# mosure/bevy_gaussian_splatting

Measured on AMD Instinct MI355X. Metric: frames/sec @1080p, 1M-splat 3DGS (sort + rasterize every frame), higher is better.
Workload: dtype f32; 1 GPU; 1000000-splat 3DGS f32 planar cloud (seed 2, reference random_gaussians_3d distributions), 1920x1080, SH degree 3, CloudSettings::default(), examples/headless.rs camera incl. its Msaa (Bevy's default Sample4: 4 samples per pixel, resolved frame); one camera per GPU; sample_count=4, parallelism=views1, sort=radix32, frames_in_flight=8, lanes=8, streams=4

## Files before the change

### bevy_gaussian_splatting_amd/_native.py

```python
from __future__ import annotations

import ctypes
import os
from typing import Optional

from . import _build_id
from .camera import BgsView
from .settings import BgsSettings

_HERE = os.path.dirname(os.path.abspath(__file__))
LIB_PATH = os.path.join(_HERE, "csrc", "libbgs.so")

BGS_OK = 0
BGS_EINVAL = -1
BGS_ENOMEM = -2
BGS_EHIP = -3
BGS_ECAPACITY = -4
BGS_EINTERNAL = -5

STAGE_NAMES = ("keygen", "depth_sort", "project", "tile_sort", "ranges", "raster")

EXPORTED_SYMBOLS = (
    "bgs_create",
    "bgs_destroy",
    "bgs_last_error",
    "bgs_version",
    "bgs_build_id",
    "bgs_set_queue_holders",
    "bgs_set_tile_trace",
    "bgs_selftest_ln_f32",
    "bgs_selftest_pack",
    "bgs_settings_default",
    "bgs_view_perspective",
    "bgs_cloud_upload_f32",
    "bgs_cloud_upload_f16",
    "bgs_cloud_free",
    "bgs_cloud_len",
    "bgs_sort",
    "bgs_render",
    "bgs_framebuffer_device_ptr",
    "bgs_sorted_entries_device_ptr",
    "bgs_set_output_srgb8",
    "bgs_framebuffer_srgb8_device_ptr",
    "bgs_set_srgb8_target",
    "bgs_set_pipeline_depth",
    "bgs_pipeline_pop",
    "bgs_frames_in_flight",
    "bgs_synchronize",
    "bgs_set_async",
    "bgs_stream",
    "bgs_set_profiling",
    "bgs_set_profiling_stride",
    "bgs_set_binning",
    "bgs_set_debug_flags",
    "bgs_get_stats",
    "bgs_radix_sort_pairs",
    "bgs_hbm_probe",
    "bgs_download",
    "bgs_set_pipeline_streams",
    "bgs_set_graphs",
    "bgs_graph_counters",
    "bgs_tile_order_counters",
    "bgs_selftest_tile_order",
    "bgs_reset_adaptive_state",
    "bgs_cloud_upload_cov3d_f32",
    "bgs_adaptive_counters",
    "bgs_set_output_rgba16f",
    "bgs_framebuffer_rgba16f_device_ptr",
    "bgs_set_packed_only",
    "bgs_device_alloc",
    "bgs_device_free",
    "bgs_upload",
    "bgs_abi_check",
    "bgs_learning_counters",
    "bgs_comm_unique_id",
    "bgs_comm_create",
    "bgs_comm_gather",
    "bgs_comm_gather_after",
    "bgs_comm_wait",
    "bgs_comm_stream",
    "bgs_comm_destroy",
)

COMM_ID_BYTES = 128
ABI_VERSION = (0 << 16) | 4


class BgsSortEntry(ctypes.Structure):
    _fields_ = [("key", ctypes.c_uint32), ("index", ctypes.c_uint32)]


class BgsStats(ctypes.Structure):
    _fields_ = [
        ("stage_ms", ctypes.c_float * 6),
        ("total_ms", ctypes.c_float),
        ("splat_count", ctypes.c_uint32),
        ("visible_count", ctypes.c_uint32),
        ("draw_count", ctypes.c_uint32),
        ("sort_path", ctypes.c_uint32),
        ("instance_count", ctypes.c_uint64),
        ("instance_capacity", ctypes.c_uint64),
        ("tiles_x", ctypes.c_uint32),
        ("tiles_y", ctypes.c_uint32),
        ("depth_passes", ctypes.c_uint32),
        ("tile_passes", ctypes.c_uint32),
        ("algorithmic_bytes", ctypes.c_uint64),
        ("regrow_count", ctypes.c_uint32),
        ("binning_mode", ctypes.c_uint32),
        ("frames_averaged", ctypes.c_uint32),
        ("list_capacity", ctypes.c_uint32),
        ("list_entries_allocated", ctypes.c_uint64),
        ("strip_tiles", ctypes.c_uint32),
        ("tile_saturation", ctypes.c_uint32),
    ]


class BgsError(RuntimeError):
    def __init__(self, status: int, message: str):
        super().__init__(f"libbgs error {status}: {message}")
        self.status = status


_lib: Optional[ctypes.CDLL] = None


def rebuild() -> str:
    import subprocess
    p = subprocess.run(["make", "-C", os.path.join(_HERE, "csrc"), "-j4", "ARCH=gfx950"], stdout=subprocess.PIPE,
                       stderr=subprocess.STDOUT, text=True)
    if p.returncode != 0:
        raise ImportError(f"building libbgs.so failed:\n{p.stdout}")
    return p.stdout


def ensure_current() -> str:
    want = _build_id.kernel_source_sha256()
    have = _build_id.library_build_id(LIB_PATH) if os.path.exists(LIB_PATH) else None
    if have != want and os.environ.get("BGS_NO_AUTOBUILD", "0") != "1":
        import fcntl
        with open(os.path.join(_HERE, "csrc", ".build.lock"), "w") as lock:
            fcntl.flock(lock, fcntl.LOCK_EX)
            try:
                have = _build_id.library_build_id(LIB_PATH) if os.path.exists(LIB_PATH) else None
                if have != want:
                    rebuild()
                    have = _build_id.library_build_id(LIB_PATH) if os.path.exists(LIB_PATH) else None
            finally:
                fcntl.flock(lock, fcntl.LOCK_UN)
    if have is None:
        raise ImportError(
            f"{LIB_PATH} not found (or it carries no build id): build the HIP extension first "
            "(python -c 'import __graft_entry__ as g; g.build()'); there is no CPU fallback")
    if have != want:
        raise ImportError(f"{LIB_PATH} was built from kernel sources {have[:12]}, this tree is {want[:12]}: rebuild it "
                          "(make -C bevy_gaussian_splatting_amd/csrc)")
    return want


def build_id() -> str:
    return load().bgs_build_id().decode()


def load() -> ctypes.CDLL:
    global _lib
    if _lib is not None:
        return _lib
    override = os.environ.get("BGS_LIB_OVERRIDE")
    if override:
        import sys
        print(f"bevy_gaussian_splatting_amd: BGS_LIB_OVERRIDE={override} — NOT the library of this tree "
              f"(build id {_build_id.library_build_id(override)})", file=sys.stderr)
        lib = ctypes.CDLL(override, mode=ctypes.RTLD_GLOBAL)
        lib.bgs_build_id.argtypes = []
        lib.bgs_build_id.restype = ctypes.c_char_p
    else:
        want = ensure_current()
        lib = ctypes.CDLL(LIB_PATH, mode=ctypes.RTLD_GLOBAL)
        lib.bgs_build_id.argtypes = []
        lib.bgs_build_id.restype = ctypes.c_char_p
        if lib.bgs_build_id().decode() != want:
            raise ImportError(f"{LIB_PATH}: bgs_build_id() disagrees with the id in the file's bytes")
    vp = ctypes.c_void_p
    u32 = ctypes.c_uint32
    fp = ctypes.POINTER(ctypes.c_float)
    up = ctypes.POINTER(ctypes.c_uint32)

    lib.bgs_create.argtypes = [ctypes.c_int, ctypes.POINTER(vp)]
    lib.bgs_create.restype = ctypes.c_int
    lib.bgs_destroy.argtypes = [vp]
    lib.bgs_destroy.restype = None
    lib.bgs_last_error.argtypes = [vp]
    lib.bgs_last_error.restype = ctypes.c_char_p
    lib.bgs_version.argtypes = []
    lib.bgs_version.restype = u32
    lib.bgs_build_id.argtypes = []
    lib.bgs_build_id.restype = ctypes.c_char_p
    lib.bgs_set_tile_trace.argtypes = [vp, vp]
    lib.bgs_set_tile_trace.restype = ctypes.c_int
    lib.bgs_set_queue_holders.argtypes = [ctypes.c_int]
    lib.bgs_set_queue_holders.restype = ctypes.c_int
    lib.bgs_selftest_ln_f32.argtypes = [vp, u32, u32, ctypes.POINTER(ctypes.c_float), ctypes.POINTER(ctypes.c_uint64)]
    lib.bgs_selftest_ln_f32.restype = ctypes.c_int
    lib.bgs_selftest_pack.argtypes = [vp, u32, vp, u32, vp]
    lib.bgs_selftest_pack.restype = ctypes.c_int
    lib.bgs_settings_default.argtypes = [ctypes.POINTER(BgsSettings)]
    lib.bgs_settings_default.restype = None
    lib.bgs_view_perspective.argtypes = [
        fp, ctypes.c_float, ctypes.c_float, u32, u32, ctypes.POINTER(BgsView)]
    lib.bgs_view_perspective.restype = None
    lib.bgs_cloud_upload_f32.argtypes = [vp, u32, fp, fp, fp, fp, ctypes.POINTER(vp)]
    lib.bgs_cloud_upload_f32.restype = ctypes.c_int
    lib.bgs_cloud_upload_f16.argtypes = [vp, u32, fp, up, up, ctypes.POINTER(vp)]
    lib.bgs_cloud_upload_f16.restype = ctypes.c_int
    lib.bgs_cloud_free.argtypes = [vp, vp]
    lib.bgs_cloud_free.restype = None
    lib.bgs_cloud_len.argtypes = [vp]
    lib.bgs_cloud_len.restype = u32
    lib.bgs_sort.argtypes = [
        vp, vp, ctypes.POINTER(BgsView), ctypes.POINTER(BgsSettings), ctypes.POINTER(BgsSortEntry)]
    lib.bgs_sort.restype = ctypes.c_int
    lib.bgs_render.argtypes = [
        vp, vp, ctypes.POINTER(BgsView), ctypes.POINTER(BgsSettings), fp]
    lib.bgs_render.restype = ctypes.c_int
    lib.bgs_framebuffer_device_ptr.argtypes = [vp, ctypes.POINTER(vp), ctypes.POINTER(ctypes.c_uint64)]
    lib.bgs_framebuffer_device_ptr.restype = ctypes.c_int
    lib.bgs_sorted_entries_device_ptr.argtypes = [vp, ctypes.POINTER(vp), up]
    lib.bgs_sorted_entries_device_ptr.restype = ctypes.c_int
    lib.bgs_synchronize.argtypes = [vp]
    lib.bgs_synchronize.restype = ctypes.c_int
    lib.bgs_set_output_srgb8.argtypes = [vp, ctypes.c_int]
    lib.bgs_set_output_srgb8.restype = ctypes.c_int
    lib.bgs_framebuffer_srgb8_device_ptr.argtypes = [vp, ctypes.POINTER(vp), ctypes.POINTER(ctypes.c_uint64)]
    lib.bgs_framebuffer_srgb8_device_ptr.restype = ctypes.c_int
    lib.bgs_set_srgb8_target.argtypes = [vp, vp]
    lib.bgs_set_srgb8_target.restype = ctypes.c_int
    lib.bgs_set_pipeline_depth.argtypes = [vp, u32]
    lib.bgs_set_pipeline_depth.restype = ctypes.c_int
    lib.bgs_pipeline_pop.argtypes = [vp, ctypes.POINTER(vp), ctypes.POINTER(vp)]
    lib.bgs_pipeline_pop.restype = ctypes.c_int
    lib.bgs_frames_in_flight.argtypes = [vp, up]
    lib.bgs_frames_in_flight.restype = ctypes.c_int
    lib.bgs_set_async.argtypes = [vp, ctypes.c_int]
    lib.bgs_set_async.restype = ctypes.c_int
    lib.bgs_stream.argtypes = [vp, ctypes.POINTER(vp)]
    lib.bgs_stream.restype = ctypes.c_int
    lib.bgs_set_profiling.argtypes = [vp, ctypes.c_int]
    lib.bgs_set_profiling.restype = ctypes.c_int
    lib.bgs_set_profiling_stride.argtypes = [vp, u32]
    lib.bgs_set_profiling_stride.restype = ctypes.c_int
    lib.bgs_set_binning.argtypes = [vp, u32]
    lib.bgs_set_binning.restype = ctypes.c_int
    lib.bgs_set_debug_flags.argtypes = [vp, u32]
    lib.bgs_set_debug_flags.restype = ctypes.c_int
    lib.bgs_get_stats.argtypes = [vp, ctypes.POINTER(BgsStats)]
    lib.bgs_get_stats.restype = ctypes.c_int
    lib.bgs_radix_sort_pairs.argtypes = [vp, ctypes.POINTER(BgsSortEntry), u32, u32]
    lib.bgs_radix_sort_pairs.restype = ctypes.c_int
    lib.bgs_hbm_probe.argtypes = [ctypes.c_void_p, ctypes.c_uint64, ctypes.c_uint32,
                                  ctypes.POINTER(ctypes.c_float), ctypes.POINTER(ctypes.c_float)]
    lib.bgs_hbm_probe.restype = ctypes.c_int
    lib.bgs_download.argtypes = [vp, vp, vp, ctypes.c_uint64]
    lib.bgs_download.restype = ctypes.c_int
    lib.bgs_set_pipeline_streams.argtypes = [vp, u32]
    lib.bgs_set_pipeline_streams.restype = ctypes.c_int
    lib.bgs_set_graphs.argtypes = [vp, ctypes.c_int]
    lib.bgs_set_graphs.restype = ctypes.c_int
    lib.bgs_graph_counters.argtypes = [vp, ctypes.POINTER(ctypes.c_uint64), ctypes.POINTER(ctypes.c_uint64)]
    lib.bgs_graph_counters.restype = ctypes.c_int
    lib.bgs_tile_order_counters.argtypes = [vp] + [ctypes.POINTER(ctypes.c_uint64)] * 3
    lib.bgs_tile_order_counters.restype = ctypes.c_int
    lib.bgs_selftest_tile_order.argtypes = [vp, vp, u32, u32, vp, vp]
    lib.bgs_selftest_tile_order.restype = ctypes.c_int
    lib.bgs_cloud_upload_cov3d_f32.argtypes = [vp, ctypes.c_uint32, ctypes.POINTER(ctypes.c_float), ctypes.POINTER(ctypes.c_float),
                                               ctypes.POINTER(ctypes.c_float), ctypes.POINTER(vp)]
    lib.bgs_cloud_upload_cov3d_f32.restype = ctypes.c_int
    lib.bgs_set_output_rgba16f.argtypes = [vp, ctypes.c_int]
    lib.bgs_set_output_rgba16f.restype = ctypes.c_int
    lib.bgs_set_packed_only.argtypes = [vp, ctypes.c_int]
    lib.bgs_set_packed_only.restype = ctypes.c_int
    lib.bgs_framebuffer_rgba16f_device_ptr.argtypes = [vp, ctypes.POINTER(vp), ctypes.POINTER(ctypes.c_uint64)]
    lib.bgs_framebuffer_rgba16f_device_ptr.restype = ctypes.c_int
    lib.bgs_device_alloc.argtypes = [vp, ctypes.c_uint64, ctypes.POINTER(vp)]
    lib.bgs_device_alloc.restype = ctypes.c_int
    lib.bgs_device_free.argtypes = [vp, vp]
    lib.bgs_device_free.restype = ctypes.c_int
    lib.bgs_upload.argtypes = [vp, vp, vp, ctypes.c_uint64]
    lib.bgs_upload.restype = ctypes.c_int
    lib.bgs_adaptive_counters.argtypes = [vp, ctypes.POINTER(ctypes.c_uint64)]
    lib.bgs_adaptive_counters.restype = ctypes.c_int
    lib.bgs_reset_adaptive_state.argtypes = [vp]
    lib.bgs_reset_adaptive_state.restype = ctypes.c_int
    lib.bgs_learning_counters.argtypes = [vp, ctypes.POINTER(ctypes.c_uint64), ctypes.POINTER(ctypes.c_uint64)]
    lib.bgs_learning_counters.restype = ctypes.c_int
    lib.bgs_abi_check.argtypes = [u32, u32, u32, u32]
    lib.bgs_abi_check.restype = ctypes.c_int
    lib.bgs_comm_unique_id.argtypes = [ctypes.c_char_p]
    lib.bgs_comm_unique_id.restype = ctypes.c_int
    lib.bgs_comm_create.argtypes = [vp, ctypes.c_char_p, u32, u32, ctypes.POINTER(vp)]
    lib.bgs_comm_create.restype = ctypes.c_int
    lib.bgs_comm_gather.argtypes = [vp, vp, u32, vp, ctypes.c_uint64, vp, ctypes.POINTER(ctypes.c_uint64)]
    lib.bgs_comm_gather.restype = ctypes.c_int
    lib.bgs_comm_gather_after.argtypes = [vp, vp, u32, vp, ctypes.c_uint64, vp, vp, ctypes.POINTER(ctypes.c_uint64)]
    lib.bgs_comm_gather_after.restype = ctypes.c_int
    lib.bgs_comm_wait.argtypes = [vp, vp, ctypes.c_uint64]
    lib.bgs_comm_wait.restype = ctypes.c_int
    lib.bgs_comm_stream.argtypes = [vp, vp, ctypes.POINTER(vp)]
    lib.bgs_comm_stream.restype = ctypes.c_int
    lib.bgs_comm_destroy.argtypes = [vp, vp]
    lib.bgs_comm_destroy.restype = None
    rc = lib.bgs_abi_check(ABI_VERSION, ctypes.sizeof(BgsView), ctypes.sizeof(BgsSettings), ctypes.sizeof(BgsStats))
    if rc != BGS_OK:
        raise ImportError("libbgs.so refuses this binding: " + (lib.bgs_last_error(None) or b"").decode("utf-8", "replace"))
    _lib = lib
    return lib


def check(lib: ctypes.CDLL, ctx, status: int) -> None:
    if status != BGS_OK:
        msg = lib.bgs_last_error(ctx)
        raise BgsError(status, msg.decode("utf-8", "replace") if msg else "")
```

### bevy_gaussian_splatting_amd/csrc/bgs_api.hip

```cpp
#include "bgs_context.h"
#include "build_id.inc"

static const char g_build_id[] = "BGS_BUILD_ID=" BGS_BUILD_ID;

namespace {
void mat4_mul(const float* a, const float* b, float* out) {
    for (int c = 0; c < 4; ++c)
        for (int r = 0; r < 4; ++r) {
            float acc = 0.0f;
            for (int k = 0; k < 4; ++k) acc += a[4 * k + r] * b[4 * c + k];
            out[4 * c + r] = acc;
        }
}

bool mat4_inverse(const float* m, float* out) {
    double a[4][8];
    for (int r = 0; r < 4; ++r)
        for (int c = 0; c < 4; ++c) {
            a[r][c] = m[4 * c + r];
            a[r][4 + c] = r == c ? 1.0 : 0.0;
        }
    for (int i = 0; i < 4; ++i) {
        int piv = i;
        for (int r = i + 1; r < 4; ++r)
// ... 154 lines not shown
    if (n && (!pv || !sh || !rot || !so)) return fail(ctx, BGS_EINVAL, "NULL plane pointer");
    if (hipSetDevice(ctx->device) != hipSuccess) return fail(ctx, BGS_EHIP, "hipSetDevice failed");
    bgs_cloud* c = new (std::nothrow) bgs_cloud();
    if (!c) return fail(ctx, BGS_ENOMEM, "out of host memory");
    const void* const planes[3] = {rot, so, sh};
    const uint32_t v4[3] = {1u, 1u, 12u};
    int rc = upload_and_pack(ctx, c, CLOUD_F32, n, pv, planes, v4, 16u);
    if (rc != BGS_OK) { bgs_cloud_free(ctx, c); return rc; }
    *out = c;
    return BGS_OK;
}

int bgs_cloud_upload_f16(bgs_ctx* ctx, uint32_t n, const float* pv, const uint32_t* sh_h2,
                         const uint32_t* rso, bgs_cloud** out) {
    if (!ctx) return fail(nullptr, BGS_EINVAL, "ctx is NULL");
    if (!out) return fail(ctx, BGS_EINVAL, "out is NULL");
    *out = nullptr;
    if (n > MAX_SPLATS) return fail(ctx, BGS_EINVAL, "too many splats");
    if (n && (!pv || !sh_h2 || !rso)) return fail(ctx, BGS_EINVAL, "NULL plane pointer");
    if (hipSetDevice(ctx->device) != hipSuccess) return fail(ctx, BGS_EHIP, "hipSetDevice failed");
    bgs_cloud* c = new (std::nothrow) bgs_cloud();
    if (!c) return fail(ctx, BGS_ENOMEM, "out of host memory");
    const void* const planes[3] = {rso, sh_h2, nullptr};
    const uint32_t v4[3] = {1u, 6u, 0u};
    int rc = upload_and_pack(ctx, c, CLOUD_F16, n, pv, planes, v4, 8u);
    if (rc != BGS_OK) { bgs_cloud_free(ctx, c); return rc; }
    *out = c;
    return BGS_OK;
}

int bgs_cloud_upload_cov3d_f32(bgs_ctx* ctx, uint32_t n, const float* pv, const float* sh, const float* cov3d_opacity,
                               bgs_cloud** out) {
    if (!ctx) return fail(nullptr, BGS_EINVAL, "ctx is NULL");
    if (!out) return fail(ctx, BGS_EINVAL, "out is NULL");
    *out = nullptr;
    if (n > MAX_SPLATS) return fail(ctx, BGS_EINVAL, "too many splats");
    if (n && (!pv || !sh || !cov3d_opacity)) return fail(ctx, BGS_EINVAL, "NULL plane pointer");
    if (hipSetDevice(ctx->device) != hipSuccess) return fail(ctx, BGS_EHIP, "hipSetDevice failed");
    bgs_cloud* c = new (std::nothrow) bgs_cloud();
    if (!c) return fail(ctx, BGS_ENOMEM, "out of host memory");
    const void* const planes[3] = {cov3d_opacity, nullptr, sh};
    const uint32_t v4[3] = {2u, 0u, 12u};
    int rc = upload_and_pack(ctx, c, CLOUD_COV3D, n, pv, planes, v4, 16u);
    if (rc != BGS_OK) { bgs_cloud_free(ctx, c); return rc; }
    *out = c;
    return BGS_OK;
}

void bgs_cloud_free(bgs_ctx* ctx, bgs_cloud* cloud) {
    if (!cloud) return;
    if (ctx) {
        (void)hipSetDevice(ctx->device);
        (void)finish_all(ctx);
        for (auto& L : ctx->lanes) {
            if (L.stream) (void)hipStreamSynchronize(L.stream);
            if (L.in.cloud == cloud) L.in.cloud = nullptr;
        }
        for (auto& sl : ctx->split_slots)
            if (sl.cloud == cloud) sl.epoch = 0;
    }
    for (auto p : cloud->allocs) if (p) (void)hipFree(p);
    delete cloud;
}

uint32_t bgs_cloud_len(const bgs_cloud* cloud) { return cloud ? cloud->ptrs.n : 0; }

int bgs_sort(bgs_ctx* ctx, const bgs_cloud* cloud, const bgs_view* view, const bgs_settings* settings,
             bgs_sort_entry* host_out) {
    int rc = run(ctx, cloud, view, settings, false);
    if (rc != BGS_OK) return rc;
    Lane& L = ctx->lanes[0];
    if (host_out && L.last_sorted_n)
        HIP_TRY(ctx, hipMemcpy(host_out, L.last_sorted, (size_t)L.last_sorted_n * sizeof(uint2), hipMemcpyDeviceToHost));
    return BGS_OK;
}

int bgs_render(bgs_ctx* ctx, const bgs_cloud* cloud, const bgs_view* view, const bgs_settings* settings,
               float* rgba_host_out) {
    int rc = run(ctx, cloud, view, settings, true);
    if (rc != BGS_OK) return rc;
    if (rgba_host_out) {
        Lane& L = ctx->lanes[ctx->recent];
        if (L.pending && (rc = finish_lane(ctx, L)) != BGS_OK) return rc;
        if (!L.fb_valid) return fail(ctx, BGS_EINVAL, "the frame wrote its packed image only (bgs_set_packed_only): no f32 target to copy");
        HIP_TRY(ctx, hipMemcpy(rgba_host_out, L.fb, (size_t)L.fb_w * L.fb_h * sizeof(float4), hipMemcpyDeviceToHost));
    }
    return BGS_OK;
}

int bgs_framebuffer_device_ptr(bgs_ctx* ctx, void** dptr, uint64_t* bytes) {
    if (!ctx || !dptr) return fail(ctx, BGS_EINVAL, "NULL argument");
    Lane& L = ctx->lanes[ctx->recent];
    if (L.pending) {
        int rc = finish_lane(ctx, L);
        if (rc != BGS_OK) return rc;
    }
    if (!L.fb) return fail(ctx, BGS_EINVAL, "no frame has been rendered yet");
    if (!L.fb_valid) return fail(ctx, BGS_EINVAL, "the last frame wrote its packed image only (bgs_set_packed_only)");
    *dptr = L.fb;
    if (bytes) *bytes = (uint64_t)L.fb_w * L.fb_h * sizeof(float4);
    return BGS_OK;
}

int bgs_framebuffer_srgb8_device_ptr(bgs_ctx* ctx, void** dptr, uint64_t* bytes) {
    if (!ctx || !dptr) return fail(ctx, BGS_EINVAL, "NULL argument");
    Lane& L = ctx->lanes[ctx->recent];
    if (L.pending) {
        int rc = finish_lane(ctx, L);
        if (rc != BGS_OK) return rc;
    }
    if (!L.fb8_out || !L.fb8_valid || L.fb8_is_f16)
        return fail(ctx, BGS_EINVAL, "no Rgba8UnormSrgb frame: call bgs_set_output_srgb8(ctx, 1) before rendering");
    *dptr = L.fb8_out;
    if (bytes) *bytes = (uint64_t)L.fb_w * L.fb_h * 4u;
    return BGS_OK;
}

int bgs_pipeline_pop(bgs_ctx* ctx, void** rgba_f32, void** rgba8) {
    if (!ctx) return fail(nullptr, BGS_EINVAL, "ctx is NULL");
    if (hipSetDevice(ctx->device) != hipSuccess) return fail(ctx, BGS_EHIP, "hipSetDevice failed");
    int best = -1;
    for (int i = 0; i < MAX_LANES; ++i)
        if ((ctx->lanes[i].pending || ctx->lanes[i].ready) && (best < 0 || ctx->lanes[i].seq < ctx->lanes[best].seq)) best = i;
    if (best < 0) return fail(ctx, BGS_EINVAL, "no frame in flight");
    Lane& L = ctx->lanes[best];
    int rc = finish_lane(ctx, L);
    if (rc != BGS_OK) return rc;
    if (rgba_f32) *rgba_f32 = L.fb_valid ? L.fb : nullptr;
    if (rgba8) *rgba8 = L.fb8_valid ? L.fb8_out : nullptr;
    return BGS_OK;
}

int bgs_frames_in_flight(bgs_ctx* ctx, uint32_t* count) {
    if (!ctx || !count) return fail(ctx, BGS_EINVAL, "NULL argument");
    uint32_t c = 0;
    for (auto& L : ctx->lanes) c += (L.pending || L.ready) ? 1u : 0u;
    *count = c;
    return BGS_OK;
}

int bgs_sorted_entries_device_ptr(bgs_ctx* ctx, void** dptr, uint32_t* n) {
    if (!ctx || !dptr) return fail(ctx, BGS_EINVAL, "NULL argument");
    Lane& L = ctx->lanes[ctx->recent];
    if (L.pending) {
        int rc = finish_lane(ctx, L);
        if (rc != BGS_OK) return rc;
    }
    if (!L.last_sorted) return fail(ctx, BGS_EINVAL, "no sort has been run yet");
    *dptr = (void*)L.last_sorted;
    if (n) *n = L.last_sorted_n;
    return BGS_OK;
}

int bgs_synchronize(bgs_ctx* ctx) {
    if (!ctx) return fail(nullptr, BGS_EINVAL, "ctx is NULL");
    if (hipSetDevice(ctx->device) != hipSuccess) return fail(ctx, BGS_EHIP, "hipSetDevice failed");
    int rc = finish_all(ctx);
    if (rc != BGS_OK) return rc;
    for (auto& L : ctx->lanes)
        if (L.stream) HIP_TRY(ctx, hipStreamSynchronize(L.stream));
    return BGS_OK;
}

int bgs_set_async(bgs_ctx* ctx, int enabled) {
    if (!ctx) return fail(nullptr, BGS_EINVAL, "ctx is NULL");
    if (!enabled) {
        int rc = finish_all(ctx);
        if (rc != BGS_OK) return rc;
    }
    ctx->async_frames = enabled != 0;
    return BGS_OK;
}

int bgs_set_pipeline_depth(bgs_ctx* ctx, uint32_t lanes) {
    if (!ctx) return fail(nullptr, BGS_EINVAL, "ctx is NULL");
    if (lanes < 1 || lanes > (uint32_t)MAX_LANES) return fail(ctx, BGS_EINVAL, "pipeline depth must be 1..8");
    if (hipSetDevice(ctx->device) != hipSuccess) return fail(ctx, BGS_EHIP, "hipSetDevice failed");
    int rc = finish_all(ctx);
    if (rc != BGS_OK) return rc;
    ctx->depth = (int)lanes;
    ctx->next = 0;
    ctx->recent = 0;
    for (uint32_t i = 0; i < lanes; ++i)
        if ((rc = lane_create(ctx, ctx->lanes[i])) != BGS_OK) return rc;
    return assign_streams(ctx);
}

int bgs_set_pipeline_streams(bgs_ctx* ctx, uint32_t streams) {
    if (!ctx) return fail(nullptr, BGS_EINVAL, "ctx is NULL");
    if (streams > (uint32_t)MAX_LANES) return fail(ctx, BGS_EINVAL, "pipeline streams must be 0..8");
    if (hipSetDevice(ctx->device) != hipSuccess) return fail(ctx, BGS_EHIP, "hipSetDevice failed");
    int rc = finish_all(ctx);
    if (rc != BGS_OK) return rc;
    for (auto st : ctx->streams)
        if (st) HIP_TRY(ctx, hipStreamSynchronize(st));
    ctx->num_streams = (int)streams;
    return assign_streams(ctx);
}

int bgs_set_srgb8_target(bgs_ctx* ctx, void* device_ptr) {
    if (!ctx) return fail(nullptr, BGS_EINVAL, "ctx is NULL");
    ctx->next_srgb8_target = (uint32_t*)device_ptr;
    return BGS_OK;
}

int bgs_download(bgs_ctx* ctx, const void* device_ptr, void* host_out, uint64_t bytes) {
    if (!ctx || !device_ptr || !host_out) return fail(ctx, BGS_EINVAL, "NULL argument");
    if (hipSetDevice(ctx->device) != hipSuccess) return fail(ctx, BGS_EHIP, "hipSetDevice failed");
    if (bytes) HIP_TRY(ctx, hipMemcpy(host_out, device_ptr, (size_t)bytes, hipMemcpyDeviceToHost));
    return BGS_OK;
}

int bgs_device_alloc(bgs_ctx* ctx, uint64_t bytes, void** device_ptr_out) {
    if (!ctx || !device_ptr_out) return fail(ctx, BGS_EINVAL, "NULL argument");
    *device_ptr_out = nullptr;
    if (hipSetDevice(ctx->device) != hipSuccess) return fail(ctx, BGS_EHIP, "hipSetDevice failed");
    void* p = nullptr;
    if (hipMalloc(&p, std::max<size_t>((size_t)bytes, 16)) != hipSuccess) {
        (void)hipGetLastError();
        return fail(ctx, BGS_ENOMEM, "hipMalloc(" + std::to_string(bytes) + " bytes) failed");
    }
    *device_ptr_out = p;
    return BGS_OK;
}

int bgs_device_free(bgs_ctx* ctx, void* device_ptr) {
    if (!ctx) return fail(nullptr, BGS_EINVAL, "ctx is NULL");
    if (!device_ptr) return BGS_OK;
    if (hipSetDevice(ctx->device) != hipSuccess) return fail(ctx, BGS_EHIP, "hipSetDevice failed");
    int rc = finish_all(ctx);
    if (rc != BGS_OK) return rc;
    HIP_TRY(ctx, hipFree(device_ptr));
    return BGS_OK;
}

int bgs_upload(bgs_ctx* ctx, void* device_ptr, const void* host_in, uint64_t bytes) {
    if (!ctx || !device_ptr || !host_in) return fail(ctx, BGS_EINVAL, "NULL argument");
    if (hipSetDevice(ctx->device) != hipSuccess) return fail(ctx, BGS_EHIP, "hipSetDevice failed");
    if (bytes) HIP_TRY(ctx, hipMemcpy(device_ptr, host_in, (size_t)bytes, hipMemcpyHostToDevice));
    return BGS_OK;
}

int bgs_set_output_srgb8(bgs_ctx* ctx, int enabled) {
    if (!ctx) return fail(nullptr, BGS_EINVAL, "ctx is NULL");
    ctx->output_srgb8 = enabled != 0;
    if (enabled) ctx->output_rgba16f = false;
    return BGS_OK;
}

int bgs_set_output_rgba16f(bgs_ctx* ctx, int enabled) {
    if (!ctx) return fail(nullptr, BGS_EINVAL, "ctx is NULL");
    ctx->output_rgba16f = enabled != 0;
    if (enabled) ctx->output_srgb8 = false;
    return BGS_OK;
}

int bgs_set_packed_only(bgs_ctx* ctx, int enabled) {
    if (!ctx) return fail(nullptr, BGS_EINVAL, "ctx is NULL");
    ctx->packed_only = enabled != 0;
    return BGS_OK;
}

int bgs_framebuffer_rgba16f_device_ptr(bgs_ctx* ctx, void** dptr, uint64_t* bytes) {
    if (!ctx || !dptr) return fail(ctx, BGS_EINVAL, "NULL argument");
    Lane& L = ctx->lanes[ctx->recent];
    if (L.pending) {
        int rc = finish_lane(ctx, L);
        if (rc != BGS_OK) return rc;
    }
    if (!L.fb8_out || !L.fb8_valid || !L.fb8_is_f16)
        return fail(ctx, BGS_EINVAL, "no Rgba16Float frame: call bgs_set_output_rgba16f(ctx, 1) before rendering");
    *dptr = L.fb8_out;
    if (bytes) *bytes = (uint64_t)L.fb_w * L.fb_h * 8u;
    return BGS_OK;
}

int bgs_stream(bgs_ctx* ctx, void** hip_stream) {
    if (!ctx || !hip_stream) return fail(ctx, BGS_EINVAL, "NULL argument");
    *hip_stream = (void*)ctx->lanes[ctx->recent].stream;
    return BGS_OK;
}

int bgs_set_profiling(bgs_ctx* ctx, int enabled) {
    if (!ctx) return fail(nullptr, BGS_EINVAL, "ctx is NULL");
    if (enabled < 0 || enabled > 2) return fail(ctx, BGS_EINVAL, "profiling level must be 0, 1 or 2");
    ctx->profiling = enabled;
    return BGS_OK;
}

int bgs_set_profiling_stride(bgs_ctx* ctx, uint32_t every_nth_frame) {
    if (!ctx) return fail(nullptr, BGS_EINVAL, "ctx is NULL");
    if (every_nth_frame == 0) return fail(ctx, BGS_EINVAL, "stride must be >= 1");
    ctx->profiling_stride = every_nth_frame;
    ctx->frame_counter = 0;
    return BGS_OK;
}

int bgs_set_binning(bgs_ctx* ctx, uint32_t mode) {
    if (!ctx) return fail(nullptr, BGS_EINVAL, "ctx is NULL");
    if (mode > BINNING_SORT) return fail(ctx, BGS_EINVAL, "binning mode must be 0 (scan) or 1 (sort)");
    int rc = finish_all(ctx);
    if (rc != BGS_OK) return rc;
    ctx->binning = mode;
    return BGS_OK;
}

// ... 102 lines not shown
```

### bevy_gaussian_splatting_amd/csrc/bgs_context.h

```cpp
#pragma once
#include <hip/hip_runtime.h>

#include <dlfcn.h>

#include <algorithm>
#include <chrono>
#include <cmath>
#include <cstdio>
#include <cstdlib>
#include <cstring>
#include <mutex>
#include <new>
#include <string>
#include <unordered_map>
#include <vector>

#include "../../include/bgs.h"
#include "../../include/bgs_diag.h"
#include "bgs_device.h"
#include "frame_params.h"
#include "kernels.h"

using namespace bgs;

struct bgs_cloud {
    CloudPtrs ptrs{};
    void* allocs[4] = {nullptr, nullptr, nullptr, nullptr};
    uint64_t bytes = 0;
};

namespace bgs_host {

extern thread_local std::string g_error;

constexpr uint64_t MIN_INSTANCE_CAPACITY = 1ull << 22;
constexpr uint64_t MAX_INSTANCE_CAPACITY = 1ull << 30;
constexpr uint32_t MAX_SPLATS = (1u << 30) - 1u;
constexpr int EV_COUNT = BGS_STAGE_COUNT + 1;
constexpr int EV_RING = 64;
constexpr int MAX_LANES = 8;

template <class T>
T* dev_alloc(size_t count) {
    void* p = nullptr;
    if (hipMalloc(&p, std::max<size_t>(count, 1) * sizeof(T)) != hipSuccess) return nullptr;
    return (T*)p;
}

struct GraphKey {
    const void* cloud[6];
    const void* bufs[11];
    uint32_t n, format, places, sort_mode, gaussian_mode, aabb, any_mode, srgb8, debug_flags;
    int32_t width, height;
    int32_t sort_blocks, bin_blocks, keygen_blocks;
    uint32_t sup_edge;
    uint64_t scratch_bytes, scratch_inst_cap;
    uint32_t scratch_n, coarse_cap, sort_path;
    const void* keygen_func;
    uint32_t keygen_threads;
    uint32_t wide_bin;
    uint32_t raster_variant;
    uint32_t split_sub;
};
struct FrameGraph {
    hipGraph_t graph = nullptr;
    hipGraphExec_t exec = nullptr;
    hipGraphNode_t keygen_node = nullptr;
    GraphKey key{};
};

struct FrameInputs {
    const bgs_cloud* cloud = nullptr;
    bgs_view view{};
    bgs_settings settings{};
    bool render = false, allow_graph = false;
    uint32_t* srgb8_target = nullptr;
    bool output_srgb8 = false, output_rgba16f = false, packed_only = false;
    uint32_t debug_flags = 0;
    uint64_t kind = 0;
    bool force_passes = false;
};

struct FramePlan {
    FrameParams fp{};
    bool render = false, scan = false, surfel = false, culled_tail = true;
    uint32_t n = 0, places = 0, rec_bytes = 0, cloud_format = 0;
    bool bucket = false, wide = false;
    uint32_t bucket_sub = 1, split_sub_out = 1;
    int split_slot = -1;
    uint64_t split_epoch = 0;
    uint32_t edges[4] = {6, 8, 16, 32}, level = 1, sup_edge = 8, num_st = 0;
    bool large = false, wide_bin = false, want_srgb8 = false;
    int sort_blocks = 0, bin_blocks = 0, binning_blocks = 0;
    uint32_t out_format = 0, ntiles = 0;
    bool raster_cleans = false;
    RasterInst raster{};
    bool heavy = false, cost = false, ordered = false, refresh = false, graph_ok = false;
    uint64_t sat_kind = 0;
};

struct Lane {
    hipStream_t stream = nullptr;
    hipEvent_t done = nullptr;
    FrameParams* d_fp = nullptr;
    FrameGraph graph[2];

    uint8_t* scratch = nullptr;
    size_t scratch_bytes = 0;
    size_t off_depth_status = 0, off_scan_status = 0, off_tile_status = 0, off_ranges = 0, off_bin_status = 0,
           off_part_status = 0, off_ctl1 = 0;
    uint32_t ctl_parity = 0;
    bool scratch_clean = false;
    uint32_t scratch_n = 0;
    uint64_t scratch_inst_cap = 0;

    uint2* entries[2] = {nullptr, nullptr};
    uint2* culled = nullptr;
    uint32_t entries_cap = 0;
    void* records = nullptr;
    size_t records_bytes = 0;
    uint32_t* rects = nullptr;
    uint2* inst[2] = {nullptr, nullptr};
    uint64_t inst_cap = 0;
    uint32_t* coarse = nullptr;
    size_t coarse_entries = 0;
    uint2* bucket_slots = nullptr;
    uint32_t bucket_sub_cap = 0;
    uint32_t* d_split_keys = nullptr;
    uint32_t* h_split_keys = nullptr;
    uint8_t* heavy[2] = {nullptr, nullptr};
    uint32_t heavy_tiles = 0, heavy_parity = 0;
    const uint8_t* heavy_done = nullptr;
    uint32_t heavy_done_grid = 0;
    bool ready = false;
    uint16_t* cost[2] = {nullptr, nullptr};
    uint16_t* order = nullptr;
    uint32_t cost_tiles = 0, cost_parity = 0;
    const uint16_t* cost_done = nullptr;
    uint32_t cost_done_grid = 0;
    uint32_t order_grid = 0xFFFFFFFFu, order_age = 0;
    float4* fb = nullptr;
    size_t fb_pixels = 0;
    uint32_t* fb8 = nullptr;
    uint32_t* fb8_out = nullptr;
    size_t fb8_pixels = 0;
    uint32_t fb_w = 0, fb_h = 0;
    bool fb8_valid = false, fb8_is_f16 = false;
    bool fb_valid = true;

    Control* h_ctl = nullptr;
    Control* h_ctl_dev = nullptr;
    hipEvent_t ev_ring[EV_RING][EV_COUNT] = {};
    uint8_t ev_kind[EV_RING] = {};
    uint32_t ev_head = 0;
    uint32_t frames_timed = 0;

    bool pending = false;
    FrameInputs in;
    FramePlan plan;
    uint32_t pending_coarse_cap = 0;
    uint64_t cost_done_kind = 0;
    uint64_t order_kind = 0;
    uint64_t seq = 0;

    const uint2* last_sorted = nullptr;
    uint32_t last_sorted_n = 0;

    bgs_stats result{};
    bool has_result = false;
    uint8_t result_kind = 0;
};

}
using namespace bgs_host;

struct bgs_ctx {
    int device = 0;
    int num_cus = 256;
    std::string error;

    Lane lanes[MAX_LANES];
    hipStream_t streams[MAX_LANES] = {};
    int num_streams = 4;
    int depth = 1;
    int next = 0;
    int recent = 0;
    uint64_t seq = 0;

    uint32_t binning = BINNING_SCAN;
    uint32_t debug_flags = 0;
    int profiling = 2;
    uint32_t profiling_stride = 1;
    uint32_t frame_counter = 0;
    bool async_frames = false;
    bool output_srgb8 = false;
    bool output_rgba16f = false;
    bool packed_only = false;
    uint32_t* next_srgb8_target = nullptr;

    uint32_t draw_hint = 0;
    bool draw_hint_valid = false;
    uint32_t draw_shrink_votes = 0;
    uint32_t sup_level = 1;
    struct SplitterSlot {
        SplitterKeys table{};
        const bgs_cloud* cloud = nullptr;
        uint32_t n = 0;
        uint32_t sort_mode = 0;
        float transform[16] = {};
        float pos[3] = {}, fwd[3] = {};
        float clip_from_view[16] = {};
        float viewport_wh[2] = {};
        float reach = 0.0f;
        uint64_t epoch = 0;
        uint64_t last_used = 0;
    };
    static constexpr int SPLITTER_SLOTS = 16;
    SplitterSlot split_slots[SPLITTER_SLOTS];
    uint64_t split_epoch = 0;
    uint64_t split_failed_epoch = 0;
    uint32_t bucket_block = 0;
    uint32_t bucket_fail_streak = 0;
    uint32_t list_shrink_votes = 0;
    uint64_t bucket_frames = 0, onesweep_frames = 0;
    uint64_t reruns_sort = 0, reruns_lists = 0, reruns_instances = 0, level_changes = 0;
    uint32_t coarse_cap_hint = 0;
    struct KindState { uint32_t sup_level = 1; bool midround = false; };
    std::unordered_map<uint64_t, KindState> kinds;
    static constexpr uint32_t LEARN_MAX = 3;
    static constexpr double MIDROUND_ON = 0.30, MIDROUND_OFF = 0.15;
    uint64_t cur_kind = 0;
    std::unordered_map<uint64_t, uint32_t> learning;
    uint64_t early_frames = 0;
    uint4* tile_trace = nullptr;
    bool use_graphs = false;
    uint64_t graph_captures = 0, graph_replays = 0;
    uint64_t cost_frames = 0, ordered_frames = 0, order_refreshes = 0;

    bool have_stats = false;
    bgs_stats stats{};
// ... 26 lines not shown
```

### bevy_gaussian_splatting_amd/csrc/bgs_frame.hip

```cpp
#include "bgs_context.h"

thread_local std::string bgs_host::g_error;

namespace bgs_host {


constexpr int MAX_DEVICES = 64;
hipStream_t g_queue_holders[MAX_DEVICES][3] = {};
int g_queue_holders_mode = -1;
std::mutex g_queue_holders_mutex;

int fail(bgs_ctx* ctx, int status, const std::string& msg) {
    if (ctx) ctx->error = msg;
    g_error = msg;
    return status;
}


size_t align_up(size_t v, size_t a) { return (v + a - 1) / a * a; }

int assign_streams(bgs_ctx* ctx) {
    const int S = ctx->num_streams > 0 ? std::min(ctx->num_streams, ctx->depth) : ctx->depth;
    for (int i = 0; i < MAX_LANES; ++i) {
        Lane& L = ctx->lanes[i];
// ... 514 lines not shown
    stt.tiles_x = render ? (uint32_t)p.fp.tiles_x : 0;
    stt.tiles_y = render ? (uint32_t)p.fp.tiles_y : 0;
    stt.depth_passes = p.places;
    stt.tile_passes = (render && !scan) ? 2 : 0;
    stt.binning_mode = scan ? BINNING_SCAN : BINNING_SORT;
    const uint64_t N = p.n, k = p.places, D = h.draw_count;
    uint64_t bytes = N * 16 + D * 8 + (p.culled_tail ? (N - D) * 8 : 0) + (p.bucket ? D * 24 : k * D * 16);
    if (render) {
        const uint64_t B = p.cloud_format == CLOUD_F16 ? 128 : 240, R = p.rec_bytes, V = h.visible_count, I = t.instances;
        const uint64_t P = (uint64_t)(uint32_t)p.fp.width * (uint32_t)p.fp.height;
        if (scan)
            bytes += V * (B - 16) + V * R + V * 8 + V * 8 + I * 8 + I * 8 + P * 16;
        else
            bytes += V * (B - 16) + V * R + I * 8 + 2 * I * 16 + I * (4 + R) + P * 16;
    }
    stt.algorithmic_bytes = bytes;
    L.has_result = true;
    L.result_kind = (uint8_t)(!render ? 1 : (scan ? 2 : 3));
}

int finish_lane(bgs_ctx* ctx, Lane& L) {
    L.ready = false;
    for (int attempt = 0; L.pending; ++attempt) {
        HIP_TRY(ctx, hipEventSynchronize(L.done));
        L.pending = false;
        int rc = check_watchdog(ctx, L);
        if (rc != BGS_OK) return rc;
        const FramePlan& p = L.plan;
        const Control& h = *L.h_ctl;
        const FrameTotals t = frame_totals(p, h);
        bool rerun = false;
        if ((rc = check_capacities(ctx, L, t, attempt, &rerun)) != BGS_OK) return rc;
        if (rerun) {
            if (attempt >= 8) return fail(ctx, BGS_ECAPACITY, "frame kept overflowing its buffers");
            ctx->regrow_count += 1;
            if ((rc = enqueue_frame(ctx, L, L.in)) != BGS_OK) return rc;
            continue;
        }

        if (p.render && p.scan) learn_feedback(ctx, L);
        learn_draw_hint(ctx, h.draw_count);
        learn_splitters(ctx, L);
        const bool level_moved = p.render && p.scan && h.visible_count > 0 && learn_level(ctx, L, t);
        if (p.render && p.scan && attempt == 0 && !level_moved && L.in.kind) {
            if (ctx->kinds.size() >= (1u << 20)) ctx->kinds.clear();
            ctx->kinds[L.in.kind].sup_level = p.level;
        }

        L.last_sorted_n = p.render ? h.draw_count : p.n;
        if (!p.render && h.draw_count < p.n) {
            HIP_TRY(ctx, hipMemcpyAsync(const_cast<uint2*>(L.last_sorted) + h.draw_count, L.culled,
                                        (size_t)(p.n - h.draw_count) * sizeof(uint2), hipMemcpyDeviceToDevice, L.stream));
            HIP_TRY(ctx, hipStreamSynchronize(L.stream));
        }
        fill_stats(ctx, L, t);
    }
    return BGS_OK;
}

int finish_all(bgs_ctx* ctx) {
    for (;;) {
        int best = -1;
        for (int i = 0; i < MAX_LANES; ++i)
            if (ctx->lanes[i].pending && (best < 0 || ctx->lanes[i].seq < ctx->lanes[best].seq)) best = i;
        if (best < 0) break;
        int rc = finish_lane(ctx, ctx->lanes[best]);
        if (rc != BGS_OK) return rc;
    }
    for (auto& L : ctx->lanes) L.ready = false;
    return BGS_OK;
}

int collect_stats(bgs_ctx* ctx) {
    Lane& R = ctx->lanes[ctx->recent];
    if (!R.has_result) return fail(ctx, BGS_EINVAL, "no frame has been run yet");
    ctx->stats = R.result;
    bgs_stats& stt = ctx->stats;
    if (ctx->profiling >= 1) {
        const uint8_t kind = R.result_kind;
        const bool render = kind != 1, scan = kind == 2;
        const int last = render ? 6 : 2;
        uint32_t used = 0;
        float acc[BGS_STAGE_COUNT] = {0, 0, 0, 0, 0, 0}, acc_total = 0.0f;
        for (auto& L : ctx->lanes) {
            const uint32_t frames = std::min<uint32_t>(L.frames_timed, EV_RING);
            for (uint32_t f = 0; f < frames; ++f) {
                const uint32_t slot = (L.ev_head + EV_RING - f) % EV_RING;
                if (L.ev_kind[slot] != kind) continue;
                hipEvent_t* const ev = L.ev_ring[slot];
                auto ms = [&](int a, int b) { float t = 0; (void)hipEventElapsedTime(&t, ev[a], ev[b]); return t; };
                if (ctx->profiling >= 2) {
                    acc[BGS_STAGE_KEYGEN] += ms(0, 1);
                    acc[BGS_STAGE_DEPTH_SORT] += ms(1, 2);
                    if (render && scan) {
                        acc[BGS_STAGE_PROJECT] += ms(2, 3);
                        acc[BGS_STAGE_RASTER] += ms(3, 6);
                    } else if (render) {
                        acc[BGS_STAGE_PROJECT] += ms(2, 3);
                        acc[BGS_STAGE_TILE_SORT] += ms(3, 4);
                        acc[BGS_STAGE_RANGES] += ms(4, 5);
                        acc[BGS_STAGE_RASTER] += ms(5, 6);
                    }
                }
                acc_total += ms(0, last);
                ++used;
            }
            L.frames_timed = 0;
        }
        if (used) {
            for (int i = 0; i < BGS_STAGE_COUNT; ++i) stt.stage_ms[i] = acc[i] / (float)used;
            stt.total_ms = acc_total / (float)used;
        }
        stt.frames_averaged = used;
    }
    ctx->have_stats = true;
    return BGS_OK;
}

FramePlan plan_frame(const bgs_ctx& ctx, const Lane& L, const FrameInputs& in) {
    FramePlan p;
    const uint32_t flags = in.debug_flags;
    const bgs_settings* s = &in.settings;
    FrameParams& fp = p.fp;
    fill_frame_params(in.cloud->ptrs.n, &in.view, s, fp);
    fp.debug = flags;
    fp.srgb8_target = (uint64_t)(uintptr_t)in.srgb8_target;
    const uint32_t n = p.n = fp.n;
    p.places = depth_places(s);
    p.render = in.render;
    p.scan = ctx.binning == BINNING_SCAN;
    p.surfel = in.render && fp.gaussian_mode == 0u && fp.aabb != 0u;
    p.rec_bytes = p.surfel ? sizeof(RecordSurfel) : sizeof(Record);
    p.cloud_format = in.cloud->ptrs.format;
    p.culled_tail = !in.render || s->rasterize_mode == BGS_RASTERIZE_DEPTH;

    const bool hint = ctx.draw_hint_valid;
    const int slot = (p.places == 4 && n > 0) ? find_splitter_slot(&ctx, in.cloud, &in.view, s) : -1;
    const uint32_t narrow_max = BUCKET_COUNT * BUCKET_SUB_KERNARG * BUCKET_TARGET;
    p.wide = (hint && ctx.draw_hint > narrow_max && !(flags & BGS_DEBUG_BUCKETS_NARROW)) || (flags & BGS_DEBUG_BUCKETS_WIDE);
    const uint32_t cap_out = p.wide ? BUCKET_CAP_WIDE : BUCKET_CAP, target_out = p.wide ? BUCKET_TARGET_WIDE : BUCKET_TARGET;
    p.bucket = p.places == 4 && n > 0 && !(flags & BGS_DEBUG_NO_BUCKET_SORT) && ctx.bucket_block == 0 && !in.force_passes &&
               ((slot >= 0 && hint) || (flags & BGS_DEBUG_GUESSED_SPLITTERS)) &&
               (!hint || ctx.draw_hint <= BUCKET_MAX * (cap_out / 4u) * 3u);
    if (hint)
        p.split_sub_out = std::min<uint32_t>(std::max<uint32_t>((ctx.draw_hint + BUCKET_COUNT * target_out - 1u) / (BUCKET_COUNT * target_out), 1u), BUCKET_SUB_MAX);
    if (flags & BGS_DEBUG_SPLIT_SUB_3) p.split_sub_out = std::max<uint32_t>(p.split_sub_out, BUCKET_SUB_KERNARG);
    if (flags & BGS_DEBUG_SPLIT_SUB_5) p.split_sub_out = std::max<uint32_t>(p.split_sub_out, 5u);
    if (p.bucket && slot >= 0) {
        p.bucket_sub = std::min<uint32_t>(std::max<uint32_t>(ctx.split_slots[slot].table.sub, 1u), BUCKET_SUB_MAX);
        if (hint && ctx.draw_hint > BUCKET_COUNT * p.bucket_sub * (cap_out / 4u) * 3u) p.bucket = false;
    }
    if (p.bucket && slot >= 0) { p.split_slot = slot; p.split_epoch = ctx.split_slots[slot].epoch; }
    fp.sort_path = p.bucket ? 1u : 0u;

    supertile_edges((uint32_t)fp.tiles_x, (uint32_t)fp.tiles_y, p.edges);
    uint32_t level = ctx.sup_level;
    if (flags & BGS_DEBUG_LEVEL_0) level = 0;
    else if (flags & BGS_DEBUG_LEVEL_1) level = 1;
    else if (flags & BGS_DEBUG_LEVEL_2) level = 2;
    else if (flags & BGS_DEBUG_LEVEL_3) level = 3;
    p.level = canonical_supertile_level(level, p.edges);
    p.sup_edge = supertile_bins_fit((uint32_t)fp.tiles_x, (uint32_t)fp.tiles_y, p.edges[p.level]) ? p.edges[p.level] : p.edges[1];
    p.num_st = (((uint32_t)fp.tiles_x + p.sup_edge - 1) / p.sup_edge) * (((uint32_t)fp.tiles_y + p.sup_edge - 1) / p.sup_edge);

    p.large = n > (4u << 20);
    p.wide_bin = ctx.depth == 1;
    p.sort_blocks = ctx.num_cus * 4;
    p.bin_blocks = ctx.num_cus * 3;
    p.binning_blocks = ctx.num_cus * 4;
    if (hint && !(flags & BGS_DEBUG_NO_DRAW_HINT)) {
        const uint64_t want = (uint64_t)ctx.draw_hint / sort_tile_size(p.large) + 8;
        p.sort_blocks = (int)std::min<uint64_t>((uint64_t)p.sort_blocks, std::max<uint64_t>(want, 32));
        p.bin_blocks = (int)std::min<uint64_t>((uint64_t)p.bin_blocks, std::max<uint64_t>((uint64_t)ctx.draw_hint / 256 + 8, 32));
        p.binning_blocks = (int)std::min<uint64_t>((uint64_t)p.binning_blocks, std::max<uint64_t>((uint64_t)ctx.draw_hint / 1024 + 4, 16));
    }
    p.want_srgb8 = in.render && (in.output_srgb8 || in.output_rgba16f || in.srgb8_target);
    p.out_format = !p.want_srgb8 ? 0u : ((in.output_rgba16f ? OUT_RGBA16F : OUT_SRGB8) |
                                         ((in.packed_only && p.scan) ? OUT_SKIP_F32 : 0u));

    p.raster_cleans = in.render && p.scan && fp.tiles_x > 0 && fp.tiles_y > 0 && !(flags & BGS_DEBUG_NO_RASTER_CLEANUP);
    bool kind_midround = false;
    if (ctx.depth > 1) { const auto kit = ctx.kinds.find(in.kind); if (kit != ctx.kinds.end()) kind_midround = kit->second.midround; }
    p.raster = raster_instantiation(fp, p.level, kind_midround, ctx.depth, flags);
    p.ntiles = (uint32_t)(fp.tiles_x * fp.tiles_y);
    const bool feedback = p.raster_cleans && !(in.allow_graph && ctx.use_graphs) && p.ntiles <= 65535u;
    p.heavy = feedback && p.raster.mode == 1 && p.level >= 2u && !ctx.tile_trace &&
              (ctx.depth == 1 || (flags & BGS_DEBUG_STRIPS_ANY_DEPTH)) && !(flags & BGS_DEBUG_NO_STRIPS);
    p.cost = feedback && (ctx.depth == 1 || !(flags & BGS_DEBUG_NO_TILE_COST_PIPELINED)) && !(flags & BGS_DEBUG_NO_TILE_COST);
    if (p.cost && p.ntiles > (uint32_t)(ctx.num_cus * 4 * raster_scan_waves_per_simd(fp))) {
        const uint32_t grid = (uint32_t)fp.tiles_x | ((uint32_t)fp.tiles_y << 16);
        const bool kept = L.cost[0] && p.ntiles <= L.cost_tiles;
        const bool have_costs = kept && L.cost_done && L.cost_done != L.cost[L.cost_parity] && L.cost_done_grid == grid;
        const bool have_order = kept && L.order_grid == grid;
        p.refresh = have_costs && (!have_order || L.order_age + 1u >= TILE_ORDER_REFRESH || (flags & BGS_DEBUG_ORDER_EVERY_FRAME));
        p.ordered = p.refresh || have_order;
    }
    p.sat_kind = !p.ordered ? 0 : (p.refresh ? L.cost_done_kind : L.order_kind);
    p.graph_ok = in.allow_graph && ctx.use_graphs && p.raster_cleans && p.bucket_sub <= BUCKET_SUB_KERNARG &&
                 !(flags & BGS_DEBUG_NO_GRAPHS) && !ctx.tile_trace;
    return p;
}

GraphKey graph_key(const FramePlan& p, const FrameInputs& in, const Lane& L, const KeygenLaunch& kg, uint32_t coarse_cap) {
    GraphKey key;
    std::memset(&key, 0, sizeof key);
    const FrameParams& fp = p.fp;
    const void* planes[6] = {in.cloud->ptrs.position_visibility, in.cloud->ptrs.packed, nullptr, nullptr, nullptr, nullptr};
    std::memcpy(key.cloud, planes, sizeof planes);
    const void* bufs[11] = {L.entries[0], L.entries[1], L.culled, L.records, L.coarse, L.fb, L.fb8, L.scratch, L.d_fp,
                            L.h_ctl_dev, L.bucket_slots};
    std::memcpy(key.bufs, bufs, sizeof bufs);
    key.n = p.n; key.format = p.cloud_format; key.places = p.places; key.sort_mode = in.settings.sort_mode;
    key.gaussian_mode = fp.gaussian_mode; key.aabb = fp.aabb;
    key.any_mode = (fp.rasterize_mode != RASTERIZE_COLOR || fp.draw_mode != 0u) ? 1u : 0u;
    key.srgb8 = p.out_format;
    key.debug_flags = in.debug_flags;
    key.width = fp.width; key.height = fp.height;
    key.sort_blocks = p.bucket ? 0 : p.sort_blocks;
    key.bin_blocks = p.bin_blocks * 4096 + p.binning_blocks;
    key.keygen_blocks = (int32_t)kg.blocks; key.keygen_func = kg.func; key.keygen_threads = kg.threads;
    key.wide_bin = p.wide_bin ? 1u : 0u;
    const RasterInst& r = p.raster;
    key.raster_variant = r.samples | (r.depth ? 0x100u : 0u) | (r.overlay ? 0x200u : 0u) | (r.mode == 1 ? 0x400u : r.mode == 2 ? 0x800u : 0u);
    key.split_sub = p.split_sub_out;
    key.sup_edge = p.sup_edge;
    key.scratch_bytes = L.scratch_bytes; key.scratch_inst_cap = L.scratch_inst_cap; key.scratch_n = L.scratch_n;
    key.coarse_cap = coarse_cap;
    key.sort_path = p.bucket ? (p.bucket_sub | (p.wide ? 0x100u : 0u)) : 0u;
    return key;
}

template <class Issue>
int launch_graph(bgs_ctx* ctx, Lane& L, const GraphKey& key, KeygenLaunch& kg, Issue&& issue) {
    FrameGraph& G = L.graph[L.ctl_parity];
    if (G.exec && std::memcmp(&G.key, &key, sizeof key) == 0) {
        HIP_TRY(ctx, kg.update_node(G.exec, G.keygen_node));
        ctx->graph_replays += 1;
    } else {
        graph_destroy(G);
        HIP_TRY(ctx, hipStreamBeginCapture(L.stream, hipStreamCaptureModeThreadLocal));
        const hipError_t ie = issue();
        const hipError_t ce = hipStreamEndCapture(L.stream, &G.graph);
        size_t roots = 1;
        if (ie != hipSuccess || ce != hipSuccess || !G.graph ||
            hipGraphInstantiate(&G.exec, G.graph, nullptr, nullptr, 0) != hipSuccess ||
            hipGraphGetRootNodes(G.graph, &G.keygen_node, &roots) != hipSuccess || roots != 1) {
            graph_destroy(G);
            (void)hipGetLastError();
            return fail(ctx, BGS_EHIP, "capturing the frame into a hipGraph failed");
        }
        G.key = key;
        ctx->graph_captures += 1;
    }
    HIP_TRY(ctx, hipGraphLaunch(G.exec, L.stream));
    return BGS_OK;
}

int ensure_frame_buffers(bgs_ctx* ctx, Lane& L, const FramePlan& p, const FrameInputs& in, uint32_t* coarse_cap) {
    int rc;
    if ((rc = lane_create(ctx, L)) != BGS_OK) return rc;
    if ((rc = ensure_entries(ctx, L, p.n)) != BGS_OK) return rc;
    if (p.bucket && p.bucket_sub > BUCKET_SUB_KERNARG && !L.d_split_keys) {
        L.d_split_keys = dev_alloc<uint32_t>(BUCKET_MAX);
        void* hp = nullptr;
        if (!L.d_split_keys || hipHostMalloc(&hp, BUCKET_MAX * sizeof(uint32_t), hipHostMallocDefault) != hipSuccess) {
            (void)hipGetLastError();
            return fail(ctx, BGS_ENOMEM, "hipMalloc / hipHostMalloc(splitter table) failed");
        }
        L.h_split_keys = (uint32_t*)hp;
    }
    if (p.bucket && (rc = ensure_bucket_slots(ctx, L, p.bucket_sub, p.wide)) != BGS_OK) return rc;
    if (p.render) {
        if (p.scan) {
            if ((rc = ensure_coarse(ctx, L, p.n, p.num_st, in.debug_flags, coarse_cap)) != BGS_OK) return rc;
            if ((rc = ensure_rects(ctx, L)) != BGS_OK) return rc;
        } else {
            if ((rc = ensure_instances(ctx, L, std::max<uint64_t>(L.inst_cap, MIN_INSTANCE_CAPACITY))) != BGS_OK) return rc;
        }
        if ((rc = ensure_records(ctx, L, (size_t)p.n * p.rec_bytes)) != BGS_OK) return rc;
        if ((rc = ensure_framebuffer(ctx, L, (uint32_t)p.fp.width, (uint32_t)p.fp.height, in.output_srgb8 || in.output_rgba16f)) != BGS_OK) return rc;
    }
    if ((rc = ensure_scratch(ctx, L, p.n, L.inst_cap)) != BGS_OK) return rc;
    if (p.heavy && (rc = ensure_heavy(ctx, L, p.ntiles)) != BGS_OK) return rc;
    if (p.cost && (rc = ensure_cost(ctx, L, p.ntiles)) != BGS_OK) return rc;
    return BGS_OK;
}

int enqueue_frame(bgs_ctx* ctx, Lane& L, const FrameInputs& in) {
    const FramePlan p = plan_frame(*ctx, L, in);
    const FrameParams& fp = p.fp;
    const uint32_t n = p.n, places = p.places, flags = in.debug_flags;
    const bool render = p.render, scan = p.scan, bucket = p.bucket;

    uint32_t coarse_cap = 1;
    int rc = ensure_frame_buffers(ctx, L, p, in, &coarse_cap);
    if (rc != BGS_OK) return rc;

    hipStream_t st = L.stream;
    const bool need_memset = !L.scratch_clean;
    if (need_memset) L.ctl_parity = 0;
    Control* ctl = (Control*)(L.scratch + (L.ctl_parity ? L.off_ctl1 : 0));
    uint32_t* depth_status = (uint32_t*)(L.scratch + L.off_depth_status);
    unsigned long long* scan_status = (unsigned long long*)(L.scratch + L.off_scan_status);
    uint32_t* tile_status = (uint32_t*)(L.scratch + L.off_tile_status);
    uint2* ranges = (uint2*)(L.scratch + L.off_ranges);
    uint32_t* bin_status = (uint32_t*)(L.scratch + L.off_bin_status);
    uint32_t* part_status = (uint32_t*)(L.scratch + L.off_part_status);
    const size_t depth_tiles = ((size_t)L.scratch_n + sort_tile_size(false) - 1) / sort_tile_size(false) + 1;
    const uint32_t grid = (uint32_t)fp.tiles_x | ((uint32_t)fp.tiles_y << 16);
    uint8_t* const heavy_out = p.heavy ? L.heavy[L.heavy_parity] : nullptr;
    const uint8_t* const heavy_in = (p.heavy && L.heavy_done && L.heavy_done != heavy_out && L.heavy_done_grid == grid) ? L.heavy_done : nullptr;
    uint16_t* const cost_out = p.cost ? L.cost[L.cost_parity] : nullptr;
    const uint16_t* const cost_in = p.refresh ? L.cost_done : nullptr;
    uint16_t* const tile_order = p.ordered ? L.order : nullptr;
    uint2* const draw_list = L.entries[places & 1u];
    const uint32_t final_xor = (fp.sort_mode == BGS_SORT_RAYON || fp.sort_mode == BGS_SORT_STD) ? 0xFFFFFFFFu : 0u;

    KeygenLaunch kg{};
    kg.fp = fp;
    kg.pos = in.cloud->ptrs.position_visibility;
    kg.entries = L.entries[0];
    kg.culled = p.culled_tail ? L.culled : nullptr;
    kg.ctl = ctl;
    kg.part_status = part_status;
    kg.places = places;
    kg.ticket_slot = 7;
    kg.fp_out = L.d_fp;
    kg.zero_word = reinterpret_cast<uint32_t*>(heavy_out);
    kg.bucket_slots = L.bucket_slots;
    kg.bucket_status = depth_status;
    if (bucket) {
        if (p.split_slot >= 0) {
            const SplitterKeys& tk = ctx->split_slots[p.split_slot].table;
            const uint32_t nkeys = BUCKET_COUNT * p.bucket_sub - 1u;
            if (p.bucket_sub <= BUCKET_SUB_KERNARG) std::memcpy(kg.split.key, tk.key, nkeys * sizeof(uint32_t));
            else std::memcpy(L.h_split_keys, tk.key, nkeys * sizeof(uint32_t));
            kg.split.device_keys = L.d_split_keys;
        } else {
            for (uint32_t i = 0; i < BUCKET_COUNT; ++i) kg.split.key[i] = (i + 1u) << 24;
        }
        kg.split.sub = p.bucket_sub;
        kg.split.wide = p.wide ? 1u : 0u;
    }
    kg.wide = p.wide_bin;
    const bool have_keygen = kg.prepare(ctx->num_cus * 4);
    FrameCleanup cl{};
    if (p.raster_cleans) {
        cl.part_status = part_status;
        cl.depth_status = depth_status;
        cl.bin_status = bin_status;
        cl.other_ctl = (Control*)(L.scratch + (L.ctl_parity ? 0 : L.off_ctl1));
        cl.host_ctl = L.h_ctl_dev;
        cl.pass_stride = (uint32_t)(depth_tiles * RADIX_BASE);
        cl.places = bucket ? 0u : places;
        cl.depth_tile = sort_tile_size(p.large);
        cl.sorted = draw_list;
        cl.key_xor = final_xor;
        cl.split_sub = p.split_sub_out;
        if (tile_order) cl.order_stats = reinterpret_cast<const uint32_t*>(reinterpret_cast<const uint8_t*>(tile_order) + tile_order_stats_offset(p.ntiles));
    }

    if (ctx->bucket_block > 0 && places == 4) ctx->bucket_block -= 1;
    if (bucket) ctx->bucket_frames += 1;
    else if (places > 0) ctx->onesweep_frames += 1;
    if (bucket && p.split_slot >= 0) ctx->split_slots[p.split_slot].last_used = ctx->seq + 1;
    if (p.cost) ctx->cost_frames += 1;
    if (p.ordered) ctx->ordered_frames += 1;
    if (p.refresh) { ctx->order_refreshes += 1; L.order_kind = L.cost_done_kind; L.order_grid = grid; L.order_age = 0; }
    else if (p.ordered) L.order_age += 1u;
    const bool timed_frame = (ctx->frame_counter++ % ctx->profiling_stride) == 0;
    const int prof = timed_frame ? ctx->profiling : 0;
    const int last_mark = render ? 6 : 2;
    if (prof) {
        L.ev_head = (L.ev_head + 1) % EV_RING;
        L.ev_kind[L.ev_head] = (uint8_t)(!render ? 1 : (scan ? 2 : 3));
        L.frames_timed += 1;
    }
    hipEvent_t* const ev = L.ev_ring[L.ev_head];
    auto mark = [&](int i) {
        if (prof >= 2 || (prof == 1 && (i == 0 || i == last_mark))) (void)hipEventRecord(ev[i], st);
    };

    auto issue = [&]() -> hipError_t {
        mark(0);
        if (cost_in) launch_tile_order(st, cost_in, tile_order, p.ntiles, fp, p.raster.mode != 0);
        if (have_keygen) {
            if (bucket && p.bucket_sub > BUCKET_SUB_KERNARG) {
                const hipError_t ce = hipMemcpyAsync(L.d_split_keys, L.h_split_keys, (BUCKET_COUNT * p.bucket_sub - 1u) * sizeof(uint32_t),
                                                     hipMemcpyHostToDevice, st);
                if (ce != hipSuccess) return ce;
            }
            hipError_t e = kg.launch(st);
            if (e != hipSuccess) return e;
        }
        mark(1);
        int cur = 0;
        if (bucket) {
            const hipError_t e = launch_bucket_sort(st, L.bucket_slots, draw_list, ctl, final_xor, BUCKET_COUNT * p.bucket_sub, p.wide);
            if (e != hipSuccess) return e;
        }
        for (uint32_t q = 0; q < (bucket ? 0u : places); ++q) {
            launch_onesweep_pass(st, L.entries[cur], L.entries[cur ^ 1], &ctl->draw_count, n, ctl->hist_depth[q],
                                 depth_status + (size_t)q * depth_tiles * RADIX_BASE, &ctl->ticket[q][0], &ctl->error,
                                 q * RADIX_BITS, q + 1 == places ? final_xor : 0u, p.large, p.sort_blocks);
            cur ^= 1;
        }
        mark(2);
        if (render && scan) {
            launch_project_bin(st, fp, L.d_fp, in.cloud->ptrs, draw_list, L.culled, ctl, bin_status, L.records, L.rects, L.coarse,
                               coarse_cap, p.sup_edge, 4, p.bin_blocks, p.binning_blocks, p.wide_bin);
            mark(3);
            launch_raster_scan(st, fp, L.d_fp, L.records, L.coarse, coarse_cap, p.sup_edge, ctl, L.fb, L.fb8,
                               (flags & BGS_DEBUG_SEPARATE_ENCODE) ? 0u : p.out_format, cl, ctx->tile_trace,
                               p.raster.mode, heavy_in, heavy_out, tile_order, cost_out);
            mark(6);
        } else if (render) {
            const uint32_t capacity = (uint32_t)std::min<uint64_t>(L.inst_cap, MAX_INSTANCE_CAPACITY);
            launch_project_emit(st, fp, in.cloud->ptrs, draw_list, L.culled, ctl, scan_status, L.records, L.inst[0], capacity,
                                4, ctx->num_cus * 3);
            mark(3);
            const size_t inst_tiles = (L.scratch_inst_cap + sort_tile_size(true) - 1) / sort_tile_size(true) + 1;
            for (uint32_t q = 0; q < 2; ++q)
                launch_onesweep_pass(st, L.inst[q], L.inst[q ^ 1], &ctl->instance_count, capacity, ctl->hist_tile[q],
                                     tile_status + (size_t)q * inst_tiles * RADIX_BASE, &ctl->ticket[5 + q][0],
                                     &ctl->error, q * RADIX_BITS, 0u, true, ctx->num_cus * 4);
            mark(4);
            launch_tile_ranges(st, L.inst[0], ctl, ranges);
            mark(5);
            launch_raster(st, fp, L.records, L.inst[0], ranges, L.fb, in.view.clear_color, ctl);
            mark(6);
        }
        if (p.want_srgb8 && !(render && scan && !(flags & BGS_DEBUG_SEPARATE_ENCODE)))
            launch_encode_srgb8(st, L.fb, L.fb8, (uint32_t)fp.width * (uint32_t)fp.height, L.d_fp, p.out_format);
        return hipGetLastError();
    };
    if (p.graph_ok && !need_memset && prof == 0 && have_keygen) {
        if ((rc = launch_graph(ctx, L, graph_key(p, in, L, kg, coarse_cap), kg, issue)) != BGS_OK) return rc;
    } else {
        if (need_memset) HIP_TRY(ctx, hipMemsetAsync(L.scratch, 0, L.scratch_bytes, st));
        if (!have_keygen) HIP_TRY(ctx, hipMemcpyAsync(L.d_fp, &fp, sizeof fp, hipMemcpyHostToDevice, st));
        HIP_TRY(ctx, issue());
    }
    L.scratch_clean = p.raster_cleans;
    if (p.raster_cleans) {
        L.ctl_parity ^= 1u;
    } else {
        if (places == 4 && n > 0) launch_splitters(st, draw_list, ctl, final_xor, p.split_sub_out);
        HIP_TRY(ctx, hipMemcpyAsync(L.h_ctl, ctl, sizeof(Control), hipMemcpyDeviceToHost, st));
    }
    HIP_TRY(ctx, hipEventRecord(L.done, st));

    L.last_sorted = draw_list;
    L.last_sorted_n = n;
    L.fb_valid = !(p.out_format & OUT_SKIP_F32) || (flags & BGS_DEBUG_SEPARATE_ENCODE);
    L.fb8_is_f16 = (p.out_format & OUT_RGBA16F) != 0u;
    L.fb8_valid = p.want_srgb8;
    if (p.want_srgb8) L.fb8_out = in.srgb8_target ? in.srgb8_target : L.fb8;
    L.pending = true;
    L.pending_coarse_cap = coarse_cap;
    L.in = in;
    L.plan = p;
    L.seq = ++ctx->seq;
    return BGS_OK;
}

int run(bgs_ctx* ctx, const bgs_cloud* cloud, const bgs_view* view, const bgs_settings* s, bool render) {
    int rc = validate(ctx, cloud, view, s, render);
    if (rc != BGS_OK) return rc;
    if (hipSetDevice(ctx->device) != hipSuccess) return fail(ctx, BGS_EHIP, "hipSetDevice failed");
    const bool async = ctx->async_frames && render && ctx->binning == BINNING_SCAN;
    Lane& L = ctx->lanes[async ? ctx->next : 0];
    if (!async && (rc = finish_all(ctx)) != BGS_OK) return rc;
    if (async && L.pending && (rc = finish_lane(ctx, L)) != BGS_OK) return rc;
    const FrameInputs in{cloud, *view, *s, render, async, render ? ctx->next_srgb8_target : nullptr,
                         ctx->output_srgb8, ctx->output_rgba16f, ctx->packed_only, ctx->debug_flags,
                         render ? frame_kind(cloud, view, s) : 0ull, false};
    if (!async) {
        ctx->recent = 0;
        ctx->regrow_count = 0;
        if (render) switch_kind(ctx, in.kind);
        if ((rc = enqueue_frame(ctx, L, in)) != BGS_OK) return rc;
        ctx->next_srgb8_target = nullptr;
        return finish_lane(ctx, L);
    }
    L.ready = false;
    const bool learn = ctx->kinds.find(in.kind) == ctx->kinds.end();
    switch_kind(ctx, in.kind);
    if ((rc = enqueue_frame(ctx, L, in)) != BGS_OK) return rc;
    ctx->next_srgb8_target = nullptr;
    ctx->recent = ctx->next;
    ctx->next = (ctx->next + 1) % ctx->depth;
    if (learn) {
        if ((rc = finish_lane(ctx, L)) != BGS_OK) return rc;
        L.ready = true;
        ctx->early_frames += 1;
        if (ctx->kinds.find(in.kind) != ctx->kinds.end()) {
            ctx->learning.erase(in.kind);
        } else if (++ctx->learning[in.kind] >= bgs_ctx::LEARN_MAX) {
            ctx->kinds[in.kind].sup_level = ctx->sup_level;
            ctx->learning.erase(in.kind);
        }
        if (ctx->learning.size() >= (1u << 16)) ctx->learning.clear();
    }
    return BGS_OK;
}

}
```

### bevy_gaussian_splatting_amd/csrc/kernels.h

```cpp
#pragma once
#include <hip/hip_runtime.h>
#include <stdint.h>

#include "bgs_device.h"

namespace bgs {

struct CloudPtrs {
    const float4* position_visibility;
    const uint4* packed;
    uint32_t packed_v4;
    uint32_t n;
    uint32_t format;
};
constexpr uint32_t PACK_ROT = 1u, PACK_SCALE_OPACITY = 2u, PACK_SH_F32 = 3u;
constexpr uint32_t PACK_COV3D = 1u;
constexpr uint32_t PACK_RSO_F16 = 1u, PACK_SH_F16 = 2u;
constexpr uint32_t CLOUD_F32 = 0, CLOUD_F16 = 1, CLOUD_COV3D = 2;

struct FrameCleanup {
    uint32_t* part_status;
    uint32_t* depth_status;
    uint32_t* bin_status;
    Control* other_ctl;
    Control* host_ctl;
    uint32_t pass_stride;
    uint32_t places;
    uint32_t depth_tile;
    const uint2* sorted;
    uint32_t key_xor;
    uint32_t split_sub;
    const uint32_t* order_stats;
};

constexpr int SORT_THREADS = 256;
constexpr int SORT_KPT_SMALL = 8;
constexpr int SORT_KPT_LARGE = 16;
inline uint32_t sort_tile_size(bool large) { return SORT_THREADS * (large ? SORT_KPT_LARGE : SORT_KPT_SMALL); }

struct KeygenLaunch {
    FrameParams fp;
    const float4* pos;
    uint2* entries;
    uint2* culled;
    Control* ctl;
    uint32_t* part_status;
    uint32_t places;
    uint32_t ticket_slot;
    FrameParams* fp_out;
    uint2* bucket_slots;
    uint32_t* bucket_status;
    SplitterTable split;
    uint32_t* zero_word;
    bool wide = false;
    const void* func;
    uint32_t blocks, threads;
    void* argv[13];
    uint32_t lds_bytes;
    bool prepare(int max_blocks);
    hipError_t launch(hipStream_t stream);
    hipError_t update_node(hipGraphExec_t exec, hipGraphNode_t node);
};
constexpr uint32_t KEYGEN_TILE = 2048;
#ifndef BGS_KEYGEN_WIDE_THREADS
#define BGS_KEYGEN_WIDE_THREADS 256
#endif
#ifndef BGS_KEYGEN_HUGE_LOG2
#define BGS_KEYGEN_HUGE_LOG2 (BGS_KEYGEN_WIDE_THREADS == 256 ? 31 : 22)
#endif
inline uint32_t keygen_tile_splats(uint32_t n) { return n >= (1u << BGS_KEYGEN_HUGE_LOG2) ? 8192u : (n >= (1u << 19) ? 4096u : 2048u); }

void launch_histogram(hipStream_t stream, const uint2* pairs, uint32_t n, uint32_t* hist ,
                      uint32_t passes);

void launch_onesweep_pass(hipStream_t stream, const uint2* in, uint2* out, const uint32_t* n_ptr,
                          uint32_t max_n, const uint32_t* hist, uint32_t* status, uint32_t* ticket,
                          uint32_t* error_flag, uint32_t shift, uint32_t key_xor, bool large_tiles,
                          int max_blocks);

hipError_t launch_bucket_sort(hipStream_t stream, const uint2* bucket_slots, uint2* out, Control* ctl, uint32_t key_xor,
                              uint32_t buckets = BUCKET_COUNT , bool wide = false);
void launch_splitters(hipStream_t stream, const uint2* sorted, Control* ctl, uint32_t key_xor, uint32_t sub = 1u);

void launch_project_emit(hipStream_t stream, const FrameParams& fp, const CloudPtrs& cloud,
                         const uint2* draw_list, const uint2* culled, Control* ctl, unsigned long long* scan_status,
                         void* records, uint2* instances, uint32_t capacity, uint32_t ticket_slot,
                         int max_blocks);

void launch_project_bin(hipStream_t stream, const FrameParams& fp, const FrameParams* d_fp, const CloudPtrs& cloud,
                        const uint2* draw_list, const uint2* culled, Control* ctl, uint32_t* bin_status, void* records,
                        uint32_t* rects, uint32_t* coarse, uint32_t coarse_cap, uint32_t sup_edge,
                        uint32_t ticket_slot, int project_blocks, int bin_blocks, bool wide_bin);

void launch_raster_scan(hipStream_t stream, const FrameParams& fp, const FrameParams* d_fp, const void* records,
                        const uint32_t* coarse, uint32_t coarse_cap,
                        uint32_t sup_edge, Control* ctl, float4* framebuffer, uint32_t* srgb8_default,
                        uint32_t out_format, const FrameCleanup& cleanup, uint4* tile_trace = nullptr,
                        int mode = 0 ,
                        const uint8_t* heavy_in = nullptr, uint8_t* heavy_out = nullptr,
                        const uint16_t* order = nullptr, uint16_t* cost_out = nullptr);
constexpr uint32_t TILE_ORDER_REFRESH = 8u;
inline size_t tile_cost_bytes(uint32_t tiles) { return ((size_t)tiles + 4u) * 2u; }
__host__ __device__ inline size_t tile_order_stats_offset(uint32_t tiles) { return (((((size_t)tiles + 3u) / 4u + 8u) * 2u + 63u) / 64u) * 64u; }
inline size_t tile_order_bytes(uint32_t tiles) { return tile_order_stats_offset(tiles) + 16u * sizeof(uint32_t); }
void launch_tile_order(hipStream_t stream, const uint16_t* cost, uint16_t* order, uint32_t ntiles, const FrameParams& fp,
                       bool midround_exit);
void launch_tile_order_runs(hipStream_t stream, const uint16_t* cost, uint16_t* order, uint32_t ntiles, uint32_t runs);
int raster_scan_waves_per_simd(const FrameParams& fp);
constexpr uint32_t HEAVY_CAP = 256u, HEAVY_LIST_OFFSET = 128u, HEAVY_FLAGS_OFFSET = HEAVY_LIST_OFFSET + 2u * HEAVY_CAP;
inline size_t heavy_feedback_bytes(uint32_t tiles) { return (size_t)HEAVY_FLAGS_OFFSET + tiles; }
constexpr uint32_t OUT_SRGB8 = 1u;
constexpr uint32_t OUT_RGBA16F = 2u;
constexpr uint32_t OUT_SKIP_F32 = 4u;

void launch_tile_ranges(hipStream_t stream, const uint2* instances, const Control* ctl, uint2* ranges);

void launch_raster(hipStream_t stream, const FrameParams& fp, const void* records,
                   const uint2* instances, const uint2* ranges, float4* framebuffer,
                   const float clear_color[4], const Control* ctl);

void launch_encode_srgb8(hipStream_t stream, const float4* framebuffer, uint32_t* default_out, uint32_t pixels,
                         const FrameParams* d_fp, uint32_t out_format = 1u);

void launch_pack_cloud(hipStream_t stream, const uint4* pos, const uint4* a, uint32_t v4_a, const uint4* b, uint32_t v4_b,
                       const uint4* c, uint32_t v4_c, uint4* out, uint32_t stride_v4, uint32_t n);

void launch_triad(hipStream_t stream, float4* a, const float4* b, const float4* c, float s, size_t n4,
                  int blocks);

void launch_selftest_ln(hipStream_t stream, uint32_t first_bits, uint32_t count, float* out, unsigned long long* sum,
                        int blocks);

}
```

### bevy_gaussian_splatting_amd/csrc/render_kernels.hip

```cpp
#include <algorithm>
#include <type_traits>

#include <hip/hip_fp16.h>
#include <hip/hip_runtime.h>

#include "kernels.h"
#include "lookback.h"
#include "pack_tables.h"
#include "splat_math.h"

#ifndef BGS_ABLATION
#define BGS_ABLATION 0
#endif

namespace bgs {

namespace {

__device__ __forceinline__ unsigned long long ld_agent64(const unsigned long long* p) {
    return __hip_atomic_load(p, __ATOMIC_RELAXED, __HIP_MEMORY_SCOPE_AGENT);
}
__device__ __forceinline__ void st_agent64(unsigned long long* p, unsigned long long v) {
    __hip_atomic_store(p, v, __ATOMIC_RELAXED, __HIP_MEMORY_SCOPE_AGENT);
}

constexpr unsigned long long S64_FLAG_SHIFT = 62;
constexpr unsigned long long S64_VALUE_MASK = (1ull << S64_FLAG_SHIFT) - 1ull;
constexpr unsigned long long S64_AGGREGATE = 1ull << S64_FLAG_SHIFT;
constexpr unsigned long long S64_PREFIX = 2ull << S64_FLAG_SHIFT;
constexpr uint32_t SPIN_LIMIT = 1u << 22;

__device__ __forceinline__ uint32_t wave_inclusive_scan(uint32_t v, int lane) {
#pragma unroll
    for (int off = 1; off < 64; off <<= 1) {
        uint32_t t = __shfl_up(v, off, 64);
        if (lane >= off) v += t;
    }
    return v;
}

__device__ __forceinline__ float half_bits_to_float(unsigned short h) {
    _Float16 x;
    __builtin_memcpy(&x, &h, 2);
    return (float)x;
}
__device__ __forceinline__ float half_lo(uint32_t v) { return half_bits_to_float((unsigned short)(v & 0xFFFFu)); }
__device__ __forceinline__ float half_hi(uint32_t v) { return half_bits_to_float((unsigned short)(v >> 16)); }

struct ShF32 {
    const float* base;
    __device__ __forceinline__ void load_all(float* c) const {
        const float4* p = reinterpret_cast<const float4*>(base);
#pragma unroll
        for (int i = 0; i < 12; ++i) {
            const float4 v = p[i];
            c[4 * i] = v.x; c[4 * i + 1] = v.y; c[4 * i + 2] = v.z; c[4 * i + 3] = v.w;
        }
    }
};
struct ShF16 {
    const uint32_t* base;
    __device__ __forceinline__ void load_all(float* c) const {
        const uint4* p = reinterpret_cast<const uint4*>(base);
#pragma unroll
        for (int i = 0; i < 6; ++i) {
            const uint4 v = p[i];
            c[8 * i] = half_lo(v.x); c[8 * i + 1] = half_hi(v.x);
            c[8 * i + 2] = half_lo(v.y); c[8 * i + 3] = half_hi(v.y);
            c[8 * i + 4] = half_lo(v.z); c[8 * i + 5] = half_hi(v.z);
            c[8 * i + 6] = half_lo(v.w); c[8 * i + 7] = half_hi(v.w);
        }
    }
};

}

__device__ __forceinline__ ColorInputs frame_color_inputs(const FrameParams& fp, const CloudPtrs& cloud,
                                                          const uint2* draw_list, const uint2* culled,
                                                          uint32_t draw_count) {
    ColorInputs ci{0.0f, 0.0f, 0.0f};
    if (fp.rasterize_mode == RASTERIZE_DEPTH && fp.n > 0u) {
        const uint32_t j_first = fp.n > 1u ? 1u : 0u, j_last = fp.n - 1u;
        const uint32_t i_first = j_first < draw_count ? draw_list[j_first].y : culled[j_first - draw_count].y;
        const uint32_t i_last = j_last < draw_count ? draw_list[j_last].y : culled[j_last - draw_count].y;
        const float4 pf = cloud.position_visibility[i_first], pl = cloud.position_visibility[i_last];
        ci.max_distance = distance_to_camera(fp, V3{pf.x, pf.y, pf.z});
        ci.min_distance = distance_to_camera(fp, V3{pl.x, pl.y, pl.z});
    }
    return ci;
}

__device__ __forceinline__ void publish_color_max(Control* ctl, const float mag) {
    const uint32_t bits = __float_as_uint(mag);
    if (bits > __hip_atomic_load(&ctl->color_max_bits, __ATOMIC_RELAXED, __HIP_MEMORY_SCOPE_AGENT))
        atomicMax(&ctl->color_max_bits, bits);
}

template <int FMT, bool SURFEL, bool ANY_MODE>
__device__ __forceinline__ uint32_t project_rank(const FrameParams& fp, const CloudPtrs& cloud,
                                                 const uint2 entry, const uint32_t j,
                                                 float4* __restrict__ records, ColorInputs ci,
                                                 bool& visible, float& color_mag) {
    const uint32_t si = entry.y;
    const uint4* __restrict__ rec = cloud.packed + (size_t)si * cloud.packed_v4;
    const float4 pv = *reinterpret_cast<const float4*>(rec);
    float rot[4], so[4], cov[6];
    if constexpr (FMT == (int)CLOUD_COV3D) {
        const float4 c0 = *reinterpret_cast<const float4*>(rec + PACK_COV3D), c1 = *reinterpret_cast<const float4*>(rec + PACK_COV3D + 1u);
        cov[0] = c0.x; cov[1] = c0.y; cov[2] = c0.z; cov[3] = c0.w; cov[4] = c1.x; cov[5] = c1.y;
        rot[0] = 1.0f; rot[1] = rot[2] = rot[3] = 0.0f;
        so[0] = so[1] = so[2] = 0.0f; so[3] = c1.z;
    } else if constexpr (FMT == (int)CLOUD_F16) {
        const uint4 raw = rec[PACK_RSO_F16];
        rot[0] = half_hi(raw.x); rot[1] = half_lo(raw.x);
        rot[2] = half_hi(raw.y); rot[3] = half_lo(raw.y);
        so[0] = half_hi(raw.z); so[1] = half_lo(raw.z);
        so[2] = half_hi(raw.w); so[3] = half_lo(raw.w);
    } else {
        const float4 r4 = *reinterpret_cast<const float4*>(rec + PACK_ROT);
        const float4 s4 = *reinterpret_cast<const float4*>(rec + PACK_SCALE_OPACITY);
        rot[0] = r4.x; rot[1] = r4.y; rot[2] = r4.z; rot[3] = r4.w;
        so[0] = s4.x; so[1] = s4.y; so[2] = s4.z; so[3] = s4.w;
    }
    Projected pr;
    ci.visibility = pv.w;
    if constexpr (FMT == (int)CLOUD_F16)
        project_splat<ANY_MODE>(fp, entry.x, V3{pv.x, pv.y, pv.z}, rot, so, ShF16{reinterpret_cast<const uint32_t*>(rec + PACK_SH_F16)}, ci, pr);
    else if constexpr (FMT == (int)CLOUD_COV3D)
        project_splat<ANY_MODE>(fp, entry.x, V3{pv.x, pv.y, pv.z}, rot, so, ShF32{reinterpret_cast<const float*>(rec + PACK_SH_F32)}, ci, pr, cov);
    else
        project_splat<ANY_MODE>(fp, entry.x, V3{pv.x, pv.y, pv.z}, rot, so, ShF32{reinterpret_cast<const float*>(rec + PACK_SH_F32)}, ci, pr);
    visible = pr.visible;
    if (!pr.draw) return RECT_EMPTY;
    color_mag = fmaxf(color_mag, fmaxf(fabsf(pr.color[0]), fmaxf(fabsf(pr.color[1]), fabsf(pr.color[2]))));
    const uint32_t rect = (uint32_t)pr.tx0 | ((uint32_t)pr.tx1 << 8) | ((uint32_t)pr.ty0 << 16) |
                          ((uint32_t)pr.ty1 << 24);
    if constexpr (SURFEL) {
        float4* dst = records + (size_t)j * 6u;
        dst[0] = make_float4(pr.quad.cx, pr.quad.cy, pr.p[0], pr.p[1]);
        const double T0x = pr.surfel.T[0], T0y = pr.surfel.T[1], T0z = pr.surfel.T[2];
        const double T1x = pr.surfel.T[3], T1y = pr.surfel.T[4], T1z = pr.surfel.T[5];
        const double T2x = pr.surfel.T[6], T2y = pr.surfel.T[7], T2z = pr.surfel.T[8];
        dst[1] = make_float4(pr.radius, pr.surfel.mean_x, pr.surfel.mean_y, (float)(T1y * T2z - T1z * T2y));
        dst[2] = make_float4((float)(T1z * T2x - T1x * T2z), (float)(T1x * T2y - T1y * T2x),
                             (float)(T2y * T0z - T2z * T0y), (float)(T2z * T0x - T2x * T0z));
        dst[3] = make_float4((float)(T2x * T0y - T2y * T0x), (float)(T0y * T1z - T0z * T1y),
                             (float)(T0z * T1x - T0x * T1z), (float)(T0x * T1y - T0y * T1x));
        dst[4] = make_float4(pr.color[0], pr.color[1], pr.color[2], pr.color[3]);
        dst[5] = make_float4(pr.ndc_z, 0.0f, 0.0f, 0.0f);
    } else {
        float4* dst = records + (size_t)j * 3u;
        dst[0] = make_float4(pr.quad.cx, pr.quad.cy, pr.p[0], pr.p[1]);
        dst[1] = make_float4(pr.p[2], pr.p[3], pr.p[4], pr.color[0]);
        dst[2] = make_float4(pr.color[1], pr.color[2], pr.color[3], pr.ndc_z);
    }
    return rect;
}

// ... 43 lines not shown
        }
        const uint32_t inc = wave_inclusive_scan(ntiles, lane);
        if (lane == 63) s_tot[wave] = inc;
        s_rect[tid] = rect;
        __syncthreads();
        const uint32_t w0 = s_tot[0], w1 = s_tot[1], w2 = s_tot[2], w3 = s_tot[3];
        const uint32_t woff = wave == 0 ? 0u : (wave == 1 ? w0 : (wave == 2 ? w0 + w1 : w0 + w1 + w2));
        const uint32_t block_total = w0 + w1 + w2 + w3;
        s_prefix[tid] = woff + inc - ntiles;

        if (tid == 0) {
            unsigned long long excl = 0ull;
            if (tile > 0u) {
                st_agent64(scan_status + tile, S64_AGGREGATE | (unsigned long long)block_total);
                uint32_t p = tile - 1u, spins = 0u;
                for (;;) {
                    const unsigned long long v = ld_agent64(scan_status + p);
                    const unsigned long long flag = v >> S64_FLAG_SHIFT;
                    if (flag == 0ull) {
                        if (++spins > SPIN_LIMIT) { atomicOr(&ctl->error, 2u); break; }
                        __builtin_amdgcn_s_sleep(1);
                        continue;
                    }
                    excl += v & S64_VALUE_MASK;
                    if (flag == 2ull || p == 0u) break;
                    --p;
                }
            }
            const unsigned long long incl = excl + (unsigned long long)block_total;
            st_agent64(scan_status + tile, S64_PREFIX | (incl & S64_VALUE_MASK));
            s_base = excl;
            if (tile == num_tiles - 1u) {
                const bool overflow = incl > (unsigned long long)capacity;
                ctl->instance_total_lo = (uint32_t)incl;
                ctl->instance_total_hi = (uint32_t)(incl >> 32);
                ctl->overflow = overflow ? 1u : 0u;
                ctl->instance_count = overflow ? 0u : (uint32_t)incl;
            }
        }
        if (ntiles) {
            const uint32_t tx0 = rect & 255u, tx1 = (rect >> 8) & 255u;
            const uint32_t ty0 = (rect >> 16) & 255u, ty1 = rect >> 24;
            const uint32_t w = tx1 - tx0 + 1u, h = ty1 - ty0 + 1u;
            for (uint32_t x = tx0; x <= tx1; ++x) atomicAdd(&s_histx[x], h);
            for (uint32_t y = ty0; y <= ty1; ++y) atomicAdd(&s_histy[y], w);
        }
        __syncthreads();

        const unsigned long long base = s_base;
        for (uint32_t i = (uint32_t)tid; i < block_total; i += 256u) {
            uint32_t lo = 0u, hi = 255u;
#pragma unroll
            for (int it = 0; it < 8; ++it) {
                const uint32_t mid = (lo + hi + 1u) >> 1;
                if (s_prefix[mid] <= i) lo = mid; else hi = mid - 1u;
            }
            const uint32_t r = s_rect[lo];
            const uint32_t tx0 = r & 255u, tx1 = (r >> 8) & 255u, ty0 = (r >> 16) & 255u;
            const uint32_t w = tx1 - tx0 + 1u;
            const uint32_t k = i - s_prefix[lo];
            const uint32_t row = k / w, col = k - row * w;
            const unsigned long long g = base + (unsigned long long)i;
            if (g < (unsigned long long)capacity)
                instances[g] = make_uint2(((ty0 + row) << 8) | (tx0 + col), tile * 256u + lo);
        }
        __syncthreads();
    }
    {
        const uint32_t hx = s_histx[tid], hy = s_histy[tid];
        if (hx) atomicAdd(&ctl->hist_tile[0][tid], hx);
        if (hy) atomicAdd(&ctl->hist_tile[1][tid], hy);
    }
#pragma unroll
    for (int off = 32; off > 0; off >>= 1) {
        visible_acc += __shfl_down(visible_acc, off, 64);
        color_mag = fmaxf(color_mag, __shfl_down(color_mag, off, 64));
    }
    if (lane == 0 && visible_acc) atomicAdd(&ctl->visible_count, visible_acc);
    __shared__ float s_cmag[4];
    if (lane == 0) s_cmag[wave] = color_mag;
    __syncthreads();
    if (tid == 0) publish_color_max(ctl, fmaxf(fmaxf(s_cmag[0], s_cmag[1]), fmaxf(s_cmag[2], s_cmag[3])));
}

void launch_project_emit(hipStream_t stream, const FrameParams& fp, const CloudPtrs& cloud,
                         const uint2* draw_list, const uint2* culled, Control* ctl,
                         unsigned long long* scan_status,
                         void* records, uint2* instances, uint32_t capacity, uint32_t ticket_slot,
                         int max_blocks) {
    if (fp.n == 0) return;
    uint32_t blocks = (fp.n + 255u) / 256u;
    if (blocks > (uint32_t)max_blocks) blocks = (uint32_t)max_blocks;
    const bool surfel = fp.gaussian_mode == 0u && fp.aabb != 0u;
    float4* rec = (float4*)records;
    const bool any_mode = fp.rasterize_mode != RASTERIZE_COLOR || fp.draw_mode != 0u;
#define BGS_LAUNCH_PE(F16, SURFEL, ANY)                                                             \
    hipLaunchKernelGGL((project_emit_kernel<F16, SURFEL, ANY>), dim3(blocks), dim3(256), 0, stream, \
                       fp, cloud, draw_list, culled, ctl, scan_status, rec, instances, capacity,    \
                       ticket_slot)
#define BGS_LAUNCH_PE2(F16, SURFEL) \
    do { if (any_mode) BGS_LAUNCH_PE(F16, SURFEL, true); else BGS_LAUNCH_PE(F16, SURFEL, false); } while (0)
    if (cloud.format == CLOUD_F16) {
        if (surfel) BGS_LAUNCH_PE2(1, true); else BGS_LAUNCH_PE2(1, false);
    } else if (cloud.format == CLOUD_COV3D) {
        BGS_LAUNCH_PE2(2, false);
    } else {
        if (surfel) BGS_LAUNCH_PE2(0, true); else BGS_LAUNCH_PE2(0, false);
    }
#undef BGS_LAUNCH_PE2
#undef BGS_LAUNCH_PE
}

template <int FMT, bool SURFEL, bool ANY_MODE>
__global__ __launch_bounds__(256) void project_kernel(const FrameParams* __restrict__ fpp, CloudPtrs cloud,
                                                      const uint2* __restrict__ draw_list,
                                                      const uint2* __restrict__ culled, Control* ctl,
                                                      float4* __restrict__ records, uint32_t* __restrict__ rects) {
    const FrameParams& fp = *fpp;
    const int tid = threadIdx.x, lane = tid & 63, wave = tid >> 6;
    const uint32_t count = ctl->sort_overflow ? 0u : ctl->draw_count;
    const uint32_t num_tiles = (count + 255u) / 256u;
    if (num_tiles == 0u) return;
    uint32_t visible_acc = 0u;
    float color_mag = 0.0f;
    const ColorInputs ci = ANY_MODE ? frame_color_inputs(fp, cloud, draw_list, culled, count)
                                    : ColorInputs{0.0f, 0.0f, 0.0f};
    for (uint32_t tile = blockIdx.x; tile < num_tiles; tile += gridDim.x) {
        const uint32_t j = tile * 256u + (uint32_t)tid;
        if (j < count) {
            bool vis = false;
            rects[j] = project_rank<FMT, SURFEL, ANY_MODE>(fp, cloud, draw_list[count - 1u - j], j, records, ci, vis, color_mag);
            visible_acc += vis ? 1u : 0u;
        }
    }
    __shared__ uint32_t s_vis[4];
#pragma unroll
    for (int off = 32; off > 0; off >>= 1) {
        visible_acc += __shfl_down(visible_acc, off, 64);
        color_mag = fmaxf(color_mag, __shfl_down(color_mag, off, 64));
    }
    __shared__ float s_cmag[4];
    if (lane == 0) {
        s_vis[wave] = visible_acc;
        s_cmag[wave] = color_mag;
    }
    __syncthreads();
    if (tid == 0) {
        const uint32_t v = s_vis[0] + s_vis[1] + s_vis[2] + s_vis[3];
        if (v) atomicAdd(&ctl->visible_count, v);
        publish_color_max(ctl, fmaxf(fmaxf(s_cmag[0], s_cmag[1]), fmaxf(s_cmag[2], s_cmag[3])));
    }
}

#ifndef BGS_BIN_LOOKBACK
#define BGS_BIN_LOOKBACK 4
#endif
constexpr uint32_t BIN_GROUPS = 16u, BIN_RANKS = 64u * BIN_GROUPS;
template <uint32_t WAVES>
__global__ __launch_bounds__(64u * WAVES) void bin_kernel(const uint32_t* __restrict__ rects, Control* ctl, uint32_t* bin_status,
                                                          uint32_t* __restrict__ coarse, uint32_t coarse_cap, uint32_t sup_mul,
                                                          uint32_t sup_x, uint32_t sup_y, uint32_t ticket_slot) {
    constexpr uint32_t GPW = BIN_GROUPS / WAVES;
    constexpr uint32_t TPS = 64u * WAVES / MAX_SUPERTILES;
    static_assert(WAVES == 4u || WAVES == 16u, "256 or 1024 threads");
    __shared__ unsigned long long s_xmask[BIN_GROUPS][32];
    __shared__ unsigned long long s_ymask[BIN_GROUPS][32];
    __shared__ uint32_t s_rect[BIN_RANKS];
    __shared__ uint32_t s_excl[MAX_SUPERTILES];
    __shared__ uint16_t s_off[BIN_GROUPS][MAX_SUPERTILES];
    __shared__ uint32_t s_block_hits;
    __shared__ uint32_t s_tile;

    const int tid = threadIdx.x, lane = tid & 63, wave = tid >> 6;
    const uint32_t count = ctl->sort_overflow ? 0u : ctl->draw_count;
    const uint32_t num_tiles = (count + BIN_RANKS - 1u) / BIN_RANKS;
    if (num_tiles == 0u) return;
    const uint32_t num_st = sup_x * sup_y;
    const uint32_t st_of_thread = (uint32_t)tid & (MAX_SUPERTILES - 1u);
    const uint32_t my_sy = st_of_thread / sup_x, my_sx = st_of_thread - my_sy * sup_x;
    const bool single_shot = gridDim.x >= num_tiles;

    for (;;) {
        if (tid == 0) { s_tile = atomicAdd(&ctl->ticket[ticket_slot][0], 1u); s_block_hits = 0u; }
        __syncthreads();
        const uint32_t tile = s_tile;
        if (tile >= num_tiles) break;
        const uint32_t rank0 = tile * BIN_RANKS;
        uint32_t rect_g[GPW];
#pragma unroll
        for (uint32_t g = 0u; g < GPW; ++g) {
            const uint32_t j = rank0 + ((uint32_t)wave * GPW + g) * 64u + (uint32_t)lane;
            rect_g[g] = j < count ? rects[j] : RECT_EMPTY;
        }
#pragma unroll
        for (uint32_t g = 0u; g < GPW; ++g) {
            const uint32_t q = (uint32_t)wave * GPW + g, rect = rect_g[g];
            s_rect[q * 64u + (uint32_t)lane] = rect;
            const uint32_t sx0 = supertile_div(rect & 255u, sup_mul), sx1 = supertile_div((rect >> 8) & 255u, sup_mul);
            const uint32_t sy0 = supertile_div((rect >> 16) & 255u, sup_mul), sy1 = supertile_div(rect >> 24, sup_mul);
            for (uint32_t c = 0u; c < sup_x; ++c) {
                const unsigned long long b = __ballot(c >= sx0 && c <= sx1);
                if (lane == 0) s_xmask[q][c] = b;
            }
            for (uint32_t r = 0u; r < sup_y; ++r) {
                const unsigned long long b = __ballot(r >= sy0 && r <= sy1);
                if (lane == 0) s_ymask[q][r] = b;
            }
        }
        __syncthreads();
        if ((uint32_t)tid < num_st) {
            uint32_t total = 0u;
#pragma unroll 4
            for (uint32_t g = 0u; g < BIN_GROUPS; ++g) {
                s_off[g][tid] = (uint16_t)total;
                total += (uint32_t)__popcll(s_xmask[g][my_sx] & s_ymask[g][my_sy]);
            }
            uint32_t* const my_status = bin_status + (size_t)tile * MAX_SUPERTILES + tid;
            uint32_t excl = 0u;
            if (tile > 0u) {
                __hip_atomic_store(my_status, STATUS_AGGREGATE | total, __ATOMIC_RELAXED, __HIP_MEMORY_SCOPE_AGENT);
                excl = lookback_u32<BGS_BIN_LOOKBACK>(bin_status + tid, tile, MAX_SUPERTILES, &ctl->error, 4u);
            }
            __hip_atomic_store(my_status, STATUS_PREFIX | ((excl + total) & STATUS_VALUE_MASK),
                               __ATOMIC_RELAXED, __HIP_MEMORY_SCOPE_AGENT);
            if (tile == num_tiles - 1u) ctl->coarse_total[tid] = excl + total;
            s_excl[tid] = excl;
            if (total) atomicAdd(&s_block_hits, total);
        }
        __syncthreads();
        if (s_block_hits >= 32u * num_st) {
            for (uint32_t st = (uint32_t)wave; st < num_st; st += WAVES) {
                const uint32_t sy = st / sup_x, sx = st - sy * sup_x;
                uint32_t pos = s_excl[st];
                uint2* __restrict__ dst = reinterpret_cast<uint2*>(coarse) + (size_t)st * coarse_cap;
                for (uint32_t g = 0u; g < BIN_GROUPS; ++g) {
                    const unsigned long long m = s_xmask[g][sx] & s_ymask[g][sy];
                    const uint32_t at = pos + __builtin_amdgcn_mbcnt_hi((uint32_t)(m >> 32),
                                                                        __builtin_amdgcn_mbcnt_lo((uint32_t)m, 0u));
                    if (((m >> lane) & 1ull) && at < coarse_cap)
                        dst[at] = make_uint2(rank0 + g * 64u + (uint32_t)lane, s_rect[g * 64u + (uint32_t)lane]);
                    pos += (uint32_t)__popcll(m);
                }
            }
        } else if (st_of_thread < num_st) {
            uint2* __restrict__ dst = reinterpret_cast<uint2*>(coarse) + (size_t)st_of_thread * coarse_cap;
            const uint32_t g0 = ((uint32_t)tid >> 8) * (BIN_GROUPS / TPS);
            for (uint32_t g = g0; g < g0 + BIN_GROUPS / TPS; ++g) {
                unsigned long long bits = s_xmask[g][my_sx] & s_ymask[g][my_sy];
                uint32_t pos = s_excl[st_of_thread] + s_off[g][st_of_thread];
                while (bits) {
                    const uint32_t l = (uint32_t)__builtin_ctzll(bits);
                    bits &= bits - 1ull;
                    if (pos < coarse_cap) dst[pos] = make_uint2(rank0 + g * 64u + l, s_rect[g * 64u + l]);
                    ++pos;
                }
            }
        }
        if (single_shot) break;
        __syncthreads();
    }
}

void launch_project_bin(hipStream_t stream, const FrameParams& fp, const FrameParams* d_fp, const CloudPtrs& cloud,
                        const uint2* draw_list, const uint2* culled, Control* ctl, uint32_t* bin_status,
                        void* records, uint32_t* rects, uint32_t* coarse, uint32_t coarse_cap, uint32_t sup_edge,
                        uint32_t ticket_slot, int project_blocks, int bin_blocks, bool wide_bin) {
    if (fp.n == 0) return;
    uint32_t blocks = (fp.n + 255u) / 256u;
    if (blocks > (uint32_t)project_blocks) blocks = (uint32_t)project_blocks;
    const uint32_t sup = sup_edge, sup_mul = supertile_mul(sup_edge);
    const uint32_t sup_x = ((uint32_t)fp.tiles_x + sup - 1u) / sup, sup_y = ((uint32_t)fp.tiles_y + sup - 1u) / sup;
    const bool surfel = fp.gaussian_mode == 0u && fp.aabb != 0u;
    float4* rec = (float4*)records;
    const bool any_mode = fp.rasterize_mode != RASTERIZE_COLOR || fp.draw_mode != 0u;
#define BGS_LAUNCH_PB(F16, SURFEL, ANY)                                                            \
    hipLaunchKernelGGL((project_kernel<F16, SURFEL, ANY>), dim3(blocks), dim3(256), 0, stream,     \
                       d_fp, cloud, draw_list, culled, ctl, rec, rects)
#define BGS_LAUNCH_PB2(F16, SURFEL) \
    do { if (any_mode) BGS_LAUNCH_PB(F16, SURFEL, true); else BGS_LAUNCH_PB(F16, SURFEL, false); } while (0)
    if (cloud.format == CLOUD_F16) {
        if (surfel) BGS_LAUNCH_PB2(1, true); else BGS_LAUNCH_PB2(1, false);
    } else if (cloud.format == CLOUD_COV3D) {
        BGS_LAUNCH_PB2(2, false);
    } else {
        if (surfel) BGS_LAUNCH_PB2(0, true); else BGS_LAUNCH_PB2(0, false);
    }
#undef BGS_LAUNCH_PB2
#undef BGS_LAUNCH_PB
    uint32_t bblocks = (fp.n + BIN_RANKS - 1u) / BIN_RANKS;
    if (bblocks > (uint32_t)bin_blocks) bblocks = (uint32_t)bin_blocks;
    if (wide_bin)
        hipLaunchKernelGGL(bin_kernel<16u>, dim3(bblocks), dim3(1024), 0, stream, rects, ctl, bin_status, coarse, coarse_cap,
                           sup_mul, sup_x, sup_y, ticket_slot);
    else
        hipLaunchKernelGGL(bin_kernel<4u>, dim3(bblocks), dim3(256), 0, stream, rects, ctl, bin_status, coarse, coarse_cap,
                           sup_mul, sup_x, sup_y, ticket_slot);
}

__global__ __launch_bounds__(256) void tile_ranges_kernel(const uint2* __restrict__ inst,
                                                          const Control* ctl, uint2* ranges) {
    const uint32_t n = ctl->instance_count;
    for (uint32_t i = blockIdx.x * 256u + threadIdx.x; i < n; i += gridDim.x * 256u) {
        const uint32_t key = inst[i].x;
        if (i == 0u || inst[i - 1u].x != key) ranges[key].x = i;
        if (i == n - 1u || inst[i + 1u].x != key) ranges[key].y = i + 1u;
    }
}

void launch_tile_ranges(hipStream_t stream, const uint2* instances, const Control* ctl, uint2* ranges) {
    hipLaunchKernelGGL(tile_ranges_kernel, dim3(2048), dim3(256), 0, stream, instances, ctl, ranges);
}

#ifndef BGS_T_EPS_LOG2
#define BGS_T_EPS_LOG2 13
#endif
constexpr float T_EPS = 1.0f / (float)(1u << BGS_T_EPS_LOG2);
constexpr float T_BUDGET = 1.0f / 2048.0f;
__device__ __forceinline__ float frame_t_eps(const uint32_t color_max_bits) {
    return fminf(T_EPS, T_BUDGET / __uint_as_float(color_max_bits));
}

template <int VARIANT>
struct StagedRecord {
    float4 a0, a1, a2, a3, a4, a5;
    __device__ __forceinline__ void load(const float4* __restrict__ rec) {
        a0 = rec[0];
        a1 = rec[1];
        a2 = rec[2];
        if constexpr (VARIANT == 2) {
            a3 = rec[3];
            a4 = rec[4];
            a5 = rec[5];
        }
    }
};

constexpr float OBB_C = 2.5479654147f;
__device__ __forceinline__ void stage_obb(float4& r0, float4& r1, const float ox, const float oy) {
    const float m00 = OBB_C * r0.z, m01 = OBB_C * r0.w, m10 = OBB_C * r1.x, m11 = OBB_C * r1.y;
    const float dx = ox - r0.x, dy = oy - r0.y;
    r0 = make_float4(fmaf(m01, dy, m00 * dx), fmaf(m11, dy, m10 * dx), m00, m01);
    r1.x = m10;
    r1.y = m11;
}

__device__ __forceinline__ void stage_surfel(const float4* __restrict__ src, const float ox, const float oy,
                                             const float aspect, float4 out[6]) {
    const float4 r0 = src[0], r1 = src[1], r2 = src[2], r3 = src[3], r4 = src[4];
    const float Ax = r1.w, Ay = r2.x, Az = r2.y, Bx = r2.z, By = r2.w, Bz = r3.x, Cx = r3.y, Cy = r3.z, Cz = r3.w;
    const float U0 = r0.z * (ox - r0.x), V0 = r0.w * (oy - r0.y);
    const float radius = r1.x;
    const float ax = r0.z * radius, bx = fmaf(U0, radius, r1.y);
    const float ay = r0.w * radius * aspect, by = fmaf(V0 * radius, aspect, r1.z);
    constexpr float C1 = 0.84932180028801907f;
    constexpr float C2 = 1.2011224087864498f;
    out[0] = make_float4(U0, r0.z, V0, r0.w);
    out[1] = make_float4(C1 * fmaf(Ax, bx, fmaf(Bx, by, Cx)), C1 * fmaf(Ay, bx, fmaf(By, by, Cy)),
                         fmaf(Az, bx, fmaf(Bz, by, Cz)), C1 * Ax * ax);
    out[2] = make_float4(C1 * Ay * ax, Az * ax, C1 * Bx * ay, C1 * By * ay);
    out[3] = make_float4(Bz * ay, C2 * (r1.y - bx), -C2 * ax, C2 * (r1.z - by));
    out[4] = make_float4(-C2 * ay, r4.x, r4.y, r4.z);
    out[5] = make_float4(r4.w, 0.0f, 0.0f, 0.0f);
}

#ifndef BGS_SURFEL_CULL_LOG2
#define BGS_SURFEL_CULL_LOG2 23
#endif
__device__ __forceinline__ bool surfel_negligible_in_tile(const float4 st[6], const float limit) {
    constexpr float H = 7.5f;
    const float pxc = fmaf(H, st[1].w + st[2].z, st[1].x), ex = H * (fabsf(st[1].w) + fabsf(st[2].z));
    const float pyc = fmaf(H, st[2].x + st[2].w, st[1].y), ey = H * (fabsf(st[2].x) + fabsf(st[2].w));
    const float pzc = fmaf(H, st[2].y + st[3].x, st[1].z), ez = H * (fabsf(st[2].y) + fabsf(st[3].x));
    const float lx = fmaxf(fabsf(pxc) - ex, 0.0f), ly = fmaxf(fabsf(pyc) - ey, 0.0f), hz = fabsf(pzc) + ez;
    const float s3 = fmaf(lx, lx, ly * ly) * __builtin_amdgcn_rcpf(hz * hz);
    const float dx = fmaxf(fabsf(fmaf(H, st[3].z, st[3].y)) - H * fabsf(st[3].z), 0.0f);
    const float dy = fmaxf(fabsf(fmaf(H, st[4].x, st[3].w)) - H * fabsf(st[4].x), 0.0f);
    const float s2 = fmaf(dx, dx, dy * dy);
    return s3 >= limit && s2 >= limit;
}
__device__ __forceinline__ float frame_surfel_limit(const uint32_t color_max_bits) {
    return (float)BGS_SURFEL_CULL_LOG2 + __builtin_amdgcn_logf(fmaxf(1.0f, __uint_as_float(color_max_bits)));
}

typedef float v2f __attribute__((ext_vector_type(2)));
constexpr float BBOX_EDGE_WIDTH = 0.08f;
constexpr float BBOX_EDGE = 1.0f - 2.0f * BBOX_EDGE_WIDTH;
template <int VARIANT, bool DEPTH = false, bool BBOX = false>
__device__ __forceinline__ void blend_px(const StagedRecord<VARIANT>& s, const float qx, const float qy,
                                         const float aspect, const float t_eps, float& T, v2f& crg, float& cb,
                                         const float z = 0.0f, const float dpx = 0.0f) {
    float alpha, r, g, b;
    bool hit;
    [[maybe_unused]] float bu = 0.0f, bv = 0.0f, blim = 1.0f;
    if constexpr (VARIANT == RV_OBB) {
        const float u = fmaf(s.a0.w, qy, fmaf(s.a0.z, qx, s.a0.x));
        const float v = fmaf(s.a1.y, qy, fmaf(s.a1.x, qx, s.a0.y));
        hit = fmaxf(fabsf(u), fabsf(v)) <= OBB_C;
        if constexpr (BBOX) { bu = u; bv = v; blim = OBB_C; }
        const float e = __builtin_amdgcn_exp2f(-fmaf(u, u, v * v));
        alpha = fminf(e * s.a2.z, 0.999f);
        r = s.a1.w; g = s.a2.x; b = s.a2.y;
    } else if constexpr (VARIANT == RV_AABB3D) {
        const float dx = qx - s.a0.x, dy = qy - s.a0.y;
        const float u = s.a0.z * dx, v = s.a0.w * dy;
        if constexpr (BBOX) { bu = u; bv = v; }
        hit = fmaxf(fabsf(u), fabsf(v)) <= 1.0f;
        const float power = fmaf(s.a1.y * u, v, -0.5f * fmaf(s.a1.x * u, u, s.a1.z * v * v));
        hit = hit && !(power > 0.0f);
        alpha = fminf(__expf(power) * s.a2.z, 0.999f);
        r = s.a1.w; g = s.a2.x; b = s.a2.y;
    } else {
        const float u = fmaf(s.a0.y, qx, s.a0.x), v = fmaf(s.a0.w, qy, s.a0.z);
        if constexpr (BBOX) { bu = u; bv = v; }
        hit = fmaxf(fabsf(u), fabsf(v)) <= 1.0f;
        const float px = fmaf(s.a2.z, qy, fmaf(s.a1.w, qx, s.a1.x));
        const float py = fmaf(s.a2.w, qy, fmaf(s.a2.x, qx, s.a1.y));
        const float pz = fmaf(s.a3.x, qy, fmaf(s.a2.y, qx, s.a1.z));
        const float icz = __builtin_amdgcn_rcpf(pz);
        const float us = px * icz, vs = py * icz;
        const float ddx = fmaf(s.a3.z, qx, s.a3.y), ddy = fmaf(s.a4.x, qy, s.a3.w);
        const float s3 = fmaf(us, us, vs * vs);
        const float s2 = fmaf(ddx, ddx, ddy * ddy);
        alpha = fminf(__builtin_amdgcn_exp2f(-fminf(s3, s2)) * s.a5.x, 0.999f);
        r = s.a4.y; g = s.a4.z; b = s.a4.w;
    }
    if constexpr (DEPTH) hit = hit && z >= dpx;
    if constexpr (BBOX) {
        const bool frame = fmaxf(fabsf(bu), fabsf(bv)) > BBOX_EDGE * blim;
        alpha = frame ? 1.0f : alpha; r = frame ? 0.3f : r; g = frame ? 1.0f : g; b = frame ? 0.1f : b;
    }
    if (hit && T >= t_eps) {
        asm volatile("");
        const float w = T * alpha;
        crg = __builtin_elementwise_fma((v2f){w, w}, (v2f){r, g}, crg);
        cb = fmaf(w, b, cb);
        T -= w;
    }
}

struct PxMs { float S, rb, r0, r1, r2, r3; };
constexpr float MS_OX0 = -0.125f, MS_OY0 = -0.375f, MS_OX1 = 0.375f, MS_OY1 = -0.125f;
__device__ __forceinline__ float ms_margin(const float a, const float b) {
    return fmaxf(fabsf(fmaf(b, MS_OY0, a * MS_OX0)), fabsf(fmaf(b, MS_OY1, a * MS_OX1)));
}
__device__ __forceinline__ float ms_inside(const float x, const float big, const float limbig) {
    float r;
    asm("v_fma_f32 %0, -|%1|, %2, %3 clamp" : "=v"(r) : "v"(x), "v"(big), "v"(limbig));
    return r;
}
// ... 1255 lines not shown
```

### bevy_gaussian_splatting_amd/csrc/sort_kernels.hip

```cpp
#include <hip/hip_runtime.h>
#include <type_traits>

#include "kernels.h"
#include "lookback.h"
#include "splat_math.h"

namespace bgs {

namespace {

__device__ __forceinline__ uint32_t ld_agent(const uint32_t* p) {
    return __hip_atomic_load(p, __ATOMIC_RELAXED, __HIP_MEMORY_SCOPE_AGENT);
}
__device__ __forceinline__ void st_agent(uint32_t* p, uint32_t v) {
    __hip_atomic_store(p, v, __ATOMIC_RELAXED, __HIP_MEMORY_SCOPE_AGENT);
}

__device__ __forceinline__ uint32_t wave_inclusive_scan(uint32_t v, int lane) {
#pragma unroll
    for (int off = 1; off < 64; off <<= 1) {
        uint32_t t = __shfl_up(v, off, 64);
        if (lane >= off) v += t;
    }
    return v;
}

__device__ __forceinline__ uint32_t block_exclusive_scan_256(uint32_t v, uint32_t* s_tot,
                                                             uint32_t& total) {
    const int lane = threadIdx.x & 63, wave = threadIdx.x >> 6;
    const uint32_t inc = wave_inclusive_scan(v, lane);
    if (lane == 63) s_tot[wave] = inc;
    __syncthreads();
    const uint32_t w0 = s_tot[0], w1 = s_tot[1], w2 = s_tot[2], w3 = s_tot[3];
    const uint32_t woff = wave == 0 ? 0u : (wave == 1 ? w0 : (wave == 2 ? w0 + w1 : w0 + w1 + w2));
    total = w0 + w1 + w2 + w3;
    __syncthreads();
    return woff + inc - v;
}


}

#ifndef BGS_KG_GROUP
#define BGS_KG_GROUP 2
#endif
template <int KG_ITEMS, bool BUCKET, int THREADS, bool ORDERED = true>
__global__ __launch_bounds__(THREADS, (THREADS == 1024 && ORDERED) ? 8 : 1) void keygen_kernel(FrameParams fp, const float4* __restrict__ pos,
                                                         uint2* __restrict__ entries,
                                                         uint2* __restrict__ culled, Control* ctl,
                                                         uint32_t* part_status, uint32_t places,
                                                         uint32_t ticket_slot, FrameParams* fp_out,
                                                         uint2* __restrict__ bucket_slots, uint32_t* bucket_status,
                                                         SplitterTable split, uint32_t* zero_word) {
    constexpr int WAVES = THREADS / 64;
    constexpr int ROWS = KG_ITEMS * WAVES;
    static_assert((THREADS == 256 || THREADS == 512 || THREADS == 1024) && ROWS <= 128, "tile geometry");
    __shared__ uint32_t s_hist[BUCKET ? 1 : 4][RADIX_BASE];
    __shared__ uint32_t s_cnt[ROWS];
    __shared__ uint32_t s_off[ROWS];
    __shared__ uint32_t s_keys[THREADS * KG_ITEMS];
    __shared__ uint32_t s_idx[BUCKET ? THREADS * KG_ITEMS : 1];
    extern __shared__ uint32_t s_dyn[];
    uint32_t* const s_bcnt = s_dyn;
    uint32_t* const s_bexcl = s_dyn;
    uint32_t* const s_split = s_dyn + (BUCKET ? BUCKET_COUNT * split.sub : 0u);
    __shared__ uint16_t s_at[BUCKET ? THREADS * KG_ITEMS : 1];
    __shared__ uint16_t s_bk[BUCKET ? THREADS * KG_ITEMS : 1];
    __shared__ uint32_t s_total;
    __shared__ uint32_t s_base;
    __shared__ uint32_t s_tile;
    const int tid = threadIdx.x, lane = tid & 63, wave = tid >> 6;
    if (fp_out && blockIdx.x == 0 && (uint32_t)tid < (uint32_t)(sizeof(FrameParams) / 4u))
        reinterpret_cast<uint32_t*>(fp_out)[tid] = reinterpret_cast<const uint32_t*>(&fp)[tid];
    if (zero_word && blockIdx.x == 0 && tid == 0) *zero_word = 0u;
    const uint32_t nsub = BUCKET ? split.sub : 1u, nb = BUCKET_COUNT * nsub;
    const uint32_t bucket_cap = (BUCKET && split.wide != 0u) ? BUCKET_CAP_WIDE : BUCKET_CAP;
    uint32_t p2 = 256u;
    while (p2 < nb) p2 <<= 1;
    if constexpr (BUCKET) {
        const uint32_t* __restrict__ keys = nsub <= BUCKET_SUB_KERNARG ? split.key : split.device_keys;
        for (uint32_t t = (uint32_t)tid; t < p2; t += (uint32_t)THREADS)
            s_split[t] = t < nb - 1u ? keys[t] : 0xFFFFFFFFu;
    } else if (tid < 256) {
#pragma unroll
        for (int p = 0; p < 4; ++p) s_hist[p][tid] = 0u;
    }
    const uint32_t sentinel = KEY_CULLED >> fp.key_shift;
    constexpr uint32_t per_tile = (uint32_t)(THREADS * KG_ITEMS);
    const uint32_t num_tiles = (fp.n + per_tile - 1u) / per_tile;
    const unsigned long long lanes_below = (1ull << lane) - 1ull;
    const bool single_shot = gridDim.x >= num_tiles;

    auto bucket_of = [&](const uint32_t kk) -> uint32_t {
        uint32_t lo = 0u;
        if (nsub == 1u) {
#pragma unroll
            for (uint32_t step = 128u; step > 0u; step >>= 1)
                if (s_split[lo + step - 1u] <= kk) lo += step;
        } else if (p2 == 512u) {
#pragma unroll
            for (uint32_t step = 256u; step > 0u; step >>= 1)
                if (s_split[lo + step - 1u] <= kk) lo += step;
        } else if (p2 == 1024u) {
#pragma unroll
            for (uint32_t step = 512u; step > 0u; step >>= 1)
                if (s_split[lo + step - 1u] <= kk) lo += step;
        } else {
            for (uint32_t step = p2 >> 1; step > 0u; step >>= 1)
                if (s_split[lo + step - 1u] <= kk) lo += step;
        }
        return min(lo, nb - 1u);
    };
    auto claim_bucket_slots = [&]() {
        if (nb <= (uint32_t)THREADS) {
            if ((uint32_t)tid < nb) {
                const uint32_t mine = s_bcnt[tid];
                s_bexcl[tid] = mine ? atomicAdd(&ctl->bucket_count[tid], mine) : 0u;
            }
            return;
        }
        for (uint32_t f0 = (uint32_t)tid; f0 < nb; f0 += 8u * (uint32_t)THREADS) {
            uint32_t ex[8];
#pragma unroll
            for (uint32_t k = 0; k < 8u; ++k) {
                const uint32_t f = f0 + k * (uint32_t)THREADS;
                const uint32_t mine = f < nb ? s_bcnt[f] : 0u;
                ex[k] = mine ? atomicAdd(&ctl->bucket_count[f], mine) : 0u;
            }
#pragma unroll
            for (uint32_t k = 0; k < 8u; ++k) {
                const uint32_t f = f0 + k * (uint32_t)THREADS;
                if (f < nb) s_bexcl[f] = ex[k];
            }
        }
    };
    if constexpr (BUCKET && !ORDERED) {
        if (blockIdx.x == 0 && tid == 0) ctl->splat_count = fp.n;
        for (uint32_t tile = blockIdx.x; tile < num_tiles; tile += gridDim.x) {
            for (uint32_t f = (uint32_t)tid; f < nb; f += (uint32_t)THREADS) s_bcnt[f] = 0u;
            if (tid == 0) s_total = 0u;
            __syncthreads();
            const uint32_t base = tile * per_tile;
            float4 pin[KG_ITEMS];
#pragma unroll
            for (int k = 0; k < KG_ITEMS; ++k) {
                const uint32_t i = base + (uint32_t)(k * THREADS) + (uint32_t)tid;
                pin[k] = i < fp.n ? pos[i] : make_float4(0.0f, 0.0f, 0.0f, 0.0f);
            }
            uint32_t key[KG_ITEMS], below[KG_ITEMS], rowoff[KG_ITEMS];
            const bool all_draw = fp.sort_mode != SORT_RADIX;
#define BGS_KG_KEYS(KIND)                                                                      \
    _Pragma("unroll") for (int k0 = 0; k0 < KG_ITEMS; k0 += BGS_KG_GROUP) {                    \
         \
        uint32_t unsure_mask = 0u;                                                             \
        _Pragma("unroll") for (int k = k0; k < k0 + BGS_KG_GROUP; ++k) {                       \
// ... 315 lines not shown
#else
__global__ __launch_bounds__(256) void onesweep_kernel(
#endif
const uint2* __restrict__ in,
                                                       uint2* __restrict__ out,
                                                       const uint32_t* __restrict__ n_ptr,
                                                       const uint32_t* __restrict__ hist,
                                                       uint32_t* status, uint32_t* ticket,
                                                       uint32_t* error_flag, uint32_t shift,
                                                       uint32_t key_xor) {
    constexpr uint32_t TILE = 256u * KPT;
    __shared__ uint2 s_pairs[TILE];
    __shared__ uint32_t s_wave_hist[4][RADIX_BASE];
    __shared__ uint32_t s_global_base[RADIX_BASE];
    __shared__ uint32_t s_hist_excl[RADIX_BASE];
    __shared__ uint32_t s_tot[4];
    __shared__ uint32_t s_tile;

    const int tid = threadIdx.x, lane = tid & 63, wave = tid >> 6;
    const uint32_t h = hist[tid];
    const uint32_t n = *n_ptr;
    const uint32_t num_tiles = (n + TILE - 1u) / TILE;
    if (num_tiles == 0u) return;

    {
        uint32_t total;
        s_hist_excl[tid] = block_exclusive_scan_256(h, s_tot, total);
    }
    const bool single_shot = gridDim.x >= num_tiles;

    for (;;) {
        if (tid == 0) s_tile = atomicAdd(ticket, 1u);
#pragma unroll
        for (int w = 0; w < 4; ++w) s_wave_hist[w][tid] = 0u;
        __syncthreads();
        const uint32_t tile = s_tile;
        if (tile >= num_tiles) break;
        auto process = [&](auto full_c) {
            constexpr bool FULL = decltype(full_c)::value;
            const uint32_t tile_base = tile * TILE;
            const uint32_t row_base = tile_base + (uint32_t)wave * (uint32_t)(KPT * 64) + (uint32_t)lane;

            uint2 kv[KPT];
            uint32_t rank[KPT];
    #pragma unroll
            for (int k = 0; k < KPT; ++k) {
                const uint32_t idx = row_base + (uint32_t)k * 64u;
                kv[k] = (FULL || idx < n) ? in[idx] : make_uint2(0xFFFFFFFFu, 0xFFFFFFFFu);
            }
            uint32_t* const wh = s_wave_hist[wave];
    #pragma unroll
            for (int k = 0; k < KPT; ++k) {
                const uint32_t idx = row_base + (uint32_t)k * 64u;
                const bool valid = FULL || idx < n;
                const uint32_t d = (kv[k].x >> shift) & (RADIX_BASE - 1u);
                const unsigned long long mv = FULL ? ~0ull : __ballot(valid);
                uint32_t m_lo = (uint32_t)mv, m_hi = (uint32_t)(mv >> 32);
    #pragma unroll
                for (int b = 0; b < 8; ++b) {
                    const int32_t seli = __builtin_amdgcn_sbfe((int32_t)d, (uint32_t)b, 1u);
                    const uint32_t sel = (uint32_t)seli;
                    const unsigned long long bal = __builtin_amdgcn_ballot_w64(seli < 0);
                    m_lo &= ~((uint32_t)bal ^ sel);
                    m_hi &= ~((uint32_t)(bal >> 32) ^ sel);
                }
                const uint32_t below = __builtin_amdgcn_mbcnt_hi(m_hi, __builtin_amdgcn_mbcnt_lo(m_lo, 0u));
                const uint32_t prev = __atomic_load_n(&wh[d], __ATOMIC_RELAXED);
                __builtin_amdgcn_wave_barrier();
                if (valid && below == 0u) __atomic_store_n(&wh[d], prev + (uint32_t)__popc(m_lo) + (uint32_t)__popc(m_hi), __ATOMIC_RELAXED);
                __builtin_amdgcn_wave_barrier();
                rank[k] = prev + below;
            }
            __syncthreads();

            uint32_t total;
            {
                const uint32_t c0 = s_wave_hist[0][tid], c1 = s_wave_hist[1][tid];
                const uint32_t c2 = s_wave_hist[2][tid], c3 = s_wave_hist[3][tid];
                s_wave_hist[0][tid] = 0u;
                s_wave_hist[1][tid] = c0;
                s_wave_hist[2][tid] = c0 + c1;
                s_wave_hist[3][tid] = c0 + c1 + c2;
                total = c0 + c1 + c2 + c3;
            }
            uint32_t* const my_status = status + (size_t)tile * RADIX_BASE + tid;
            uint32_t excl = 0u;
            if (tile > 0u) {
                st_agent(my_status, STATUS_AGGREGATE | total);
                excl = num_tiles > 1024u ? lookback_u32<16>(status + tid, tile, RADIX_BASE, error_flag, 1u)
                                         : lookback_u32<4>(status + tid, tile, RADIX_BASE, error_flag, 1u);
            }
            st_agent(my_status, STATUS_PREFIX | ((excl + total) & STATUS_VALUE_MASK));

            uint32_t blk_total;
            const uint32_t bexcl = block_exclusive_scan_256(total, s_tot, blk_total);
            s_global_base[tid] = s_hist_excl[tid] + excl - bexcl;
    #pragma unroll
            for (int w = 0; w < 4; ++w) s_wave_hist[w][tid] += bexcl;
            __syncthreads();

    #pragma unroll
            for (int k = 0; k < KPT; ++k) {
                const uint32_t idx = row_base + (uint32_t)k * 64u;
                if (FULL || idx < n) {
                    const uint32_t d = (kv[k].x >> shift) & (RADIX_BASE - 1u);
                    const uint32_t slot = s_wave_hist[wave][d] + rank[k];
                    s_pairs[slot] = kv[k];
                }
            }
            __syncthreads();
            const uint32_t count = FULL ? TILE : min(TILE, n - tile_base);
    #pragma unroll
            for (int k = 0; k < KPT; ++k) {
                const uint32_t slot = (uint32_t)k * 256u + (uint32_t)tid;
                if (FULL || slot < count) {
                    uint2 e = s_pairs[slot];
                    const uint32_t d = (e.x >> shift) & (RADIX_BASE - 1u);
                    e.x ^= key_xor;
                    const uint32_t dst = s_global_base[d] + slot;
                    if (dst < n) out[dst] = e;
                }
            }
        };
        if ((tile + 1u) * TILE <= n) process(std::true_type{}); else process(std::false_type{});
        if (single_shot) break;
        __syncthreads();
    }
}

void launch_onesweep_pass(hipStream_t stream, const uint2* in, uint2* out, const uint32_t* n_ptr,
                          uint32_t max_n, const uint32_t* hist, uint32_t* status, uint32_t* ticket,
                          uint32_t* error_flag, uint32_t shift, uint32_t key_xor, bool large_tiles,
                          int max_blocks) {
    if (max_n == 0) return;
    const uint32_t tile = sort_tile_size(large_tiles);
    uint32_t blocks = (max_n + tile - 1u) / tile;
    if (blocks > (uint32_t)max_blocks) blocks = (uint32_t)max_blocks;
    if (large_tiles)
        hipLaunchKernelGGL(onesweep_kernel<SORT_KPT_LARGE>, dim3(blocks), dim3(256), 0, stream, in, out,
                           n_ptr, hist, status, ticket, error_flag, shift, key_xor);
    else
        hipLaunchKernelGGL(onesweep_kernel<SORT_KPT_SMALL>, dim3(blocks), dim3(256), 0, stream, in, out,
                           n_ptr, hist, status, ticket, error_flag, shift, key_xor);
}

#ifndef BGS_BUCKET_SORT_THREADS
#define BGS_BUCKET_SORT_THREADS 256
#endif
constexpr uint32_t BUCKET_SORT_THREADS = BGS_BUCKET_SORT_THREADS;
template <uint32_t THREADS, uint32_t CAP, uint32_t NF>
__global__ __launch_bounds__(THREADS) void bucket_sort_kernel(const uint2* __restrict__ slots,
                                                              uint2* __restrict__ out, Control* ctl,
                                                              uint32_t key_xor, uint32_t nb ) {
    constexpr uint32_t WAVES = THREADS / 64u;
    constexpr uint32_t EPT = CAP / THREADS;
    constexpr uint32_t FPT = NF / THREADS;
    constexpr bool PACK = NF > 4096u;
    constexpr uint32_t FWORDS = PACK ? NF / 2u + 1u : NF + 1u;
    static_assert((NF == 2048u || NF == 4096u || NF == 8192u) && BUCKET_COUNT == 256u && (THREADS == 256u || THREADS == 1024u) &&
                  EPT >= 1u && FPT >= 2u && FPT % 2u == 0u && CAP <= 65535u, "bucket geometry");
    extern __shared__ uint2 s_el[];
    __shared__ uint32_t s_f[FWORDS];
    __shared__ uint32_t s_tot[WAVES];
    __shared__ uint32_t s_red[WAVES][2];

    const int tid = threadIdx.x, lane = tid & 63, wave = tid >> 6;
    const uint32_t b = blockIdx.x;
    uint32_t before = 0u, mine = 0u, mx = 0u;
    for (uint32_t i = (uint32_t)tid; i < nb; i += THREADS) {
        const uint32_t cnt = ctl->bucket_count[i];
        before += i < b ? cnt : 0u;
        mine += i == b ? cnt : 0u;
        mx = max(mx, cnt);
    }
#pragma unroll
    for (int off = 32; off > 0; off >>= 1) {
        before += (uint32_t)__shfl_xor((int)before, off, 64);
        mine += (uint32_t)__shfl_xor((int)mine, off, 64);
        mx = max(mx, (uint32_t)__shfl_xor((int)mx, off, 64));
    }
    if (lane == 0) { s_red[wave][0] = before; s_red[wave][1] = mine; s_tot[wave] = mx; }
    for (uint32_t j = (uint32_t)tid; j < FWORDS; j += THREADS) s_f[j] = 0u;
    __syncthreads();
    uint32_t base = 0u, m = 0u;
    mx = 0u;
#pragma unroll
    for (uint32_t w = 0; w < WAVES; ++w) { base += s_red[w][0]; m += s_red[w][1]; mx = max(mx, s_tot[w]); }
    if (b == 0u && tid == 0) {
        ctl->bucket_max = mx;
        if (mx > CAP) {
            ctl->sort_overflow = 1u;
            ctl->draw_count = 0u;
        }
    }
    if (b == nb - 1u && tid == 0 && mx <= CAP) ctl->draw_count = base + m;
    if (m == 0u || mx > CAP) return;
    __syncthreads();

    const uint2* __restrict__ src = slots + (size_t)b * CAP;
    uint2 kv[EPT];
    uint32_t kmn = 0xFFFFFFFFu, kmx = 0u;
#pragma unroll
    for (uint32_t k = 0; k < EPT; ++k) {
        const uint32_t e = k * THREADS + (uint32_t)tid;
        kv[k] = make_uint2(0u, 0u);
        if (e < m) {
            kv[k] = src[e];
            kmn = min(kmn, kv[k].x);
            kmx = max(kmx, kv[k].x);
        }
    }
#pragma unroll
    for (int off = 32; off > 0; off >>= 1) {
        kmn = min(kmn, (uint32_t)__shfl_xor((int)kmn, off, 64));
        kmx = max(kmx, (uint32_t)__shfl_xor((int)kmx, off, 64));
    }
    if (lane == 0) { s_red[wave][0] = kmn; s_red[wave][1] = kmx; }
    __syncthreads();
    kmn = 0xFFFFFFFFu; kmx = 0u;
#pragma unroll
    for (uint32_t w = 0; w < WAVES; ++w) { kmn = min(kmn, s_red[w][0]); kmx = max(kmx, s_red[w][1]); }
    const uint32_t span = kmx - kmn;
    const bool direct = span < NF;
    const uint32_t scale = direct ? 0u : (uint32_t)(((unsigned long long)NF << 32) / ((unsigned long long)span + 1ull));
    auto fine_of = [&](const uint32_t key) -> uint32_t { const uint32_t d = key - kmn; return direct ? d : __umulhi(d, scale); };

    uint32_t slot[EPT];
#pragma unroll
    for (uint32_t k = 0; k < EPT; ++k) {
        const uint32_t e = k * THREADS + (uint32_t)tid;
        if (e < m) {
            const uint32_t fb = fine_of(kv[k].x);
            if constexpr (PACK) slot[k] = fb | (((atomicAdd(&s_f[fb >> 1], 1u << ((fb & 1u) << 4)) >> ((fb & 1u) << 4)) & 0xFFFFu) << 16);
            else slot[k] = fb | (atomicAdd(&s_f[fb], 1u) << 16);
        }
    }
    __syncthreads();
    uint32_t f[FPT], fsum = 0u, fmax = 0u;
#pragma unroll
    for (uint32_t j = 0; j < FPT; ++j) {
        if constexpr (PACK) f[j] = (s_f[((uint32_t)tid * FPT + j) >> 1] >> ((j & 1u) << 4)) & 0xFFFFu;
        else f[j] = s_f[(uint32_t)tid * FPT + j];
        fmax = max(fmax, f[j]);
        fsum += f[j];
    }
    const uint32_t finc = wave_inclusive_scan(fsum, lane);
    if (lane == 63) s_tot[wave] = finc;
    __syncthreads();
    uint32_t fexcl = finc - fsum;
#pragma unroll
    for (uint32_t w = 0; w < WAVES; ++w) fexcl += w < (uint32_t)wave ? s_tot[w] : 0u;
    if constexpr (PACK) {
#pragma unroll
        for (uint32_t j = 0; j < FPT; j += 2u) {
            s_f[((uint32_t)tid * FPT + j) >> 1] = fexcl | ((fexcl + f[j]) << 16);
            fexcl += f[j] + f[j + 1u];
        }
        if (tid == 0) s_f[NF / 2u] = m;
    } else {
#pragma unroll
        for (uint32_t j = 0; j < FPT; ++j) {
            s_f[(uint32_t)tid * FPT + j] = fexcl;
            fexcl += f[j];
        }
        if (tid == 0) s_f[NF] = m;
    }
    auto fine_start = [&](const uint32_t fb) -> uint32_t {
        if constexpr (PACK) return (uint32_t)reinterpret_cast<const uint16_t*>(s_f)[fb];
        else return s_f[fb];
    };
    if (__syncthreads_or(fmax > BUCKET_FINE_MAX ? 1 : 0)) {
        if (tid == 0) {
            atomicOr(&ctl->sort_overflow, 2u);
            ctl->draw_count = 0u;
        }
        return;
    }
#pragma unroll
    for (uint32_t k = 0; k < EPT; ++k) {
        const uint32_t e = k * THREADS + (uint32_t)tid;
        if (e < m) s_el[fine_start(slot[k] & 0xFFFFu) + (slot[k] >> 16)] = make_uint2(kv[k].y, kv[k].x);
    }
    __syncthreads();

    const unsigned long long* const s_el64 = reinterpret_cast<const unsigned long long*>(s_el);
    constexpr uint32_t G = EPT >= 8u ? 8u : EPT;
#pragma unroll 1
    for (uint32_t k0 = 0; k0 < EPT; k0 += G) {
        if (k0 * THREADS >= m) break;
        unsigned long long el[G];
        uint32_t fs[G], fe[G];
#pragma unroll
        for (uint32_t k = 0; k < G; ++k) {
            const uint32_t p = (k0 + k) * THREADS + (uint32_t)tid;
            el[k] = s_el64[min(p, m - 1u)];
        }
#pragma unroll
        for (uint32_t k = 0; k < G; ++k) {
            const uint32_t fb = fine_of((uint32_t)(el[k] >> 32));
            fs[k] = fine_start(fb);
            fe[k] = fine_start(fb + 1u);
        }
#pragma unroll
        for (uint32_t k = 0; k < G; ++k) {
            const uint32_t p = (k0 + k) * THREADS + (uint32_t)tid;
            if (p < m) {
                uint32_t r = 0u;
                for (uint32_t j = fs[k]; j < fe[k]; ++j) r += s_el64[j] < el[k] ? 1u : 0u;
                out[base + fs[k] + r] = make_uint2((uint32_t)(el[k] >> 32) ^ key_xor, (uint32_t)el[k]);
            }
        }
    }
}

hipError_t launch_bucket_sort(hipStream_t stream, const uint2* bucket_slots, uint2* out, Control* ctl, uint32_t key_xor, uint32_t buckets,
                              bool wide) {
    if (wide) {
        const auto k = &bucket_sort_kernel<1024u, BUCKET_CAP_WIDE, BUCKET_FINE_WIDE>;
        constexpr int lds = (int)(BUCKET_CAP_WIDE * sizeof(uint2));
        const hipError_t e = hipFuncSetAttribute(reinterpret_cast<const void*>(k), hipFuncAttributeMaxDynamicSharedMemorySize, lds);
        if (e != hipSuccess) return e;
        hipLaunchKernelGGL(k, dim3(buckets), dim3(1024), lds, stream, bucket_slots, out, ctl, key_xor, buckets);
    } else {
        hipLaunchKernelGGL((bucket_sort_kernel<BUCKET_SORT_THREADS, BUCKET_CAP, BUCKET_FINE>), dim3(buckets), dim3(BUCKET_SORT_THREADS),
                           BUCKET_CAP * sizeof(uint2), stream, bucket_slots, out, ctl, key_xor, buckets);
    }
    return hipSuccess;
}

__global__ __launch_bounds__(256) void splitter_kernel(const uint2* __restrict__ sorted, Control* ctl, uint32_t key_xor, uint32_t sub) {
    const uint32_t d = ctl->draw_count, nbk = BUCKET_COUNT * min(max(sub, 1u), BUCKET_SUB_MAX);
    for (uint32_t t = threadIdx.x; t < BUCKET_MAX; t += 256u)
        ctl->splitters[t] = (d != 0u && t < nbk - 1u) ? (sorted[(uint32_t)(((unsigned long long)(t + 1u) * d) / nbk)].x ^ key_xor) : 0xFFFFFFFFu;
}

void launch_splitters(hipStream_t stream, const uint2* sorted, Control* ctl, uint32_t key_xor, uint32_t sub) {
    hipLaunchKernelGGL(splitter_kernel, dim3(1), dim3(256), 0, stream, sorted, ctl, key_xor, sub);
}

__global__ __launch_bounds__(256) void triad_kernel(float4* __restrict__ a, const float4* __restrict__ b,
                                                    const float4* __restrict__ c, float s, size_t n4) {
    const size_t stride = (size_t)gridDim.x * 256u;
    for (size_t i = (size_t)blockIdx.x * 256u + threadIdx.x; i < n4; i += stride) {
        const float4 x = b[i], y = c[i];
        a[i] = make_float4(x.x + s * y.x, x.y + s * y.y, x.z + s * y.z, x.w + s * y.w);
    }
}

__global__ void __launch_bounds__(256) selftest_ln_kernel(uint32_t first_bits, uint32_t count, float* __restrict__ out,
                                                          unsigned long long* __restrict__ sum) {
    unsigned long long acc = 0;
    for (uint64_t i = (uint64_t)blockIdx.x * 256 + threadIdx.x; i < count; i += (uint64_t)gridDim.x * 256) {
        const uint32_t in_bits = first_bits + (uint32_t)i;
        const float r = ln_f32_cr(__uint_as_float(in_bits));
        if (out) out[i] = r;
        acc += ln_selftest_mix(in_bits, __float_as_uint(r));
    }
#pragma unroll
    for (int o = 32; o > 0; o >>= 1) acc += __shfl_xor(acc, o, 64);
    if ((threadIdx.x & 63) == 0) atomicAdd(sum, acc);
}

void launch_selftest_ln(hipStream_t stream, uint32_t first_bits, uint32_t count, float* out, unsigned long long* sum,
                        int blocks) {
    hipLaunchKernelGGL(selftest_ln_kernel, dim3(blocks), dim3(256), 0, stream, first_bits, count, out, sum);
}

void launch_triad(hipStream_t stream, float4* a, const float4* b, const float4* c, float s, size_t n4,
                  int blocks) {
    if (n4 == 0) return;
    hipLaunchKernelGGL(triad_kernel, dim3(blocks), dim3(256), 0, stream, a, b, c, s, n4);
}

}
```

### bevy_gaussian_splatting_amd/plugin.py

```python
from __future__ import annotations

import ctypes
from dataclasses import dataclass
from typing import Optional, Union

import numpy as np

from . import _native
from .camera import View
from .gaussian import PlanarGaussian3d, PlanarGaussian3dF16
from .settings import CloudSettings

SORT_ENTRY_DTYPE = np.dtype([("key", np.uint32), ("index", np.uint32)])


@dataclass
class SortedEntries:

    camera_count: int
    entry_count: int
    sorted: np.ndarray

    @staticmethod
    def new(camera_count: int, entry_count: int) -> "SortedEntries":
# ... 131 lines not shown
                     sorted_entries: Optional[SortedEntries] = None, camera_indices=None) -> SortedEntries:
        views = list(views)
        idx = list(range(len(views))) if camera_indices is None else [int(i) for i in camera_indices]
        if len(idx) != len(views):
            raise ValueError("camera_indices must match views")
        count = (max(idx) + 1) if idx else 0
        if sorted_entries is None:
            sorted_entries = SortedEntries.for_cloud(count, handle.n)
        if count > sorted_entries.camera_count:
            raise ValueError("sorted_entries has fewer camera chunks than the camera indices need")
        for view, ci in zip(views, idx):
            chunk = sorted_entries.chunk(ci, handle.n)
            v, s = view.to_native(), settings.to_native()
            tmp = np.empty(handle.n, dtype=SORT_ENTRY_DTYPE)
            self._check(self._lib.bgs_sort(self._ctx, handle._ptr, ctypes.byref(v), ctypes.byref(s),
                                           tmp.ctypes.data_as(ctypes.POINTER(_native.BgsSortEntry))))
            chunk[:] = tmp
        return sorted_entries

    def prepare(self, view: View, settings: CloudSettings) -> "PreparedView":
        return PreparedView(view.to_native(), settings.to_native(), view.width, view.height)

    def render(self, handle: PlanarGaussian3dHandle, view, settings: Optional[CloudSettings] = None,
               download: bool = True) -> Optional[np.ndarray]:
        if isinstance(view, PreparedView):
            v, s = view.view, view.settings
        else:
            v, s = view.to_native(), settings.to_native()
        if download:
            out = np.empty((view.height, view.width, 4), dtype=np.float32)
            ptr = _fptr(out)
        else:
            out, ptr = None, None
        self._check(self._lib.bgs_render(self._ctx, handle._ptr, ctypes.byref(v), ctypes.byref(s), ptr))
        return out

    def radix_sort_pairs(self, keys: np.ndarray, passes: int = 4) -> np.ndarray:
        keys = np.ascontiguousarray(keys, dtype=np.uint32)
        e = np.empty(keys.shape[0], dtype=SORT_ENTRY_DTYPE)
        e["key"] = keys
        e["index"] = np.arange(keys.shape[0], dtype=np.uint32)
        self._check(
            self._lib.bgs_radix_sort_pairs(
                self._ctx, e.ctypes.data_as(ctypes.POINTER(_native.BgsSortEntry)),
                keys.shape[0], int(passes)))
        return e

    def hbm_probe(self, nbytes: int = 1 << 29, iters: int = 20):
        c, t = ctypes.c_float(), ctypes.c_float()
        self._check(self._lib.bgs_hbm_probe(self._ctx, int(nbytes), int(iters), ctypes.byref(c), ctypes.byref(t)))
        return float(c.value), float(t.value)

    def selftest_ln(self, first_bits: int, count: int, download: Optional[bool] = None):
        if download is None:
            download = count <= (1 << 24)
        out = np.empty(count, np.float32) if download else None
        chk = ctypes.c_uint64()
        self._check(self._lib.bgs_selftest_ln_f32(
            self._ctx, int(first_bits), int(count),
            out.ctypes.data_as(ctypes.POINTER(ctypes.c_float)) if download else None, ctypes.byref(chk)))
        return out, int(chk.value)

    def selftest_pack(self, fmt: str, device_in: int, pixels: int, device_out: int) -> None:
        code = fmt if isinstance(fmt, int) else {"srgb8": 1, "rgba16f": 2}[fmt]
        self._check(self._lib.bgs_selftest_pack(self._ctx, code, device_in or None, int(pixels), device_out or None))

    def set_pipeline_streams(self, streams: int) -> None:
        self._check(self._lib.bgs_set_pipeline_streams(self._ctx, int(streams)))

    def set_graphs(self, enabled: bool) -> None:
        self._check(self._lib.bgs_set_graphs(self._ctx, 1 if enabled else 0))

    def graph_counters(self) -> tuple:
        c, r = ctypes.c_uint64(), ctypes.c_uint64()
        self._check(self._lib.bgs_graph_counters(self._ctx, ctypes.byref(c), ctypes.byref(r)))
        return int(c.value), int(r.value)

    def tile_order_counters(self) -> tuple:
        c, r, n = ctypes.c_uint64(), ctypes.c_uint64(), ctypes.c_uint64()
        self._check(self._lib.bgs_tile_order_counters(self._ctx, ctypes.byref(c), ctypes.byref(r), ctypes.byref(n)))
        return int(c.value), int(r.value), int(n.value)

    def selftest_tile_order(self, cost: np.ndarray, runs: int = 1, sums: bool = False):
        c = np.ascontiguousarray(cost, dtype=np.uint16)
        out = np.empty((c.size + 3) // 4, np.uint16)
        two = np.zeros(2, np.uint32)
        self._check(self._lib.bgs_selftest_tile_order(self._ctx, c.ctypes.data_as(ctypes.c_void_p), c.size, runs,
                                                      out.ctypes.data_as(ctypes.c_void_p), two.ctypes.data_as(ctypes.c_void_p)))
        return (out, (int(two[0]), int(two[1]))) if sums else out

    def synchronize(self) -> None:
        self._check(self._lib.bgs_synchronize(self._ctx))

    def set_profiling(self, level: int) -> None:
        self._check(self._lib.bgs_set_profiling(self._ctx, int(level)))

    def set_profiling_stride(self, every_nth_frame: int) -> None:
        self._check(self._lib.bgs_set_profiling_stride(self._ctx, int(every_nth_frame)))

    def set_pipeline_depth(self, lanes: int) -> None:
        self._check(self._lib.bgs_set_pipeline_depth(self._ctx, int(lanes)))

    def set_output_srgb8(self, enabled: bool) -> None:
        self._check(self._lib.bgs_set_output_srgb8(self._ctx, 1 if enabled else 0))

    def set_srgb8_target(self, device_ptr: Optional[int]) -> None:
        self._check(self._lib.bgs_set_srgb8_target(self._ctx, ctypes.c_void_p(device_ptr or 0)))

    def set_output_rgba16f(self, enabled: bool) -> None:
        self._check(self._lib.bgs_set_output_rgba16f(self._ctx, 1 if enabled else 0))

    def set_packed_only(self, enabled: bool) -> None:
        self._check(self._lib.bgs_set_packed_only(self._ctx, 1 if enabled else 0))

    def framebuffer_rgba16f_device_ptr(self):
        p = ctypes.c_void_p()
        nbytes = ctypes.c_uint64()
        self._check(self._lib.bgs_framebuffer_rgba16f_device_ptr(self._ctx, ctypes.byref(p), ctypes.byref(nbytes)))
        return p.value, nbytes.value

    def framebuffer_srgb8_device_ptr(self):
        p = ctypes.c_void_p()
        nbytes = ctypes.c_uint64()
        self._check(self._lib.bgs_framebuffer_srgb8_device_ptr(self._ctx, ctypes.byref(p), ctypes.byref(nbytes)))
        return p.value, nbytes.value

    def pipeline_pop(self):
        a, b = ctypes.c_void_p(), ctypes.c_void_p()
        self._check(self._lib.bgs_pipeline_pop(self._ctx, ctypes.byref(a), ctypes.byref(b)))
        return a.value, b.value

    def frames_in_flight(self) -> int:
        c = ctypes.c_uint32()
        self._check(self._lib.bgs_frames_in_flight(self._ctx, ctypes.byref(c)))
        return int(c.value)

    def set_async(self, enabled: bool) -> None:
        self._check(self._lib.bgs_set_async(self._ctx, 1 if enabled else 0))

    def set_binning(self, mode: str) -> None:
        self._check(self._lib.bgs_set_binning(self._ctx, {"scan": 0, "sort": 1}[mode]))

    def set_debug_flags(self, flags: int) -> None:
        self._check(self._lib.bgs_set_debug_flags(self._ctx, int(flags)))

    def draw_list(self) -> np.ndarray:
        p, n = ctypes.c_void_p(), ctypes.c_uint32()
        self._check(self._lib.bgs_sorted_entries_device_ptr(self._ctx, ctypes.byref(p), ctypes.byref(n)))
        out = np.empty(n.value, dtype=np.dtype([("key", np.uint32), ("index", np.uint32)]))
        if n.value:
            self._check(self._lib.bgs_download(self._ctx, p, out.ctypes.data_as(ctypes.c_void_p), out.nbytes))
        return out

    def device_alloc(self, nbytes: int) -> int:
        p = ctypes.c_void_p()
        self._check(self._lib.bgs_device_alloc(self._ctx, int(nbytes), ctypes.byref(p)))
        return int(p.value or 0)

    def device_free(self, device_ptr: int) -> None:
        self._check(self._lib.bgs_device_free(self._ctx, ctypes.c_void_p(device_ptr)))

    def upload_bytes(self, device_ptr: int, host: np.ndarray) -> None:
        a = np.ascontiguousarray(host)
        self._check(self._lib.bgs_upload(self._ctx, ctypes.c_void_p(device_ptr), a.ctypes.data_as(ctypes.c_void_p), a.nbytes))

    def download(self, device_ptr: int, host_out: np.ndarray) -> np.ndarray:
        if not host_out.flags["C_CONTIGUOUS"] or not host_out.flags["WRITEABLE"]:
            raise ValueError("host_out must be a writeable C-contiguous array")
        self._check(self._lib.bgs_download(self._ctx, ctypes.c_void_p(device_ptr), host_out.ctypes.data_as(ctypes.c_void_p),
                                           host_out.nbytes))
        return host_out

    def upload_depth(self, depth: np.ndarray) -> int:
        d = np.ascontiguousarray(depth, dtype=np.float32)
        if d.ndim != 3 or d.shape[2] not in (1, 2, 4, 8):
            raise ValueError("depth must be [height, width, samples] with 1, 2, 4 or 8 samples")
        p = self.device_alloc(d.nbytes)
        self.upload_bytes(p, d)
        return p

    def set_tile_trace(self, device_ptr: Optional[int]) -> None:
        self._check(self._lib.bgs_set_tile_trace(self._ctx, ctypes.c_void_p(device_ptr or 0)))

    def build_id(self) -> str:
        return self._lib.bgs_build_id().decode()

    def adaptive_counters(self) -> dict:
        out = (ctypes.c_uint64 * 8)()
        self._check(self._lib.bgs_adaptive_counters(self._ctx, out))
        names = ("bucket_frames", "onesweep_frames", "reruns_sort", "reruns_lists", "reruns_instances",
                 "level_changes", "supertile_level", "list_capacity_hint")
        return {k: int(v) for k, v in zip(names, out)}

    def learning_counters(self) -> dict:
        a, b = ctypes.c_uint64(), ctypes.c_uint64()
        self._check(self._lib.bgs_learning_counters(self._ctx, ctypes.byref(a), ctypes.byref(b)))
        return {"early_frames": a.value, "kinds_settled": b.value}

    @staticmethod
    def comm_unique_id() -> bytes:
        buf = ctypes.create_string_buffer(_native.COMM_ID_BYTES)
        lib = _native.load()
        _native.check(lib, None, lib.bgs_comm_unique_id(buf))
        return buf.raw

    def comm_create(self, unique_id: bytes, world_size: int, rank: int) -> int:
        if len(unique_id) != _native.COMM_ID_BYTES:
            raise ValueError("unique_id must be the 128 bytes of comm_unique_id()")
        out = ctypes.c_void_p()
        self._check(self._lib.bgs_comm_create(self._ctx, unique_id, int(world_size), int(rank), ctypes.byref(out)))
        return out.value

    def comm_gather(self, comm: int, root: int, send_ptr: int, nbytes: int, recv_ptr: Optional[int]) -> int:
        ticket = ctypes.c_uint64()
        self._check(self._lib.bgs_comm_gather(self._ctx, comm, int(root), ctypes.c_void_p(send_ptr), int(nbytes),
                                              ctypes.c_void_p(recv_ptr or 0), ctypes.byref(ticket)))
        return ticket.value

    def comm_gather_after(self, comm: int, root: int, send_ptr: int, nbytes: int, recv_ptr: Optional[int],
                          hip_stream: Optional[int] = None) -> int:
        t = ctypes.c_uint64(0)
        self._check(self._lib.bgs_comm_gather_after(self._ctx, comm, int(root), ctypes.c_void_p(send_ptr), int(nbytes),
                                                    ctypes.c_void_p(recv_ptr or 0), ctypes.c_void_p(hip_stream or 0), ctypes.byref(t)))
        return int(t.value)

    def comm_wait(self, comm: int, ticket: int = 0) -> None:
        self._check(self._lib.bgs_comm_wait(self._ctx, comm, int(ticket)))

    def comm_destroy(self, comm: int) -> None:
        self._lib.bgs_comm_destroy(self._ctx, comm)

    def reset_adaptive_state(self) -> None:
        self._check(self._lib.bgs_reset_adaptive_state(self._ctx))

    def framebuffer_device_ptr(self):
        p = ctypes.c_void_p()
        nbytes = ctypes.c_uint64()
        self._check(self._lib.bgs_framebuffer_device_ptr(self._ctx, ctypes.byref(p), ctypes.byref(nbytes)))
        return p.value, nbytes.value

    def stream_handle(self) -> int:
        p = ctypes.c_void_p()
        self._check(self._lib.bgs_stream(self._ctx, ctypes.byref(p)))
        return p.value or 0

    def stats(self) -> dict:
        st = _native.BgsStats()
        self._check(self._lib.bgs_get_stats(self._ctx, ctypes.byref(st)))
        d = {
            "total_ms": float(st.total_ms),
            "splat_count": int(st.splat_count),
            "visible_count": int(st.visible_count),
            "draw_count": int(st.draw_count),
            "instance_count": int(st.instance_count),
            "instance_capacity": int(st.instance_capacity),
            "list_entries_allocated": int(st.list_entries_allocated),
            "strip_tiles": int(st.strip_tiles),
            "tile_saturation": {"known": bool((int(st.tile_saturation) >> 16) & 1), "work_share": (int(st.tile_saturation) & 0x7FFF) / 0x7FFF,
                                "midround_exit": bool(int(st.tile_saturation) >> 31)},
            "tiles": (int(st.tiles_x), int(st.tiles_y)),
            "depth_passes": int(st.depth_passes),
            "tile_passes": int(st.tile_passes),
            "algorithmic_bytes": int(st.algorithmic_bytes),
            "regrow_count": int(st.regrow_count),
            "sort_path": "bucket" if st.sort_path else "onesweep",
            "list_capacity": int(st.list_capacity),
            "binning": "sort" if st.binning_mode else "scan",
            "frames_averaged": int(st.frames_averaged),
            "stage_ms": {n: float(st.stage_ms[i]) for i, n in enumerate(_native.STAGE_NAMES)},
        }
        return d
```

### include/bgs.h

```cpp
#ifndef BGS_H
#define BGS_H

#include <stdint.h>

#ifdef __cplusplus
extern "C" {
#endif

#define BGS_VERSION_MAJOR 0
#define BGS_VERSION_MINOR 4

typedef enum bgs_status {
    BGS_OK = 0,
    BGS_EINVAL = -1,
    BGS_ENOMEM = -2,
    BGS_EHIP = -3,
    BGS_ECAPACITY = -4,
    BGS_EINTERNAL = -5
} bgs_status;

typedef struct bgs_ctx bgs_ctx;
typedef struct bgs_cloud bgs_cloud;

typedef struct bgs_view {
    float world_from_view[16];
    float view_from_world[16];
    float clip_from_view[16];
    float clip_from_world[16];
    float viewport[4];
    float clear_color[4];
    float previous_clip_from_world[16];
    float delta_time;
    uint32_t sample_count;
    uint32_t reserved[2];
    uint64_t depth_device_ptr;
    uint64_t reserved_ptr;
} bgs_view;

#define BGS_GAUSSIAN_2D 0u
#define BGS_GAUSSIAN_3D 1u
#define BGS_COLOR_SRGB 0u
#define BGS_COLOR_LINEAR 1u
#define BGS_SORT_NONE 0u
#define BGS_SORT_RADIX 1u
#define BGS_SORT_RAYON 2u
#define BGS_SORT_STD 3u

#define BGS_RASTERIZE_CLASSIFICATION 0u
#define BGS_RASTERIZE_COLOR 1u
#define BGS_RASTERIZE_DEPTH 2u
#define BGS_RASTERIZE_NORMAL 3u
#define BGS_RASTERIZE_OPTICAL_FLOW 4u
#define BGS_RASTERIZE_POSITION 5u
#define BGS_RASTERIZE_VELOCITY 6u

#define BGS_DRAW_ALL 0u
#define BGS_DRAW_SELECTED 1u
#define BGS_DRAW_HIGHLIGHT_SELECTED 2u

typedef struct bgs_settings {
    float transform[16];
    float global_opacity;
    float global_scale;
    uint32_t gaussian_mode;
    uint32_t aabb;
    uint32_t opacity_adaptive_radius;
    uint32_t color_space;
    uint32_t radix_depth_bits;
    uint32_t sh_degree;
    uint32_t sort_mode;
    uint32_t rasterize_mode;
    uint32_t num_classes;
    uint32_t draw_mode;
    uint32_t visualize_bounding_box;
    uint32_t reserved[1];
    float position_min[4];
    float position_max[4];
} bgs_settings;

typedef struct bgs_sort_entry {
    uint32_t key;
    uint32_t index;
} bgs_sort_entry;

#define BGS_STAGE_KEYGEN 0
#define BGS_STAGE_DEPTH_SORT 1
#define BGS_STAGE_PROJECT 2
#define BGS_STAGE_TILE_SORT 3
#define BGS_STAGE_RANGES 4
#define BGS_STAGE_RASTER 5
#define BGS_STAGE_COUNT 6

typedef struct bgs_stats {
    float stage_ms[BGS_STAGE_COUNT];
    float total_ms;
    uint32_t splat_count;
    uint32_t visible_count;
    uint32_t draw_count;
    uint32_t sort_path;
    uint64_t instance_count;
    uint64_t instance_capacity;
    uint32_t tiles_x, tiles_y;
    uint32_t depth_passes;
    uint32_t tile_passes;
    uint64_t algorithmic_bytes;
    uint32_t regrow_count;
    uint32_t binning_mode;
    uint32_t frames_averaged;
    uint32_t list_capacity;
    uint64_t list_entries_allocated;
    uint32_t strip_tiles;
    uint32_t tile_saturation;
} bgs_stats;

int bgs_create(int hip_device, bgs_ctx** out);
void bgs_destroy(bgs_ctx* ctx);
const char* bgs_last_error(const bgs_ctx* ctx);
uint32_t bgs_version(void);
#define BGS_ABI_VERSION ((BGS_VERSION_MAJOR << 16) | BGS_VERSION_MINOR)
int bgs_abi_check(uint32_t version, uint32_t sizeof_view, uint32_t sizeof_settings, uint32_t sizeof_stats);
const char* bgs_build_id(void);

void bgs_settings_default(bgs_settings* out);

void bgs_view_perspective(const float world_from_view[16], float fov_y_radians,
                          float near_plane, uint32_t width, uint32_t height,
                          bgs_view* out);

int bgs_cloud_upload_f32(bgs_ctx* ctx, uint32_t n, const float* position_visibility,
                         const float* spherical_harmonic, const float* rotation,
                         const float* scale_opacity, bgs_cloud** out);
int bgs_cloud_upload_f16(bgs_ctx* ctx, uint32_t n, const float* position_visibility,
                         const uint32_t* spherical_harmonic_h2,
                         const uint32_t* rotation_scale_opacity, bgs_cloud** out);
int bgs_cloud_upload_cov3d_f32(bgs_ctx* ctx, uint32_t n, const float* position_visibility,
                               const float* spherical_harmonic, const float* covariance_3d_opacity,
                               bgs_cloud** out);
void bgs_cloud_free(bgs_ctx* ctx, bgs_cloud* cloud);
uint32_t bgs_cloud_len(const bgs_cloud* cloud);

int bgs_sort(bgs_ctx* ctx, const bgs_cloud* cloud, const bgs_view* view,
             const bgs_settings* settings, bgs_sort_entry* host_out);

int bgs_render(bgs_ctx* ctx, const bgs_cloud* cloud, const bgs_view* view,
               const bgs_settings* settings, float* rgba_host_out);

int bgs_framebuffer_device_ptr(bgs_ctx* ctx, void** dptr, uint64_t* bytes);
int bgs_set_output_srgb8(bgs_ctx* ctx, int enabled);
int bgs_framebuffer_srgb8_device_ptr(bgs_ctx* ctx, void** dptr, uint64_t* bytes);
int bgs_set_output_rgba16f(bgs_ctx* ctx, int enabled);
int bgs_framebuffer_rgba16f_device_ptr(bgs_ctx* ctx, void** dptr, uint64_t* bytes);
int bgs_set_packed_only(bgs_ctx* ctx, int enabled);
int bgs_set_srgb8_target(bgs_ctx* ctx, void* device_ptr);
int bgs_download(bgs_ctx* ctx, const void* device_ptr, void* host_out, uint64_t bytes);
int bgs_device_alloc(bgs_ctx* ctx, uint64_t bytes, void** device_ptr_out);
int bgs_device_free(bgs_ctx* ctx, void* device_ptr);
int bgs_upload(bgs_ctx* ctx, void* device_ptr, const void* host_in, uint64_t bytes);

int bgs_set_pipeline_depth(bgs_ctx* ctx, uint32_t lanes );
int bgs_pipeline_pop(bgs_ctx* ctx, void** rgba_f32_dptr_or_null, void** rgba8_dptr_or_null);
int bgs_frames_in_flight(bgs_ctx* ctx, uint32_t* count);

int bgs_sorted_entries_device_ptr(bgs_ctx* ctx, void** dptr, uint32_t* n);

int bgs_synchronize(bgs_ctx* ctx);
int bgs_set_async(bgs_ctx* ctx, int enabled);
int bgs_stream(bgs_ctx* ctx, void** hip_stream);

#define BGS_BINNING_SCAN 0u
#define BGS_BINNING_SORT 1u
int bgs_set_binning(bgs_ctx* ctx, uint32_t mode);

int bgs_reset_adaptive_state(bgs_ctx* ctx);
int bgs_set_profiling(bgs_ctx* ctx, int enabled);
int bgs_set_profiling_stride(bgs_ctx* ctx, uint32_t every_nth_frame);
int bgs_get_stats(bgs_ctx* ctx, bgs_stats* out);

int bgs_set_pipeline_streams(bgs_ctx* ctx, uint32_t streams);
int bgs_set_graphs(bgs_ctx* ctx, int enabled);

#define BGS_COMM_ID_BYTES 128
typedef struct bgs_comm bgs_comm;
int bgs_comm_unique_id(uint8_t id_out[BGS_COMM_ID_BYTES]);
int bgs_comm_create(bgs_ctx* ctx, const uint8_t id[BGS_COMM_ID_BYTES], uint32_t world_size, uint32_t rank, bgs_comm** out);
int bgs_comm_gather(bgs_ctx* ctx, bgs_comm* comm, uint32_t root, const void* send_device_ptr, uint64_t bytes_per_rank,
                    void* recv_device_ptr_root_only, uint64_t* ticket_out_or_null);
int bgs_comm_gather_after(bgs_ctx* ctx, bgs_comm* comm, uint32_t root, const void* send_device_ptr, uint64_t bytes_per_rank,
                          void* recv_device_ptr_root_only, void* hip_stream_or_null, uint64_t* ticket_out_or_null);
int bgs_comm_wait(bgs_ctx* ctx, bgs_comm* comm, uint64_t ticket);
int bgs_comm_stream(bgs_ctx* ctx, bgs_comm* comm, void** hip_stream);
void bgs_comm_destroy(bgs_ctx* ctx, bgs_comm* comm);
#ifdef __cplusplus
}
#endif
#endif
```

### include/bgs_diag.h

```cpp
#ifndef BGS_DIAG_H
#define BGS_DIAG_H

#include "bgs.h"

#ifdef __cplusplus
extern "C" {
#endif

enum bgs_debug_flag {
    BGS_DEBUG_BUCKETS_NARROW = 0x100,
    BGS_DEBUG_SPLIT_SUB_3 = 0x200,
    BGS_DEBUG_SPLIT_SUB_5 = 0x400,
    BGS_DEBUG_BUCKETS_WIDE = 0x800,
    BGS_DEBUG_NO_RASTER_CLEANUP = 0x1000,
    BGS_DEBUG_NO_DRAW_HINT = 0x2000,
    BGS_DEBUG_NO_GRAPHS = 0x4000,
    BGS_DEBUG_LEVEL_1 = 0x8000,
    BGS_DEBUG_LEVEL_0 = 0x10000,
    BGS_DEBUG_MIDROUND_ALWAYS = 0x20000,
    BGS_DEBUG_SEPARATE_ENCODE = 0x40000,
    BGS_DEBUG_NO_BUCKET_SORT = 0x80000,
    BGS_DEBUG_SMALL_LISTS = 0x100000,
    BGS_DEBUG_GUESSED_SPLITTERS = 0x200000,
    BGS_DEBUG_LEVEL_2 = 0x400000,
    BGS_DEBUG_LEVEL_3 = 0x800000,
    BGS_DEBUG_NO_MIDROUND = 0x1000000,
    BGS_DEBUG_NO_STRIPS = 0x2000000,
    BGS_DEBUG_STRIPS_ANY_DEPTH = 0x4000000,
    BGS_DEBUG_RERUN_EVERY_FRAME = 0x8000000,
    BGS_DEBUG_NO_TILE_COST = 0x10000000,
    BGS_DEBUG_NO_TILE_COST_PIPELINED = 0x20000000,
    BGS_DEBUG_ORDER_EVERY_FRAME = 0x40000000
};
int bgs_set_debug_flags(bgs_ctx* ctx, uint32_t flags);

int bgs_adaptive_counters(bgs_ctx* ctx, uint64_t out[8]);

int bgs_learning_counters(bgs_ctx* ctx, uint64_t* early_frames, uint64_t* kinds_settled);

int bgs_radix_sort_pairs(bgs_ctx* ctx, bgs_sort_entry* entries_inout, uint32_t n,
                         uint32_t passes);

int bgs_hbm_probe(bgs_ctx* ctx, uint64_t bytes, uint32_t iters, float* copy_gbs, float* triad_gbs);

int bgs_selftest_ln_f32(bgs_ctx* ctx, uint32_t first_bits, uint32_t count, float* host_out, uint64_t* checksum_out);

int bgs_set_queue_holders(int enabled);

int bgs_set_tile_trace(bgs_ctx* ctx, void* device_ptr);

int bgs_graph_counters(bgs_ctx* ctx, uint64_t* captures, uint64_t* replays);

int bgs_tile_order_counters(bgs_ctx* ctx, uint64_t* cost_frames, uint64_t* ordered_frames, uint64_t* refreshes);

int bgs_selftest_tile_order(bgs_ctx* ctx, const uint16_t* host_cost, uint32_t ntiles, uint32_t runs, uint16_t* host_order,
                            uint32_t* host_sums);

enum bgs_pack_format { BGS_PACK_SRGB8 = 1, BGS_PACK_RGBA16F = 2 };
int bgs_selftest_pack(bgs_ctx* ctx, uint32_t format, const void* device_in_rgba_f32, uint32_t pixels, void* device_out);

#ifdef __cplusplus
}
#endif
#endif
```

Baseline: 23420 frames/s.

## Fuse bucket sort with per-splat projection in one kernel

Pulls the bucket sort body into a shared header and adds a fused kernel that sorts each depth bucket and then projects the sorted splats in the same block, writing records and rects directly. The project_bin launch is told the splats are already projected and only does binning. This removes a separate pass that re-reads the sorted draw list and restarts work, at the cost of higher register and LDS pressure in the fused kernel and fewer blocks' worth of parallelism for the projection work. A debug flag restores the split path, and a diagnostic API exposes the vertex-stage buffers.

Result: faster. 24190 frames/s, median of 6 (+3.3%).

```diff
diff --git a/bevy_gaussian_splatting_amd/_native.py b/bevy_gaussian_splatting_amd/_native.py
--- a/bevy_gaussian_splatting_amd/_native.py
+++ b/bevy_gaussian_splatting_amd/_native.py
@@ -40,6 +40,7 @@
     "bgs_render",
     "bgs_framebuffer_device_ptr",
     "bgs_sorted_entries_device_ptr",
+    "bgs_vertex_stage_device_ptr",
     "bgs_set_output_srgb8",
     "bgs_framebuffer_srgb8_device_ptr",
     "bgs_set_srgb8_target",
@@ -226,6 +227,8 @@
     lib.bgs_framebuffer_device_ptr.restype = ctypes.c_int
     lib.bgs_sorted_entries_device_ptr.argtypes = [vp, ctypes.POINTER(vp), up]
     lib.bgs_sorted_entries_device_ptr.restype = ctypes.c_int
+    lib.bgs_vertex_stage_device_ptr.argtypes = [vp, ctypes.POINTER(vp), up, ctypes.POINTER(vp), up]
+    lib.bgs_vertex_stage_device_ptr.restype = ctypes.c_int
     lib.bgs_synchronize.argtypes = [vp]
     lib.bgs_synchronize.restype = ctypes.c_int
     lib.bgs_set_output_srgb8.argtypes = [vp, ctypes.c_int]
diff --git a/bevy_gaussian_splatting_amd/csrc/bgs_api.hip b/bevy_gaussian_splatting_amd/csrc/bgs_api.hip
--- a/bevy_gaussian_splatting_amd/csrc/bgs_api.hip
+++ b/bevy_gaussian_splatting_amd/csrc/bgs_api.hip
@@ -330,6 +330,22 @@
     return BGS_OK;
 }
 
+int bgs_vertex_stage_device_ptr(bgs_ctx* ctx, void** records, uint32_t* record_bytes, void** rects, uint32_t* ranks) {
+    if (!ctx || !records || !record_bytes || !rects || !ranks) return fail(ctx, BGS_EINVAL, "NULL argument");
+    Lane& L = ctx->lanes[ctx->recent];
+    if (L.pending) {
+        int rc = finish_lane(ctx, L);
+        if (rc != BGS_OK) return rc;
+    }
+    if (!L.plan.render || !L.plan.scan || !L.records || !L.rects)
+        return fail(ctx, BGS_EINVAL, "the last call was not a BGS_BINNING_SCAN render");
+    *records = (void*)L.records;
+    *record_bytes = L.plan.rec_bytes;
+    *rects = (void*)L.rects;
+    *ranks = L.h_ctl->draw_count;
+    return BGS_OK;
+}
+
 int bgs_synchronize(bgs_ctx* ctx) {
     if (!ctx) return fail(nullptr, BGS_EINVAL, "ctx is NULL");
     if (hipSetDevice(ctx->device) != hipSuccess) return fail(ctx, BGS_EHIP, "hipSetDevice failed");
diff --git a/bevy_gaussian_splatting_amd/csrc/bgs_context.h b/bevy_gaussian_splatting_amd/csrc/bgs_context.h
--- a/bevy_gaussian_splatting_amd/csrc/bgs_context.h
+++ b/bevy_gaussian_splatting_amd/csrc/bgs_context.h
@@ -86,6 +86,7 @@
     bool render = false, scan = false, surfel = false, culled_tail = true;
     uint32_t n = 0, places = 0, rec_bytes = 0, cloud_format = 0;
     bool bucket = false, wide = false;
+    bool fused = false;
     uint32_t bucket_sub = 1, split_sub_out = 1;
     int split_slot = -1;
     uint64_t split_epoch = 0;
diff --git a/bevy_gaussian_splatting_amd/csrc/bgs_frame.hip b/bevy_gaussian_splatting_amd/csrc/bgs_frame.hip
--- a/bevy_gaussian_splatting_amd/csrc/bgs_frame.hip
+++ b/bevy_gaussian_splatting_amd/csrc/bgs_frame.hip
@@ -690,6 +690,8 @@
     }
     if (p.bucket && slot >= 0) { p.split_slot = slot; p.split_epoch = ctx.split_slots[slot].epoch; }
     fp.sort_path = p.bucket ? 1u : 0u;
+    p.fused = p.bucket && !p.wide && in.render && p.scan && fp.rasterize_mode == RASTERIZE_COLOR && fp.draw_mode == 0u &&
+              !(flags & BGS_DEBUG_SPLIT_SORT_PROJECT);
 
     supertile_edges((uint32_t)fp.tiles_x, (uint32_t)fp.tiles_y, p.edges);
     uint32_t level = ctx.sup_level;
@@ -764,7 +766,7 @@
     key.sup_edge = p.sup_edge;
     key.scratch_bytes = L.scratch_bytes; key.scratch_inst_cap = L.scratch_inst_cap; key.scratch_n = L.scratch_n;
     key.coarse_cap = coarse_cap;
-    key.sort_path = p.bucket ? (p.bucket_sub | (p.wide ? 0x100u : 0u)) : 0u;
+    key.sort_path = p.bucket ? (p.bucket_sub | (p.wide ? 0x100u : 0u) | (p.fused ? 0x200u : 0u)) : 0u;
     return key;
 }
 
@@ -934,8 +936,13 @@
         mark(1);
         int cur = 0;
         if (bucket) {
-            const hipError_t e = launch_bucket_sort(st, L.bucket_slots, draw_list, ctl, final_xor, BUCKET_COUNT * p.bucket_sub, p.wide);
-            if (e != hipSuccess) return e;
+            if (p.fused) {
+                launch_bucket_sort_project(st, fp, L.d_fp, in.cloud->ptrs, L.bucket_slots, draw_list, ctl, final_xor,
+                                           BUCKET_COUNT * p.bucket_sub, L.records, L.rects);
+            } else {
+                const hipError_t e = launch_bucket_sort(st, L.bucket_slots, draw_list, ctl, final_xor, BUCKET_COUNT * p.bucket_sub, p.wide);
+                if (e != hipSuccess) return e;
+            }
         }
         for (uint32_t q = 0; q < (bucket ? 0u : places); ++q) {
             launch_onesweep_pass(st, L.entries[cur], L.entries[cur ^ 1], &ctl->draw_count, n, ctl->hist_depth[q],
@@ -946,7 +953,7 @@
         mark(2);
         if (render && scan) {
             launch_project_bin(st, fp, L.d_fp, in.cloud->ptrs, draw_list, L.culled, ctl, bin_status, L.records, L.rects, L.coarse,
-                               coarse_cap, p.sup_edge, 4, p.bin_blocks, p.binning_blocks, p.wide_bin);
+                               coarse_cap, p.sup_edge, 4, p.bin_blocks, p.binning_blocks, p.wide_bin, p.fused);
             mark(3);
             launch_raster_scan(st, fp, L.d_fp, L.records, L.coarse, coarse_cap, p.sup_edge, ctl, L.fb, L.fb8,
                                (flags & BGS_DEBUG_SEPARATE_ENCODE) ? 0u : p.out_format, cl, ctx->tile_trace,
diff --git a/bevy_gaussian_splatting_amd/csrc/bucket_sort.h b/bevy_gaussian_splatting_amd/csrc/bucket_sort.h
--- /dev/null
+++ b/bevy_gaussian_splatting_amd/csrc/bucket_sort.h
@@ -0,0 +1,203 @@
+#pragma once
+
+#include <hip/hip_runtime.h>
+#include <stdint.h>
+
+#include "bgs_device.h"
+
+namespace bgs {
+
+__device__ __forceinline__ uint32_t bucket_wave_inclusive_scan(uint32_t v, int lane) {
+#pragma unroll
+    for (int off = 1; off < 64; off <<= 1) {
+        uint32_t t = __shfl_up(v, off, 64);
+        if (lane >= off) v += t;
+    }
+    return v;
+}
+
+struct BucketPlace {
+    uint32_t base;
+    uint32_t pairs;
+    uint32_t count;
+};
+
+template <uint32_t THREADS, uint32_t CAP, uint32_t NF, bool WANT_COUNT, class Placed>
+__device__ __forceinline__ bool bucket_sort_body(const uint2* __restrict__ slots, uint2* __restrict__ out, Control* ctl,
+                                                 uint32_t key_xor, uint32_t nb ,
+                                                 BucketPlace& place, Placed&& placed) {
+    constexpr uint32_t WAVES = THREADS / 64u;
+    constexpr uint32_t EPT = CAP / THREADS;
+    constexpr uint32_t FPT = NF / THREADS;
+    constexpr bool PACK = NF > 4096u;
+    constexpr uint32_t FWORDS = PACK ? NF / 2u + 1u : NF + 1u;
+    static_assert((NF == 2048u || NF == 4096u || NF == 8192u) && BUCKET_COUNT == 256u && (THREADS == 256u || THREADS == 1024u) &&
+                  EPT >= 1u && FPT >= 2u && FPT % 2u == 0u && CAP <= 65535u, "bucket geometry");
+    extern __shared__ uint2 s_el[];
+    __shared__ uint32_t s_f[FWORDS];
+    __shared__ uint32_t s_tot[WAVES];
+    __shared__ uint32_t s_red[WAVES][WANT_COUNT ? 3 : 2];
+
+    const int tid = threadIdx.x, lane = tid & 63, wave = tid >> 6;
+    const uint32_t b = blockIdx.x;
+    uint32_t before = 0u, mine = 0u, mx = 0u, all = 0u;
+    for (uint32_t i = (uint32_t)tid; i < nb; i += THREADS) {
+        const uint32_t cnt = ctl->bucket_count[i];
+        before += i < b ? cnt : 0u;
+        mine += i == b ? cnt : 0u;
+        mx = max(mx, cnt);
+        if constexpr (WANT_COUNT) all += cnt;
+    }
+#pragma unroll
+    for (int off = 32; off > 0; off >>= 1) {
+        before += (uint32_t)__shfl_xor((int)before, off, 64);
+        mine += (uint32_t)__shfl_xor((int)mine, off, 64);
+        mx = max(mx, (uint32_t)__shfl_xor((int)mx, off, 64));
+        if constexpr (WANT_COUNT) all += (uint32_t)__shfl_xor((int)all, off, 64);
+    }
+    if (lane == 0) {
+        s_red[wave][0] = before; s_red[wave][1] = mine; s_tot[wave] = mx;
+        if constexpr (WANT_COUNT) s_red[wave][2] = all;
+    }
+    for (uint32_t j = (uint32_t)tid; j < FWORDS; j += THREADS) s_f[j] = 0u;
+    __syncthreads();
+    uint32_t base = 0u, m = 0u;
+    mx = 0u;
+#pragma unroll
+    for (uint32_t w = 0; w < WAVES; ++w) { base += s_red[w][0]; m += s_red[w][1]; mx = max(mx, s_tot[w]); }
+    if constexpr (WANT_COUNT) {
+        all = 0u;
+#pragma unroll
+        for (uint32_t w = 0; w < WAVES; ++w) all += s_red[w][2];
+    }
+    place.base = base; place.pairs = m; place.count = all;
+    if (b == 0u && tid == 0) {
+        ctl->bucket_max = mx;
+        if (mx > CAP) {
+            ctl->sort_overflow = 1u;
+            ctl->draw_count = 0u;
+        }
+    }
+    if (b == nb - 1u && tid == 0 && mx <= CAP) ctl->draw_count = base + m;
+    if (m == 0u || mx > CAP) return false;
+    __syncthreads();
+
+    const uint2* __restrict__ src = slots + (size_t)b * CAP;
+    uint2 kv[EPT];
+    uint32_t kmn = 0xFFFFFFFFu, kmx = 0u;
+#pragma unroll
+    for (uint32_t k = 0; k < EPT; ++k) {
+        const uint32_t e = k * THREADS + (uint32_t)tid;
+        kv[k] = make_uint2(0u, 0u);
+        if (e < m) {
+            kv[k] = src[e];
+            kmn = min(kmn, kv[k].x);
+            kmx = max(kmx, kv[k].x);
+        }
+    }
+#pragma unroll
+    for (int off = 32; off > 0; off >>= 1) {
+        kmn = min(kmn, (uint32_t)__shfl_xor((int)kmn, off, 64));
+        kmx = max(kmx, (uint32_t)__shfl_xor((int)kmx, off, 64));
+    }
+    if (lane == 0) { s_red[wave][0] = kmn; s_red[wave][1] = kmx; }
+    __syncthreads();
+    kmn = 0xFFFFFFFFu; kmx = 0u;
+#pragma unroll
+    for (uint32_t w = 0; w < WAVES; ++w) { kmn = min(kmn, s_red[w][0]); kmx = max(kmx, s_red[w][1]); }
+    const uint32_t span = kmx - kmn;
+    const bool direct = span < NF;
+    const uint32_t scale = direct ? 0u : (uint32_t)(((unsigned long long)NF << 32) / ((unsigned long long)span + 1ull));
+    auto fine_of = [&](const uint32_t key) -> uint32_t { const uint32_t d = key - kmn; return direct ? d : __umulhi(d, scale); };
+
+    uint32_t slot[EPT];
+#pragma unroll
+    for (uint32_t k = 0; k < EPT; ++k) {
+        const uint32_t e = k * THREADS + (uint32_t)tid;
+        if (e < m) {
+            const uint32_t fb = fine_of(kv[k].x);
+            if constexpr (PACK) slot[k] = fb | (((atomicAdd(&s_f[fb >> 1], 1u << ((fb & 1u) << 4)) >> ((fb & 1u) << 4)) & 0xFFFFu) << 16);
+            else slot[k] = fb | (atomicAdd(&s_f[fb], 1u) << 16);
+        }
+    }
+    __syncthreads();
+    uint32_t f[FPT], fsum = 0u, fmax = 0u;
+#pragma unroll
+    for (uint32_t j = 0; j < FPT; ++j) {
+        if constexpr (PACK) f[j] = (s_f[((uint32_t)tid * FPT + j) >> 1] >> ((j & 1u) << 4)) & 0xFFFFu;
+        else f[j] = s_f[(uint32_t)tid * FPT + j];
+        fmax = max(fmax, f[j]);
+        fsum += f[j];
+    }
+    const uint32_t finc = bucket_wave_inclusive_scan(fsum, lane);
+    if (lane == 63) s_tot[wave] = finc;
+    __syncthreads();
+    uint32_t fexcl = finc - fsum;
+#pragma unroll
+    for (uint32_t w = 0; w < WAVES; ++w) fexcl += w < (uint32_t)wave ? s_tot[w] : 0u;
+    if constexpr (PACK) {
+#pragma unroll
+        for (uint32_t j = 0; j < FPT; j += 2u) {
+            s_f[((uint32_t)tid * FPT + j) >> 1] = fexcl | ((fexcl + f[j]) << 16);
+            fexcl += f[j] + f[j + 1u];
+        }
+        if (tid == 0) s_f[NF / 2u] = m;
+    } else {
+#pragma unroll
+        for (uint32_t j = 0; j < FPT; ++j) {
+            s_f[(uint32_t)tid * FPT + j] = fexcl;
+            fexcl += f[j];
+        }
+        if (tid == 0) s_f[NF] = m;
+    }
+    auto fine_start = [&](const uint32_t fb) -> uint32_t {
+        if constexpr (PACK) return (uint32_t)reinterpret_cast<const uint16_t*>(s_f)[fb];
+        else return s_f[fb];
+    };
+    if (__syncthreads_or(fmax > BUCKET_FINE_MAX ? 1 : 0)) {
+        if (tid == 0) {
+            atomicOr(&ctl->sort_overflow, 2u);
+            ctl->draw_count = 0u;
+        }
+        return false;
+    }
+#pragma unroll
+    for (uint32_t k = 0; k < EPT; ++k) {
+        const uint32_t e = k * THREADS + (uint32_t)tid;
+        if (e < m) s_el[fine_start(slot[k] & 0xFFFFu) + (slot[k] >> 16)] = make_uint2(kv[k].y, kv[k].x);
+    }
+    __syncthreads();
+
+    const unsigned long long* const s_el64 = reinterpret_cast<const unsigned long long*>(s_el);
+    constexpr uint32_t G = EPT >= 8u ? 8u : EPT;
+#pragma unroll 1
+    for (uint32_t k0 = 0; k0 < EPT; k0 += G) {
+        if (k0 * THREADS >= m) break;
+        unsigned long long el[G];
+        uint32_t fs[G], fe[G];
+#pragma unroll
+        for (uint32_t k = 0; k < G; ++k) {
+            const uint32_t p = (k0 + k) * THREADS + (uint32_t)tid;
+            el[k] = s_el64[min(p, m - 1u)];
+        }
+#pragma unroll
+        for (uint32_t k = 0; k < G; ++k) {
+            const uint32_t fb = fine_of((uint32_t)(el[k] >> 32));
+            fs[k] = fine_start(fb);
+            fe[k] = fine_start(fb + 1u);
+        }
+#pragma unroll
+        for (uint32_t k = 0; k < G; ++k) {
+            const uint32_t p = (k0 + k) * THREADS + (uint32_t)tid;
+            if (p < m) {
+                uint32_t r = 0u;
+                for (uint32_t j = fs[k]; j < fe[k]; ++j) r += s_el64[j] < el[k] ? 1u : 0u;
+                out[base + fs[k] + r] = make_uint2((uint32_t)(el[k] >> 32) ^ key_xor, (uint32_t)el[k]);
+                placed(p, fs[k] + r);
+            }
+        }
+    }
+    return true;
+}
+
+}
diff --git a/bevy_gaussian_splatting_amd/csrc/kernels.h b/bevy_gaussian_splatting_amd/csrc/kernels.h
--- a/bevy_gaussian_splatting_amd/csrc/kernels.h
+++ b/bevy_gaussian_splatting_amd/csrc/kernels.h
@@ -90,7 +90,10 @@
 void launch_project_bin(hipStream_t stream, const FrameParams& fp, const FrameParams* d_fp, const CloudPtrs& cloud,
                         const uint2* draw_list, const uint2* culled, Control* ctl, uint32_t* bin_status, void* records,
                         uint32_t* rects, uint32_t* coarse, uint32_t coarse_cap, uint32_t sup_edge,
-                        uint32_t ticket_slot, int project_blocks, int bin_blocks, bool wide_bin);
+                        uint32_t ticket_slot, int project_blocks, int bin_blocks, bool wide_bin, bool projected = false);
+void launch_bucket_sort_project(hipStream_t stream, const FrameParams& fp, const FrameParams* d_fp, const CloudPtrs& cloud,
+                                const uint2* bucket_slots, uint2* out, Control* ctl, uint32_t key_xor, uint32_t buckets,
+                                void* records, uint32_t* rects);
 
 void launch_raster_scan(hipStream_t stream, const FrameParams& fp, const FrameParams* d_fp, const void* records,
                         const uint32_t* coarse, uint32_t coarse_cap,
diff --git a/bevy_gaussian_splatting_amd/csrc/render_kernels.hip b/bevy_gaussian_splatting_amd/csrc/render_kernels.hip
--- a/bevy_gaussian_splatting_amd/csrc/render_kernels.hip
+++ b/bevy_gaussian_splatting_amd/csrc/render_kernels.hip
@@ -4,6 +4,7 @@
 #include <hip/hip_fp16.h>
 #include <hip/hip_runtime.h>
 
+#include "bucket_sort.h"
 #include "kernels.h"
 #include "lookback.h"
 #include "pack_tables.h"
@@ -353,6 +354,52 @@
     }
 }
 
+template <int FMT, bool SURFEL>
+__global__ __launch_bounds__(256) void bucket_sort_project_kernel(const uint2* __restrict__ slots, uint2* __restrict__ out, Control* ctl,
+                                                                  uint32_t key_xor, uint32_t nb, const FrameParams* __restrict__ fpp,
+                                                                  CloudPtrs cloud, float4* __restrict__ records,
+                                                                  uint32_t* __restrict__ rects) {
+    extern __shared__ uint2 s_el[];
+    __shared__ uint16_t s_perm[BUCKET_CAP];
+    __shared__ uint32_t s_vis[4];
+    __shared__ float s_cmag[4];
+    BucketPlace place;
+    if (!bucket_sort_body<256u, BUCKET_CAP, BUCKET_FINE, true>(slots, out, ctl, key_xor, nb, place,
+                                                              [&](uint32_t p, uint32_t d) { s_perm[d] = (uint16_t)p; }))
+        return;
+    __syncthreads();
+    const FrameParams& fp = *fpp;
+    const int tid = threadIdx.x, lane = tid & 63, wave = tid >> 6;
+    const unsigned long long* const s_el64 = reinterpret_cast<const unsigned long long*>(s_el);
+    uint32_t visible_acc = 0u;
+    float color_mag = 0.0f;
+    const ColorInputs ci{0.0f, 0.0f, 0.0f};
+    const uint32_t j0 = place.count - place.base - place.pairs;
+#pragma unroll 1
+    for (uint32_t r = (uint32_t)tid; r < place.pairs; r += 256u) {
+        const unsigned long long el = s_el64[s_perm[place.pairs - 1u - r]];
+        const uint32_t j = j0 + r;
+        bool vis = false;
+        rects[j] = project_rank<FMT, SURFEL, false>(fp, cloud, make_uint2((uint32_t)(el >> 32) ^ key_xor, (uint32_t)el), j, records, ci, vis, color_mag);
+        visible_acc += vis ? 1u : 0u;
+    }
+#pragma unroll
+    for (int off = 32; off > 0; off >>= 1) {
+        visible_acc += __shfl_down(visible_acc, off, 64);
+        color_mag = fmaxf(color_mag, __shfl_down(color_mag, off, 64));
+    }
+    if (lane == 0) {
+        s_vis[wave] = visible_acc;
+        s_cmag[wave] = color_mag;
+    }
+    __syncthreads();
+    if (tid == 0) {
+        const uint32_t v = s_vis[0] + s_vis[1] + s_vis[2] + s_vis[3];
+        if (v) atomicAdd(&ctl->visible_count, v);
+        publish_color_max(ctl, fmaxf(fmaxf(s_cmag[0], s_cmag[1]), fmaxf(s_cmag[2], s_cmag[3])));
+    }
+}
+
 #ifndef BGS_BIN_LOOKBACK
 #define BGS_BIN_LOOKBACK 4
 #endif
@@ -465,7 +512,7 @@
 void launch_project_bin(hipStream_t stream, const FrameParams& fp, const FrameParams* d_fp, const CloudPtrs& cloud,
                         const uint2* draw_list, const uint2* culled, Control* ctl, uint32_t* bin_status,
                         void* records, uint32_t* rects, uint32_t* coarse, uint32_t coarse_cap, uint32_t sup_edge,
-                        uint32_t ticket_slot, int project_blocks, int bin_blocks, bool wide_bin) {
+                        uint32_t ticket_slot, int project_blocks, int bin_blocks, bool wide_bin, bool projected) {
     if (fp.n == 0) return;
     uint32_t blocks = (fp.n + 255u) / 256u;
     if (blocks > (uint32_t)project_blocks) blocks = (uint32_t)project_blocks;
@@ -479,7 +526,8 @@
                        d_fp, cloud, draw_list, culled, ctl, rec, rects)
 #define BGS_LAUNCH_PB2(F16, SURFEL) \
     do { if (any_mode) BGS_LAUNCH_PB(F16, SURFEL, true); else BGS_LAUNCH_PB(F16, SURFEL, false); } while (0)
-    if (cloud.format == CLOUD_F16) {
+    if (projected) {
+    } else if (cloud.format == CLOUD_F16) {
         if (surfel) BGS_LAUNCH_PB2(1, true); else BGS_LAUNCH_PB2(1, false);
     } else if (cloud.format == CLOUD_COV3D) {
         BGS_LAUNCH_PB2(2, false);
@@ -496,6 +544,23 @@
     else
         hipLaunchKernelGGL(bin_kernel<4u>, dim3(bblocks), dim3(256), 0, stream, rects, ctl, bin_status, coarse, coarse_cap,
                            sup_mul, sup_x, sup_y, ticket_slot);
+}
+
+void launch_bucket_sort_project(hipStream_t stream, const FrameParams& fp, const FrameParams* d_fp, const CloudPtrs& cloud,
+                                const uint2* bucket_slots, uint2* out, Control* ctl, uint32_t key_xor, uint32_t buckets,
+                                void* records, uint32_t* rects) {
+    const bool surfel = fp.gaussian_mode == 0u && fp.aabb != 0u;
+#define BGS_LAUNCH_BSP(FMT, SURFEL)                                                                                      \
+    hipLaunchKernelGGL((bucket_sort_project_kernel<FMT, SURFEL>), dim3(buckets), dim3(256), BUCKET_CAP * sizeof(uint2), \
+                       stream, bucket_slots, out, ctl, key_xor, buckets, d_fp, cloud, (float4*)records, rects)
+    if (cloud.format == CLOUD_F16) {
+        if (surfel) BGS_LAUNCH_BSP(1, true); else BGS_LAUNCH_BSP(1, false);
+    } else if (cloud.format == CLOUD_COV3D) {
+        BGS_LAUNCH_BSP(2, false);
+    } else {
+        if (surfel) BGS_LAUNCH_BSP(0, true); else BGS_LAUNCH_BSP(0, false);
+    }
+#undef BGS_LAUNCH_BSP
 }
 
 __global__ __launch_bounds__(256) void tile_ranges_kernel(const uint2* __restrict__ inst,
diff --git a/bevy_gaussian_splatting_amd/csrc/sort_kernels.hip b/bevy_gaussian_splatting_amd/csrc/sort_kernels.hip
--- a/bevy_gaussian_splatting_amd/csrc/sort_kernels.hip
+++ b/bevy_gaussian_splatting_amd/csrc/sort_kernels.hip
@@ -1,6 +1,7 @@
 #include <hip/hip_runtime.h>
 #include <type_traits>
 
+#include "bucket_sort.h"
 #include "kernels.h"
 #include "lookback.h"
 #include "splat_math.h"
@@ -622,165 +623,8 @@
 __global__ __launch_bounds__(THREADS) void bucket_sort_kernel(const uint2* __restrict__ slots,
                                                               uint2* __restrict__ out, Control* ctl,
                                                               uint32_t key_xor, uint32_t nb ) {
-    constexpr uint32_t WAVES = THREADS / 64u;
-    constexpr uint32_t EPT = CAP / THREADS;
-    constexpr uint32_t FPT = NF / THREADS;
-    constexpr bool PACK = NF > 4096u;
-    constexpr uint32_t FWORDS = PACK ? NF / 2u + 1u : NF + 1u;
-    static_assert((NF == 2048u || NF == 4096u || NF == 8192u) && BUCKET_COUNT == 256u && (THREADS == 256u || THREADS == 1024u) &&
-                  EPT >= 1u && FPT >= 2u && FPT % 2u == 0u && CAP <= 65535u, "bucket geometry");
-    extern __shared__ uint2 s_el[];
-    __shared__ uint32_t s_f[FWORDS];
-    __shared__ uint32_t s_tot[WAVES];
-    __shared__ uint32_t s_red[WAVES][2];
-
-    const int tid = threadIdx.x, lane = tid & 63, wave = tid >> 6;
-    const uint32_t b = blockIdx.x;
-    uint32_t before = 0u, mine = 0u, mx = 0u;
-    for (uint32_t i = (uint32_t)tid; i < nb; i += THREADS) {
-        const uint32_t cnt = ctl->bucket_count[i];
-        before += i < b ? cnt : 0u;
-        mine += i == b ? cnt : 0u;
-        mx = max(mx, cnt);
-    }
-#pragma unroll
-    for (int off = 32; off > 0; off >>= 1) {
-        before += (uint32_t)__shfl_xor((int)before, off, 64);
-        mine += (uint32_t)__shfl_xor((int)mine, off, 64);
-        mx = max(mx, (uint32_t)__shfl_xor((int)mx, off, 64));
-    }
-    if (lane == 0) { s_red[wave][0] = before; s_red[wave][1] = mine; s_tot[wave] = mx; }
-    for (uint32_t j = (uint32_t)tid; j < FWORDS; j += THREADS) s_f[j] = 0u;
-    __syncthreads();
-    uint32_t base = 0u, m = 0u;
-    mx = 0u;
-#pragma unroll
-    for (uint32_t w = 0; w < WAVES; ++w) { base += s_red[w][0]; m += s_red[w][1]; mx = max(mx, s_tot[w]); }
-    if (b == 0u && tid == 0) {
-        ctl->bucket_max = mx;
-        if (mx > CAP) {
-            ctl->sort_overflow = 1u;
-            ctl->draw_count = 0u;
-        }
-    }
-    if (b == nb - 1u && tid == 0 && mx <= CAP) ctl->draw_count = base + m;
-    if (m == 0u || mx > CAP) return;
-    __syncthreads();
-
-    const uint2* __restrict__ src = slots + (size_t)b * CAP;
-    uint2 kv[EPT];
-    uint32_t kmn = 0xFFFFFFFFu, kmx = 0u;
-#pragma unroll
-    for (uint32_t k = 0; k < EPT; ++k) {
-        const uint32_t e = k * THREADS + (uint32_t)tid;
-        kv[k] = make_uint2(0u, 0u);
-        if (e < m) {
-            kv[k] = src[e];
-            kmn = min(kmn, kv[k].x);
-            kmx = max(kmx, kv[k].x);
-        }
-    }
-#pragma unroll
-    for (int off = 32; off > 0; off >>= 1) {
-        kmn = min(kmn, (uint32_t)__shfl_xor((int)kmn, off, 64));
-        kmx = max(kmx, (uint32_t)__shfl_xor((int)kmx, off, 64));
-    }
-    if (lane == 0) { s_red[wave][0] = kmn; s_red[wave][1] = kmx; }
-    __syncthreads();
-    kmn = 0xFFFFFFFFu; kmx = 0u;
-#pragma unroll
-    for (uint32_t w = 0; w < WAVES; ++w) { kmn = min(kmn, s_red[w][0]); kmx = max(kmx, s_red[w][1]); }
-    const uint32_t span = kmx - kmn;
-    const bool direct = span < NF;
-    const uint32_t scale = direct ? 0u : (uint32_t)(((unsigned long long)NF << 32) / ((unsigned long long)span + 1ull));
-    auto fine_of = [&](const uint32_t key) -> uint32_t { const uint32_t d = key - kmn; return direct ? d : __umulhi(d, scale); };
-
-    uint32_t slot[EPT];
-#pragma unroll
-    for (uint32_t k = 0; k < EPT; ++k) {
-        const uint32_t e = k * THREADS + (uint32_t)tid;
-        if (e < m) {
-            const uint32_t fb = fine_of(kv[k].x);
-            if constexpr (PACK) slot[k] = fb | (((atomicAdd(&s_f[fb >> 1], 1u << ((fb & 1u) << 4)) >> ((fb & 1u) << 4)) & 0xFFFFu) << 16);
-            else slot[k] = fb | (atomicAdd(&s_f[fb], 1u) << 16);
-        }
-    }
-    __syncthreads();
-    uint32_t f[FPT], fsum = 0u, fmax = 0u;
-#pragma unroll
-    for (uint32_t j = 0; j < FPT; ++j) {
-        if constexpr (PACK) f[j] = (s_f[((uint32_t)tid * FPT + j) >> 1] >> ((j & 1u) << 4)) & 0xFFFFu;
-        else f[j] = s_f[(uint32_t)tid * FPT + j];
-        fmax = max(fmax, f[j]);
-        fsum += f[j];
-    }
-    const uint32_t finc = wave_inclusive_scan(fsum, lane);
-    if (lane == 63) s_tot[wave] = finc;
-    __syncthreads();
-    uint32_t fexcl = finc - fsum;
-#pragma unroll
-    for (uint32_t w = 0; w < WAVES; ++w) fexcl += w < (uint32_t)wave ? s_tot[w] : 0u;
-    if constexpr (PACK) {
-#pragma unroll
-        for (uint32_t j = 0; j < FPT; j += 2u) {
-            s_f[((uint32_t)tid * FPT + j) >> 1] = fexcl | ((fexcl + f[j]) << 16);
-            fexcl += f[j] + f[j + 1u];
-        }
-        if (tid == 0) s_f[NF / 2u] = m;
-    } else {
-#pragma unroll
-        for (uint32_t j = 0; j < FPT; ++j) {
-            s_f[(uint32_t)tid * FPT + j] = fexcl;
-            fexcl += f[j];
-        }
-        if (tid == 0) s_f[NF] = m;
-    }
-    auto fine_start = [&](const uint32_t fb) -> uint32_t {
-        if constexpr (PACK) return (uint32_t)reinterpret_cast<const uint16_t*>(s_f)[fb];
-        else return s_f[fb];
-    };
-    if (__syncthreads_or(fmax > BUCKET_FINE_MAX ? 1 : 0)) {
-        if (tid == 0) {
-            atomicOr(&ctl->sort_overflow, 2u);
-            ctl->draw_count = 0u;
-        }
-        return;
-    }
-#pragma unroll
-    for (uint32_t k = 0; k < EPT; ++k) {
-        const uint32_t e = k * THREADS + (uint32_t)tid;
-        if (e < m) s_el[fine_start(slot[k] & 0xFFFFu) + (slot[k] >> 16)] = make_uint2(kv[k].y, kv[k].x);
-    }
-    __syncthreads();
-
-    const unsigned long long* const s_el64 = reinterpret_cast<const unsigned long long*>(s_el);
-    constexpr uint32_t G = EPT >= 8u ? 8u : EPT;
-#pragma unroll 1
-    for (uint32_t k0 = 0; k0 < EPT; k0 += G) {
-        if (k0 * THREADS >= m) break;
-        unsigned long long el[G];
-        uint32_t fs[G], fe[G];
-#pragma unroll
-        for (uint32_t k = 0; k < G; ++k) {
-            const uint32_t p = (k0 + k) * THREADS + (uint32_t)tid;
-            el[k] = s_el64[min(p, m - 1u)];
-        }
-#pragma unroll
-        for (uint32_t k = 0; k < G; ++k) {
-            const uint32_t fb = fine_of((uint32_t)(el[k] >> 32));
-            fs[k] = fine_start(fb);
-            fe[k] = fine_start(fb + 1u);
-        }
-#pragma unroll
-        for (uint32_t k = 0; k < G; ++k) {
-            const uint32_t p = (k0 + k) * THREADS + (uint32_t)tid;
-            if (p < m) {
-                uint32_t r = 0u;
-                for (uint32_t j = fs[k]; j < fe[k]; ++j) r += s_el64[j] < el[k] ? 1u : 0u;
-                out[base + fs[k] + r] = make_uint2((uint32_t)(el[k] >> 32) ^ key_xor, (uint32_t)el[k]);
-            }
-        }
-    }
+    BucketPlace place;
+    bucket_sort_body<THREADS, CAP, NF, false>(slots, out, ctl, key_xor, nb, place, [](uint32_t, uint32_t) {});
 }
 
 hipError_t launch_bucket_sort(hipStream_t stream, const uint2* bucket_slots, uint2* out, Control* ctl, uint32_t key_xor, uint32_t buckets,
diff --git a/bevy_gaussian_splatting_amd/plugin.py b/bevy_gaussian_splatting_amd/plugin.py
--- a/bevy_gaussian_splatting_amd/plugin.py
+++ b/bevy_gaussian_splatting_amd/plugin.py
@@ -307,6 +307,17 @@
             self._check(self._lib.bgs_download(self._ctx, p, out.ctypes.data_as(ctypes.c_void_p), out.nbytes))
         return out
 
+    def vertex_stage(self):
+        rec, rct, nb, n = ctypes.c_void_p(), ctypes.c_void_p(), ctypes.c_uint32(), ctypes.c_uint32()
+        self._check(self._lib.bgs_vertex_stage_device_ptr(self._ctx, ctypes.byref(rec), ctypes.byref(nb), ctypes.byref(rct),
+                                                          ctypes.byref(n)))
+        rects = np.empty(n.value, np.uint32)
+        records = np.empty((n.value, nb.value // 4), np.float32)
+        if n.value:
+            self._check(self._lib.bgs_download(self._ctx, rct, rects.ctypes.data_as(ctypes.c_void_p), rects.nbytes))
+            self._check(self._lib.bgs_download(self._ctx, rec, records.ctypes.data_as(ctypes.c_void_p), records.nbytes))
+        return rects, records
+
     def device_alloc(self, nbytes: int) -> int:
         p = ctypes.c_void_p()
         self._check(self._lib.bgs_device_alloc(self._ctx, int(nbytes), ctypes.byref(p)))
diff --git a/include/bgs.h b/include/bgs.h
--- a/include/bgs.h
+++ b/include/bgs.h
@@ -162,6 +162,7 @@
 int bgs_frames_in_flight(bgs_ctx* ctx, uint32_t* count);
 
 int bgs_sorted_entries_device_ptr(bgs_ctx* ctx, void** dptr, uint32_t* n);
+int bgs_vertex_stage_device_ptr(bgs_ctx* ctx, void** records, uint32_t* record_bytes, void** rects, uint32_t* ranks);
 
 int bgs_synchronize(bgs_ctx* ctx);
 int bgs_set_async(bgs_ctx* ctx, int enabled);
diff --git a/include/bgs_diag.h b/include/bgs_diag.h
--- a/include/bgs_diag.h
+++ b/include/bgs_diag.h
@@ -8,6 +8,7 @@
 #endif
 
 enum bgs_debug_flag {
+    BGS_DEBUG_SPLIT_SORT_PROJECT = 0x80,
     BGS_DEBUG_BUCKETS_NARROW = 0x100,
     BGS_DEBUG_SPLIT_SUB_3 = 0x200,
     BGS_DEBUG_SPLIT_SUB_5 = 0x400,
```
